# ElenaRyumina/AVCER

Measured on AMD Instinct MI355X. Metric: clips/sec (224x224x16f + 2s@16kHz), full AV path: static CNN + LSTM + wav2vec2 audio model + fusion, higher is better.
Workload: dtype f16x3 (f16 MFMA on hi/lo-split f32 operands, f32 accumulate)

## Files before the change

avcer_amd/_lib.py:

```python
from __future__ import annotations

import ctypes as C
import os

from .build import LIB, source_hash

c_ctx = C.c_void_p
c_stream = C.c_void_p


class ConvDesc(C.Structure):
    _fields_ = [
        ("batch", C.c_int32), ("in_h", C.c_int32), ("in_w", C.c_int32),
        ("out_h", C.c_int32), ("out_w", C.c_int32),
        ("cin", C.c_int32), ("kh", C.c_int32), ("kw", C.c_int32),
        ("stride_h", C.c_int32), ("stride_w", C.c_int32), ("pad_h", C.c_int32), ("pad_w", C.c_int32),
        ("dil_h", C.c_int32), ("dil_w", C.c_int32),
        ("x_stride_b", C.c_int64), ("x_stride_h", C.c_int64), ("x_stride_w", C.c_int64),
        ("x_coff", C.c_int32), ("n", C.c_int32),
        ("y_ld", C.c_int64), ("y_coff", C.c_int32),
        ("r_ld", C.c_int64), ("r_coff", C.c_int32),
        ("act", C.c_int32), ("res_after_act", C.c_int32), ("groups", C.c_int32),
        ("x2_cin", C.c_int32), ("x2_coff", C.c_int32), ("x2_stride", C.c_int32),
        ("x2_stride_b", C.c_int64), ("x2_stride_h", C.c_int64), ("x2_stride_w", C.c_int64),
        ("tile_n", C.c_int32),
        ("r_sub", C.c_int32), ("r_h", C.c_int32), ("r_w", C.c_int32),
        ("tile_m", C.c_int32),
    ]


ABI_VERSION = 8
SPLIT_TRAILER = 256

SIGNATURES = {
    "avcer_abi_version": (C.c_int, []),
    "avcer_source_hash": (C.c_char_p, []),
    "avcer_ctx_create": (C.c_int, [C.c_int, C.POINTER(c_ctx)]),
    "avcer_ctx_destroy": (None, [c_ctx]),
    "avcer_last_error": (C.c_char_p, [c_ctx]),
    "avcer_x3_overflow_count": (C.c_int, [c_ctx, C.c_int, C.POINTER(C.c_int64), c_stream]),
    "avcer_load_static": (C.c_int, [c_ctx, C.c_void_p, C.c_size_t]),
    "avcer_load_dynamic": (C.c_int, [c_ctx, C.c_void_p, C.c_size_t]),
    "avcer_load_audio": (C.c_int, [c_ctx, C.c_void_p, C.c_size_t]),
    "avcer_static_forward": (C.c_int, [c_ctx, C.c_void_p, C.c_int, C.c_int, C.c_int, C.c_int, C.c_void_p, C.c_void_p,
                                       C.c_void_p, c_stream]),
    "avcer_set_static_batch": (C.c_int, [c_ctx, C.c_int]),
    "avcer_set_static_back_batch": (C.c_int, [c_ctx, C.c_int]),
    "avcer_set_static_lanes": (C.c_int, [c_ctx, C.c_int]),
    "avcer_set_static_lane_range": (C.c_int, [c_ctx, C.c_int, C.c_int]),
    "avcer_static_forward_nchw": (C.c_int, [c_ctx, C.c_void_p, C.c_int, C.c_int, C.c_void_p, C.c_void_p, C.c_void_p,
                                            c_stream]),
    "avcer_gather_windows": (C.c_int, [c_ctx, C.c_void_p, C.c_void_p, C.c_int, C.c_void_p, c_stream]),
    "avcer_dynamic_forward": (C.c_int, [c_ctx, C.c_void_p, C.c_int, C.c_void_p, c_stream]),
    "avcer_dynamic_forward_mode": (C.c_int, [c_ctx, C.c_void_p, C.c_int, C.c_int, C.c_void_p, c_stream]),
    "avcer_audio_forward": (C.c_int, [c_ctx, C.c_void_p, C.c_int, C.c_int, C.c_int, C.c_int, C.c_void_p, c_stream]),
    "avcer_audio_num_classes": (C.c_int, [c_ctx]),
    "avcer_audio_head_kind": (C.c_int, [c_ctx]),
    "avcer_audio_forward_features": (C.c_int, [c_ctx, C.c_void_p, C.c_int, C.c_int, C.c_int, C.c_int, C.c_void_p, C.c_void_p,
                                               c_stream]),
    "avcer_gru_layer": (C.c_int, [c_ctx, C.c_void_p, C.c_void_p, C.c_void_p, C.c_int, C.c_int, C.c_int, C.c_int, C.c_void_p,
                                  c_stream]),
    "avcer_audio_chunks": (C.c_int, [c_ctx, C.c_void_p, C.c_void_p, C.c_void_p, C.c_int, C.c_int, C.c_int, C.c_void_p,
                                     c_stream]),
    "avcer_resample": (C.c_int, [c_ctx, C.c_void_p, C.c_int, C.c_int64, C.c_int, C.c_void_p, C.c_void_p, C.c_int, C.c_int, C.c_int,
                                 C.c_int, C.c_void_p, C.c_int64, c_stream]),
    "avcer_weight_search_counts": (C.c_int, [c_ctx, C.c_void_p, C.c_void_p, C.c_int64, C.c_int, C.c_int, C.c_void_p, C.c_int,
                                             C.c_void_p, C.c_void_p, c_stream]),
    "avcer_audio_frame_mean": (C.c_int, [c_ctx, C.c_void_p, C.c_void_p, C.c_void_p, C.c_int, C.c_int, C.c_int,
                                         C.c_void_p, C.c_void_p, c_stream]),
    "avcer_load_face": (C.c_int, [c_ctx, C.c_void_p, C.c_size_t]),
    "avcer_face_num_priors": (C.c_int, [C.c_int, C.c_int]),
    "avcer_face_kind": (C.c_int, [c_ctx]),
    "avcer_s3fd_num_priors": (C.c_int, [C.c_int, C.c_int]),
    "avcer_s3fd_detect": (C.c_int, [c_ctx, C.c_void_p, C.c_void_p, C.c_void_p] + [C.c_int] * 4 + [C.c_float] * 4 + [C.c_int] * 2 +
                          [C.c_float, C.c_void_p, C.c_void_p, c_stream]),
    "avcer_face_forward": (C.c_int, [c_ctx, C.c_void_p, C.c_int, C.c_int, C.c_int, C.c_int, C.c_int, C.c_void_p,
                                     C.c_void_p, C.c_void_p, c_stream]),
    "avcer_face_decode": (C.c_int, [c_ctx, C.c_void_p, C.c_void_p, C.c_void_p, C.c_void_p, C.c_int, C.c_int, C.c_int,
                                    C.c_float, C.c_float, C.c_void_p, c_stream]),
    "avcer_face_decode_batch": (C.c_int, [c_ctx, C.c_void_p, C.c_void_p, C.c_void_p, C.c_void_p, C.c_int, C.c_int, C.c_int, C.c_int,
                                          C.c_float, C.c_float, C.c_void_p, c_stream]),
    "avcer_track_faces": (C.c_int, [c_ctx, C.c_void_p, C.c_int, C.c_void_p, C.c_int, C.c_int, C.c_int, C.c_double, C.c_double,
                                    C.c_void_p, C.POINTER(C.c_int64)]),
    "avcer_lsap": (C.c_int, [C.c_int, C.c_int, C.c_void_p, C.c_void_p, C.c_void_p]),
    "avcer_tracker_create": (C.c_void_p, [C.c_double, C.c_double]),
    "avcer_tracker_push": (C.c_int, [C.c_void_p, C.c_void_p, C.c_int, C.c_void_p, C.c_int, C.c_int64, C.c_int, C.c_int, C.c_void_p,
                                     C.POINTER(C.c_int64)]),
    "avcer_tracker_last_error": (C.c_char_p, [C.c_void_p]),
    "avcer_tracker_destroy": (None, [C.c_void_p]),
    "avcer_jpeg_probe": (C.c_int, [C.c_void_p, C.c_size_t, C.c_void_p]),
    "avcer_jpeg_entropy_batch": (C.c_int, [c_ctx, C.c_void_p, C.c_void_p, C.c_int, C.c_void_p, C.c_int64, C.c_void_p, C.c_int,
                                           C.POINTER(C.c_int64)]),
    "avcer_jpeg_tiles": (C.c_int, [c_ctx, C.c_void_p, C.c_int64, C.c_void_p, C.c_int, C.c_void_p, C.c_void_p, c_stream]),
    "avcer_jpeg_rgb": (C.c_int, [c_ctx, C.c_void_p, C.c_int64, C.c_void_p, C.c_int, C.c_void_p, C.c_void_p, C.c_int, C.c_int, c_stream]),
    "avcer_jpeg_frames": (C.c_int, [c_ctx, C.c_void_p, C.c_int64, C.c_void_p, C.c_int, C.c_void_p, C.c_void_p, C.c_int, C.c_int, C.c_int,
                                    c_stream]),
    "avcer_jpeg_entropy_batch_ex": (C.c_int, [c_ctx, C.c_void_p, C.c_void_p, C.c_int, C.c_void_p, C.c_int64, C.c_void_p, C.c_int, C.c_int,
                                              C.POINTER(C.c_int64)]),
    "avcer_jpeg_scan_batch_ex": (C.c_int, [c_ctx, C.c_void_p, C.c_void_p, C.c_int, C.c_void_p, C.c_int64, C.c_void_p, C.c_void_p, C.c_void_p,
                                           C.c_int, C.c_int, C.c_int, C.POINTER(C.c_int32), C.POINTER(C.c_int64), C.POINTER(C.c_int64)]),
    "avcer_jpeg_quant_tables": (C.c_int, [C.c_int, C.c_void_p]),
    "avcer_jpeg_plan": (C.c_int, [C.c_void_p, C.c_int, C.c_int, C.c_int, C.c_void_p, C.POINTER(C.c_int64)]),
    "avcer_jpeg_forward": (C.c_int, [c_ctx, C.c_void_p, C.c_int, C.c_int, C.c_int, C.c_void_p, C.c_void_p, C.c_int, C.c_int, C.c_void_p,
                                     C.c_int64, c_stream]),
    "avcer_jpeg_write_batch": (C.c_int, [c_ctx, C.c_void_p, C.c_void_p, C.c_int, C.c_void_p, C.c_int64, C.c_void_p, C.c_int,
                                         C.POINTER(C.c_int64)]),
    "avcer_jpeg_roundtrip_tiles": (C.c_int, [c_ctx, C.c_void_p, C.c_int, C.c_int, C.c_int, C.c_void_p, C.c_void_p, C.c_int, C.c_int,
                                             C.c_void_p, C.c_int64, C.c_void_p, C.c_void_p, c_stream]),
    "avcer_jpeg_roundtrip_rgb": (C.c_int, [c_ctx, C.c_void_p, C.c_int, C.c_int, C.c_int, C.c_void_p, C.c_void_p, C.c_int, C.c_int,
                                           C.c_void_p, C.c_int64, C.c_void_p, C.c_void_p, C.c_int, C.c_int, c_stream]),
    "avcer_jpeg_pack": (C.c_int, [c_ctx, C.c_void_p, C.c_int64, C.c_void_p, C.c_int, C.c_void_p, C.c_int64, C.c_void_p, C.c_void_p,
                                  C.c_void_p, c_stream]),
    "avcer_jpeg_scan_batch": (C.c_int, [c_ctx, C.c_void_p, C.c_void_p, C.c_int, C.c_void_p, C.c_int64, C.c_void_p, C.c_void_p, C.c_void_p,
                                        C.c_int, C.c_int, C.POINTER(C.c_int32), C.POINTER(C.c_int64), C.POINTER(C.c_int64)]),
    "avcer_jpeg_unpack": (C.c_int, [c_ctx, C.c_void_p, C.c_int64, C.c_void_p, C.c_void_p, C.c_int, C.c_void_p, C.c_int, C.c_void_p,
                                    C.c_int64, C.c_void_p, C.c_int, c_stream]),
    "avcer_jpeg_unpack_host": (C.c_int, [c_ctx, C.c_void_p, C.c_int64, C.c_void_p, C.c_void_p, C.c_int, C.c_void_p, C.c_int, C.c_void_p,
                                         C.c_int64, C.c_void_p, C.c_int]),
    "avcer_crop_tiles": (C.c_int, [c_ctx, C.c_void_p, C.c_int, C.c_int, C.c_int, C.c_void_p, C.c_int, C.c_int,
                                   C.c_void_p, c_stream]),
    "avcer_static_forward_cam": (C.c_int, [c_ctx, C.c_void_p, C.c_int, C.c_int, C.c_int, C.c_int, C.c_void_p, C.c_void_p,
                                           C.c_void_p, C.c_void_p, c_stream]),
    "avcer_crop_resize_linear": (C.c_int, [c_ctx, C.c_void_p, C.c_int, C.c_int, C.c_int, C.c_void_p, C.c_int, C.c_int, C.c_int,
                                           C.c_int, C.c_void_p, c_stream]),
    "avcer_cam_render": (C.c_int, [c_ctx, C.c_void_p, C.c_void_p, C.c_void_p, C.c_void_p, C.c_int, C.c_void_p, C.c_double,
                                   C.c_void_p, c_stream]),
    "avcer_annotate_frames": (C.c_int, [c_ctx, C.c_void_p, C.c_int, C.c_int, C.c_int, C.c_void_p, C.c_int, C.c_void_p, C.c_int64,
                                        C.c_void_p, C.c_int, C.c_void_p, C.c_int, C.c_int64, c_stream]),
    "avcer_fuse":(C.c_int, [c_ctx, C.c_void_p, C.c_void_p, C.c_void_p, C.c_int, C.c_int, C.c_int, C.c_void_p,
                             C.c_void_p, C.c_int, C.c_int, C.c_void_p, C.c_void_p, c_stream]),
    "avcer_fuse_videos": (C.c_int, [c_ctx] + [C.c_void_p] * 8 + [C.c_int, C.c_int64, C.c_int64, C.c_int, C.c_void_p, C.c_void_p,
                                    C.c_int, C.c_int] + [C.c_void_p] * 4 + [c_stream]),
    "avcer_conv_gemm": (C.c_int, [c_ctx, C.POINTER(ConvDesc), C.c_int, C.c_void_p, C.c_void_p, C.c_void_p, C.c_void_p,
                                  C.c_void_p, C.c_void_p, c_stream]),
    "avcer_split_weights": (C.c_int, [c_ctx, C.c_void_p, C.c_void_p, C.c_size_t, c_stream]),
    "avcer_split_weight_rows": (C.c_int, [c_ctx, C.c_void_p, C.c_void_p, C.c_int, C.c_int, c_stream]),
    "avcer_weight_frags": (C.c_int, [c_ctx, C.c_void_p, C.c_void_p, C.c_int, C.c_int, c_stream]),
    "avcer_conv_gemm_dual": (C.c_int, [c_ctx, C.POINTER(ConvDesc), C.c_int, C.c_void_p, C.c_void_p, C.c_void_p, C.c_void_p,
                                       C.c_void_p, C.c_void_p, C.c_void_p, c_stream]),
    "avcer_face_nms": (C.c_int, [c_ctx, C.c_void_p, C.c_int, C.c_int, C.c_float, C.c_float, C.c_int, C.c_int, C.c_float,
                                 C.c_void_p, C.c_void_p, c_stream]),
    "avcer_dwsep": (C.c_int, [c_ctx] + [C.c_int] * 7 + [C.c_void_p] * 8 + [C.c_void_p]),
    "avcer_s3fd_stem": (C.c_int, [c_ctx, C.c_void_p] + [C.c_int] * 4 + [C.c_void_p] * 3 + [C.c_int, c_stream]),
    "avcer_maxpool2": (C.c_int, [c_ctx, C.c_void_p, C.c_void_p] + [C.c_int] * 6 + [c_stream]),
    "avcer_s3fd_head": (C.c_int, [c_ctx, C.c_void_p, C.c_int] + [C.c_void_p] * 3 + [C.c_int] * 7 + [C.c_void_p, C.c_void_p, c_stream]),
    "avcer_bneck_chain": (C.c_int, [c_ctx, C.c_int, C.c_int, C.c_int, C.c_int, C.c_void_p, C.c_void_p, C.c_int, C.c_int] + [C.c_void_p] * 9 +
                          [c_stream]),
    "avcer_bneck_tail": (C.c_int, [c_ctx, C.c_int, C.c_int64] + [C.c_void_p] * 8 + [c_stream]),
    "avcer_stem_pool": (C.c_int, [c_ctx, C.c_void_p, C.c_size_t, C.c_void_p, C.c_void_p, C.c_void_p, C.c_void_p, C.c_int, c_stream]),
    "avcer_stem_pool_u8": (C.c_int, [c_ctx, C.c_void_p, C.c_int, C.c_int, C.c_int, C.c_void_p, C.c_void_p, C.c_void_p, C.c_void_p,
                                     c_stream]),
    "avcer_attention_long": (C.c_int, [c_ctx, C.c_void_p, C.c_void_p, C.c_int, C.c_int, C.c_int, C.c_int, C.c_float, C.c_int, C.c_int,
                                       c_stream]),
    "avcer_set_audio_max_tokens": (C.c_int, [c_ctx, C.c_int]),
    "avcer_audio_max_tokens": (C.c_int, [c_ctx]),
    "avcer_attention": (C.c_int, [c_ctx, C.c_void_p, C.c_void_p, C.c_int, C.c_int, C.c_int, C.c_int, C.c_float, C.c_int, C.c_int,
                                  c_stream]),
    "avcer_measure_ceilings": (C.c_int, [c_ctx, C.POINTER(C.c_double), C.POINTER(C.c_double), c_stream]),
    "avcer_gemm_stats": (C.c_int, [c_ctx, C.POINTER(C.c_int64), C.POINTER(C.c_double), C.c_int]),
    "avcer_profile_enable": (C.c_int, [c_ctx, C.c_int]),
    "avcer_profile_read": (C.c_int, [c_ctx, C.POINTER(C.c_double), C.POINTER(C.c_int64)]),
    "avcer_profile_read_families": (C.c_int, [c_ctx, C.c_int, C.POINTER(C.c_double), C.POINTER(C.c_int64), C.POINTER(C.c_double),
                                              C.POINTER(C.c_double)]),
    "avcer_profile_read_launches": (C.c_int, [c_ctx, C.c_int64, C.c_void_p, C.c_void_p, C.c_void_p, C.c_void_p, C.c_void_p,
                                              C.POINTER(C.c_int64)]),
    "avcer_debug_tap": (C.c_int, [c_ctx, C.c_char_p, C.c_void_p, C.c_size_t]),
    "avcer_debug_tap_copied": (C.c_int64, [c_ctx]),
}

_lib = None
_PRODUCT_LIB = LIB


def load() -> C.CDLL:
    global _lib
    if _lib is None:
        if not os.path.exists(LIB):
            raise RuntimeError(
                f"{LIB} is missing: run `python -m avcer_amd.build` (hipcc, gfx950). "
                "avcer_amd has no CPU or PyTorch fallback for the hot path.")
        import torch

        lib = C.CDLL(LIB, mode=C.RTLD_GLOBAL)
        for name, (res, args) in SIGNATURES.items():
            fn = getattr(lib, name)
            fn.restype = res
            fn.argtypes = args
        if lib.avcer_abi_version() != ABI_VERSION:
            raise RuntimeError(f"{LIB}: ABI version {lib.avcer_abi_version()}, this binding is written for {ABI_VERSION} "
                               "(include/avcer_hip.h AVCER_ABI_VERSION): rebuild with `python -m avcer_amd.build`")
        check_source_hash(lib, LIB)
        _lib = lib
    return _lib


def check_source_hash(lib, path: str, tree_hash: str | None = None) -> str:
    have = lib.avcer_source_hash().decode()
    want = tree_hash if tree_hash is not None else source_hash()
    if "+lab" in have or os.path.abspath(path) != os.path.abspath(_PRODUCT_LIB):
        return have
    if have != want:
        raise RuntimeError(f"{path} was built from sources with hash {have}, the tree's csrc/ + include/ hash is {want}: "
                           "stale binary -- rebuild with `python -m avcer_amd.build`")
    return have


class AvcerError(RuntimeError):
    def __init__(self, code: int, msg: str):
        super().__init__(f"libavcer_hip error {code}: {msg}")
        self.code = code
```

avcer_amd/csrc/api.hip:

```cpp
#include "common.h"
#include "split_dev.h"
#include "_source_hash.h"

#include <algorithm>
#include <cmath>
#include <new>

int set_err(avcer_ctx* ctx, int code, const char* fmt, ...) {
    if (ctx) {
        va_list ap;
        va_start(ap, fmt);
        vsnprintf(ctx->err, sizeof(ctx->err), fmt, ap);
        va_end(ap);
    }
    return code;
}

int ws_reserve(avcer_ctx* ctx, int slot, size_t bytes, void** out) {
    DevBuf& b = ctx->ws[slot];
    if (b.cap < bytes) {
        if (b.p) {
            HIP_TRY(ctx, hipDeviceSynchronize());
            HIP_TRY(ctx, hipFree(b.p));
            b.p = nullptr;
// ... 261 lines not shown
    return d;
}

constexpr long kTailPairRows = 16384;
constexpr int kStages[4][3] = {{64, 3, 1}, {128, 4, 2}, {256, 6, 2}, {512, 3, 2}};

int begin_forward(avcer_ctx* ctx, const char* who, Model& m, int mode, bool bf16_form, hipStream_t st) {
    if (mode < AVCER_MODE_FP32 || mode > AVCER_MODE_F16X3) return set_err(ctx, AVCER_EINVAL, "%s: mode %d", who, mode);
    HIP_TRY(ctx, hipSetDevice(ctx->device));
    if (mode == AVCER_MODE_BF16 && bf16_form) TRY(ensure_all_bf16(ctx, m, st));
    if (mode == AVCER_MODE_F16X3) TRY(ensure_all_x3(ctx, m, st));
    return AVCER_OK;
}

struct FaceGeom {
    int OH, OW, PH, PW, MH, MW;
    int fh[5], fw[5];
    int priors;
    int max_frames;
};
FaceGeom face_geom(int H, int W) {
    FaceGeom g{};
    g.OH = (H - 1) / 2 + 1; g.OW = (W - 1) / 2 + 1;
    g.PH = 2 * (g.OH - 1) + 8; g.PW = 2 * (g.OW - 1) + 8;
    g.MH = (g.OH - 1) / 2 + 1; g.MW = (g.OW - 1) / 2 + 1;
    g.fh[1] = g.MH; g.fw[1] = g.MW;
    for (int li = 2; li <= 4; ++li) { g.fh[li] = (g.fh[li - 1] - 1) / 2 + 1; g.fw[li] = (g.fw[li - 1] - 1) / 2 + 1; }
    g.priors = 2 * (g.fh[2] * g.fw[2] + g.fh[3] * g.fw[3] + g.fh[4] * g.fw[4]);
    const size_t per_frame = std::max({(size_t)g.PH * g.PW * 4, (size_t)g.OH * g.OW * 64, (size_t)g.MH * g.MW * 256}) * 4;
    g.max_frames = (int)std::max<size_t>(1, (size_t)0xF0000000u / per_frame);
    return g;
}

}

extern "C" int avcer_abi_version(void) { return AVCER_ABI_VERSION; }
extern "C" const char* avcer_source_hash(void) { return AVCER_SOURCE_HASH; }

extern "C" int avcer_ctx_create(int device, avcer_ctx** out) {
    if (!out) return AVCER_EINVAL;
    *out = nullptr;
    int count = 0;
    if (hipGetDeviceCount(&count) != hipSuccess || device < 0 || device >= count) return AVCER_EHIP;
    if (hipSetDevice(device) != hipSuccess) return AVCER_EHIP;
    avcer_ctx* c = new (std::nothrow) avcer_ctx();
    if (!c) return AVCER_ENOMEM;
    c->device = device;
    hipDeviceProp_t prop;
    if (hipGetDeviceProperties(&prop, device) == hipSuccess && prop.multiProcessorCount > 0)
        c->block_slots = 2 * prop.multiProcessorCount;
    if (hipMalloc((void**)&c->ovf, 256) != hipSuccess || hipMemset(c->ovf, 0, 256) != hipSuccess) {
        (void)hipGetLastError();
        if (c->ovf) (void)hipFree(c->ovf);
        delete c;
        return AVCER_ENOMEM;
    }
    *out = c;
    return AVCER_OK;
}

extern "C" void avcer_ctx_destroy(avcer_ctx* ctx) {
    if (!ctx) return;
    (void)hipSetDevice(ctx->device);
    (void)hipDeviceSynchronize();
    free_model(ctx->stat);
    free_model(ctx->dyn);
    free_model(ctx->aud);
    free_model(ctx->face);
    for (auto& b : ctx->ws)
        if (b.p) (void)hipFree(b.p);
    for (hipEvent_t e : ctx->prof_ev) (void)hipEventDestroy(e);
    if (ctx->ovf) (void)hipFree(ctx->ovf);
    if (ctx->lane_stream) {
        (void)hipStreamDestroy(ctx->lane_stream);
        (void)hipEventDestroy(ctx->lane_ev[0]);
        (void)hipEventDestroy(ctx->lane_ev[1]);
    }
    delete ctx;
}

extern "C" const char* avcer_last_error(const avcer_ctx* ctx) { return ctx ? ctx->err : "null context"; }

extern "C" int avcer_x3_overflow_count(avcer_ctx* ctx, int reset, int64_t* count, avcer_stream_t stream) {
    if (!ctx) return AVCER_EINVAL;
    hipStream_t st = (hipStream_t)stream;
    HIP_TRY(ctx, hipSetDevice(ctx->device));
    if (!count) {
        if (!reset) return set_err(ctx, AVCER_EINVAL, "x3_overflow_count: null count without reset");
        HIP_TRY(ctx, hipMemsetAsync(ctx->ovf, 0, sizeof(unsigned), st));
        return AVCER_OK;
    }
    unsigned host = 0;
    HIP_TRY(ctx, hipMemcpyAsync(&host, ctx->ovf, sizeof(host), hipMemcpyDeviceToHost, st));
    if (reset) HIP_TRY(ctx, hipMemsetAsync(ctx->ovf, 0, sizeof(host), st));
    HIP_TRY(ctx, hipStreamSynchronize(st));
    *count = (int64_t)host;
    return AVCER_OK;
}

extern "C" int avcer_load_static(avcer_ctx* ctx, const void* blob, size_t nbytes) {
    if (!ctx) return AVCER_EINVAL;
    HIP_TRY(ctx, hipSetDevice(ctx->device));
    return load_blob(ctx, ctx->stat, blob, nbytes);
}
extern "C" int avcer_load_dynamic(avcer_ctx* ctx, const void* blob, size_t nbytes) {
    if (!ctx) return AVCER_EINVAL;
    HIP_TRY(ctx, hipSetDevice(ctx->device));
    return load_blob(ctx, ctx->dyn, blob, nbytes);
}
extern "C" int avcer_load_audio(avcer_ctx* ctx, const void* blob, size_t nbytes) {
    if (!ctx) return AVCER_EINVAL;
    HIP_TRY(ctx, hipSetDevice(ctx->device));
    ctx->aud_max_tokens = 256;
    TRY(load_blob(ctx, ctx->aud, blob, nbytes));
    auto it = ctx->aud.t.find("fd.w");
    if (it == ctx->aud.t.end()) return set_err(ctx, AVCER_EFORMAT, "audio blob lacks fd.w");
    ctx->aud_classes = (int)it->second.dims[0];
    const bool gru = ctx->aud.t.count("gru1.whh.w") != 0, tl = ctx->aud.t.count("tl1.qkv.w") != 0;
    ctx->aud_head = gru ? 1 : 3;
    if (gru == tl) {
        free_model(ctx->aud);
        ctx->aud_head = 0;
        ctx->aud_classes = 0;
        return set_err(ctx, AVCER_EINVAL, "audio blob holds %s: one of gru1.whh.w (ExprModelV1) and tl1.qkv.w (ExprModelV2 / V3) is expected",
                       gru ? "both a GRU and a transformer head" : "neither a GRU nor a transformer head");
    }
    return AVCER_OK;
}
extern "C" int avcer_audio_num_classes(const avcer_ctx* ctx) { return ctx ? ctx->aud_classes : 0; }
extern "C" int avcer_audio_head_kind(const avcer_ctx* ctx) { return ctx && ctx->aud.loaded ? ctx->aud_head : 0; }
extern "C" int avcer_audio_max_tokens(const avcer_ctx* ctx) { return ctx ? ctx->aud_max_tokens : 0; }
extern "C" int avcer_set_audio_max_tokens(avcer_ctx* ctx, int tokens) {
    if (!ctx) return AVCER_EINVAL;
    if (!ctx->aud.loaded) return set_err(ctx, AVCER_ESTATE, "set_audio_max_tokens: audio weights not loaded");
    if (tokens < 256 || tokens > AVCER_AUDIO_MAX_TOKENS)
        return set_err(ctx, AVCER_EINVAL, "set_audio_max_tokens: %d outside [256,%d]", tokens, AVCER_AUDIO_MAX_TOKENS);
    auto pe = ctx->aud.t.find("pe");
    if (ctx->aud_head == 3 && (pe == ctx->aud.t.end() || pe->second.dims[0] < tokens))
        return set_err(ctx, AVCER_EINVAL, "set_audio_max_tokens: %d tokens, but the loaded model's pe has %lld rows (pack_audio(sd, pe_rows=...))",
                       tokens, pe == ctx->aud.t.end() ? 0LL : (long long)pe->second.dims[0]);
    ctx->aud_max_tokens = tokens;
    return AVCER_OK;
}

struct Trunk {
    void* X;
    void* pp[2];
    void* T1;
    void* T2;
    int h, w, cin;
    bool stride_last;
    bool w2_frags;
    const char* tap;
};

static void run_bneck_stage(Net& net, Trunk& t, int li, int b_begin, int b_end, int nb, void* last_out, const std::string& end_tap) {
    avcer_ctx* ctx = net.ctx;
    const std::string tap = t.tap;
    const int act = net.act.kind;
    const size_t es = net.act.es;
    const int planes = kStages[li][0], blocks = kStages[li][1];
    const int fused_from = li == 0 ? 0 : 1;
    for (int b = b_begin; b < b_end; ++b) {
        const int s = t.stride_last ? (b == blocks - 1 && li < 3 ? kStages[li + 1][2] : 1) : (b == 0 ? kStages[li][2] : 1);
        const int h = t.h, w = t.w, oh = (h - 1) / s + 1, ow = (w - 1) / s + 1;
        const long M = (long)nb * h * w;
        const std::string p = "l" + std::to_string(li + 1) + "." + std::to_string(b) + ".",
                          pn = "l" + std::to_string(li + 1) + "." + std::to_string(b + 1) + ".";
        void* dst = (b == b_end - 1 && last_out) ? last_out : (t.X == t.pp[0] ? t.pp[1] : t.pp[0]);
        const bool fused = net.x3 && li < 3 && b >= fused_from, chain = fused && li < 2, next = b + 1 < blocks;
        if (!fused || b == fused_from)
            net.gemm(conv2d_desc(nb, h, w, t.cin, 1, 1, 1, 0, planes, 1), p + "c1.w", net.F(p + "c1.s"), net.F(p + "c1.b"), t.X,
                     nullptr, t.T1, act, act);
        if (chain) {
            const bool first = b == 0;
            const Tensor *w2 = net.T(p + "c2.wf"), *w3 = net.T(first ? p + "c3d.w" : p + "c3.wf"),
                         *w1n = next ? net.T(pn + "c1.wf") : nullptr;
            if (net.err != AVCER_OK) return;
            if (!w2->x3 || !w3->x3 || (next && !w1n->x3)) {
                net.err = set_err(ctx, AVCER_ESTATE, "%s: split chain weights not prepared", p.c_str());
                return;
            }
            net.chk(launch_bneck(ctx, planes, nb, h, w, t.T1, t.X, first ? t.cin : 0, s, dst, next ? t.T2 : nullptr, w2->x3,
                                 net.F(p + "c2.b"), w3->x3, net.F(first ? p + "c3d.b" : p + "c3.b"), next ? w1n->x3 : nullptr,
                                 next ? net.F(pn + "c1.b") : nullptr, net.st, t.w2_frags ? w2->x3f : nullptr));
            if (ctx->tap_dst) {
                net.tap((tap + "chain_out:" + p).c_str(), dst, (size_t)nb * oh * ow * planes * 4 * es);
                if (next) net.tap((tap + "chain_t1n:" + p).c_str(), t.T2, (size_t)M * planes * es);
            }
            std::swap(t.T1, t.T2);
        } else {
            net.gemm(conv2d_desc(nb, h, w, planes, 3, 3, s, 1, planes, 1), p + "c2.w", net.F(p + "c2.s"), net.F(p + "c2.b"), t.T1,
                     nullptr, t.T2, act, act);
            avcer_conv_desc d3 = conv2d_desc(nb, oh, ow, planes, 1, 1, 1, 0, planes * 4, 1);
            if (fused && next && M <= kTailPairRows) {
                net.gemm(d3, p + "c3.wf", nullptr, net.F(p + "c3.b"), t.T2, t.X, dst, act, act);
                net.gemm(conv2d_desc(nb, h, w, planes * 4, 1, 1, 1, 0, planes, 1), pn + "c1.wf", nullptr, net.F(pn + "c1.b"), dst,
                         nullptr, t.T1, act, act);
            } else if (fused && next) {
                const Tensor *w3 = net.T(p + "c3.wf"), *w1n = net.T(pn + "c1.wf");
                if (net.err != AVCER_OK) return;
                if (!w3->x3 || !w1n->x3) {
                    net.err = set_err(ctx, AVCER_ESTATE, "%s: split tail weights not prepared", p.c_str());
                    return;
                }
                net.chk(launch_bneck_tail(ctx, planes, M, t.T2, t.X, dst, t.T1, w3->x3, net.F(p + "c3.b"), w1n->x3,
                                          net.F(pn + "c1.b"), net.st));
                if (ctx->tap_dst) {
                    net.tap((tap + "tail_out:" + p).c_str(), dst, (size_t)M * planes * 4 * es);
                    net.tap((tap + "tail_t1n:" + p).c_str(), t.T1, (size_t)M * planes * es);
                }
            } else if (b == 0) {
                d3.x2_cin = t.cin; d3.x2_stride = s;
                d3.x2_stride_b = (int64_t)h * w * t.cin; d3.x2_stride_h = (int64_t)w * t.cin; d3.x2_stride_w = t.cin;
                net.gemm(d3, p + "c3d.w", nullptr, net.F(p + "c3d.b"), t.T2, nullptr, dst, act, act, t.X);
            } else {
                d3.r_sub = s; d3.r_h = h; d3.r_w = w;
                net.gemm(d3, p + "c3.w", net.F(p + "c3.s"), net.F(p + "c3.b"), t.T2, t.X, dst, act, act);
            }
        }
        t.X = dst;
        t.h = oh;
        t.w = ow;
        t.cin = planes * 4;
        const size_t out_bytes = (size_t)nb * oh * ow * t.cin * es;
        if (li == 0 && b == 0) {
            net.tap((tap + "l1b0_c1").c_str(), chain ? t.T2 : t.T1, (size_t)nb * oh * ow * planes * es);
            if (!chain) net.tap((tap + "l1b0_c2").c_str(), t.T2, (size_t)nb * oh * ow * planes * es);
            net.tap((tap + "l1b0").c_str(), t.X, out_bytes);
        }
        if (ctx->tap_dst) net.tap((tap + "blk" + std::to_string(li + 1) + "_" + std::to_string(b)).c_str(), t.X, out_bytes);
    }
    if (b_end == blocks) net.tap(end_tap.c_str(), t.X, (size_t)nb * t.h * t.w * t.cin * es);
}

template <class Lane>
static int run_two_lanes(avcer_ctx* ctx, hipStream_t st, const Lane& lane) {
    auto hip = [ctx](hipError_t e, const char* what) {
        return e == hipSuccess ? AVCER_OK : set_err(ctx, AVCER_EHIP, "two lanes: %s failed: %s", what, hipGetErrorString(e));
    };
    if (!ctx->lane_stream) {
        hipStream_t s = nullptr;
        hipEvent_t ev[2] = {nullptr, nullptr};
        int r = hip(hipStreamCreateWithFlags(&s, hipStreamNonBlocking), "hipStreamCreateWithFlags");
        for (hipEvent_t& e : ev)
            if (r == AVCER_OK) r = hip(hipEventCreateWithFlags(&e, hipEventDisableTiming), "hipEventCreateWithFlags");
        if (r != AVCER_OK) {
            for (hipEvent_t e : ev)
                if (e) (void)hipEventDestroy(e);
            if (s) (void)hipStreamDestroy(s);
            return r;
        }
        ctx->lane_stream = s;
        ctx->lane_ev[0] = ev[0];
        ctx->lane_ev[1] = ev[1];
    }
    hipStream_t s = ctx->lane_stream;
    TRY(hip(hipEventRecord(ctx->lane_ev[0], st), "fork hipEventRecord"));
    int r = hip(hipStreamWaitEvent(s, ctx->lane_ev[0], 0), "fork hipStreamWaitEvent");
    if (r == AVCER_OK) r = lane(1, s);
    if (r == AVCER_OK) r = lane(0, st);
    const hipError_t e = hipEventRecord(ctx->lane_ev[1], s);
    const int rj = hip(e == hipSuccess ? hipStreamWaitEvent(st, ctx->lane_ev[1], 0) : e, "join");
    if (rj != AVCER_OK) (void)hipStreamSynchronize(s);
    return r != AVCER_OK ? r : rj;
}

static int static_forward_lane(avcer_ctx* ctx, int slot, const uint8_t* frames, const float* nchw, int n, int in_h, int in_w, int mode,
                               float* logits, float* probs, float* feats, float* cam, hipStream_t st) {
    Net net{ctx, ctx->stat, mode_storage(mode), st};
    const int act = net.act.kind, bf = act == KIND_BF16;
    const size_t es = net.act.es;
    const int NB = std::min(n, ctx->static_batch);
    const int NS = std::min(n, ctx->static_back > 0 ? ctx->static_back : 2 * NB);
    const size_t back_elems = (size_t)NS * 28 * 28 * 512;
    if (back_elems * es >= 0xF0000000ull) return set_err(ctx, AVCER_EINVAL, "static_forward: %d frames per back pass", NS);
    const int kCamChunk = 256;
    void *P, *buf[4], *bbuf[4], *pooled_sp;
    float *pooled, *feat_ws, *cam_g = nullptr;
    TRY(ws_carve(ctx, slot, "static", [&](Arena& ar) {
        P = ar.get((size_t)NB * 230 * 230 * 4 * es);
        for (auto& b : buf) b = ar.get((size_t)NB * 112 * 112 * 64 * es);
        for (auto& b : bbuf) b = ar.get(back_elems * es);
        pooled = ar.get<float>((size_t)NS * 2048 * 4);
        pooled_sp = ar.get((size_t)NS * 2048 * 4);
        feat_ws = ar.get<float>((size_t)NS * 512 * 4);
        if (cam) cam_g = ar.get<float>((size_t)std::min(NS, kCamChunk) * 7 * 2048 * 4);
    }));
    auto run_stem = [&](int f0, int nb, void** B) {
        if (net.x3) {
            const Tensor* w = net.T("stem7.w");
            if (net.err != AVCER_OK) return;
            if (!w->x3) { net.err = set_err(ctx, AVCER_ESTATE, "stem7.w: split weights not prepared"); return; }
            if (frames) {
                net.chk(launch_stem_pool_u8(ctx, frames + (size_t)f0 * in_h * in_w * 3, in_h, in_w, w->x3, net.F("stem.s"),
                                            net.F("stem.b9"), B[1], nb, st));
                net.tap("stem", B[1], (size_t)nb * 55 * 55 * 64 * es);
                return;
            }
            net.chk(k_pack_nchw(ctx, nchw + (size_t)f0 * 3 * 224 * 224, nb, P, 3, st));
            net.chk(launch_stem_pool(ctx, P, (size_t)nb * 230 * 230 * 4 * 2, w->x3, net.F("stem.s"), net.F("stem.b"), B[1], nb, st));
            net.tap("stem", B[1], (size_t)nb * 55 * 55 * 64 * es);
            return;
        }
        if (frames) net.chk(k_preprocess(ctx, frames + (size_t)f0 * in_h * in_w * 3, nb, in_h, in_w, P, bf, st));
        else net.chk(k_pack_nchw(ctx, nchw + (size_t)f0 * 3 * 224 * 224, nb, P, bf, st));
        net.gemm(stem_desc(nb, 230, 230), "stem.w", net.F("stem.s"), net.F("stem.b"), P, nullptr, B[0], bf, act);
        net.tap("pre", P, (size_t)nb * 230 * 230 * 4 * es);
        net.tap("stem_conv", B[0], (size_t)nb * 112 * 112 * 64 * es);
        net.chk(k_maxpool(ctx, B[0], B[1], nb, 112, 112, 64, 3, 0, 55, 55, act, st));
        net.tap("stem", B[1], (size_t)nb * 55 * 55 * 64 * es);
    };
    for (int s0 = 0; s0 < n; s0 += NS) {
        const int nb = std::min(NS, n - s0);
        for (int c0 = 0; c0 < nb; c0 += NB) {
            const int cn = std::min(NB, nb - c0);
            Trunk t{buf[1], {buf[0], buf[1]}, buf[2], buf[3], 55, 55, 64, true, true, ""};
            run_stem(s0 + c0, cn, buf);
            run_bneck_stage(net, t, 0, 0, kStages[0][1], cn, nullptr, "layer1");
            run_bneck_stage(net, t, 1, 0, 1, cn, (char*)bbuf[0] + (size_t)c0 * 28 * 28 * 512 * es, "layer2");
        }
        Trunk t{bbuf[0], {bbuf[1], bbuf[0]}, bbuf[2], bbuf[3], 28, 28, 512, true, true, ""};
        for (int li = 1; li < 4; ++li)
            run_bneck_stage(net, t, li, li == 1 ? 1 : 0, kStages[li][1], nb, nullptr, "layer" + std::to_string(li + 1));
        net.chk(k_avgpool_hw(ctx, t.X, pooled, net.x3 ? pooled_sp : nullptr, nb, t.h * t.w, 2048, act, st));
        net.tap("avgpool", pooled, (size_t)nb * 2048 * 4);
        float* fo = feats ? feats + (size_t)s0 * 512 : feat_ws;
        {
            avcer_conv_desc fd = linear_desc(nb, 2048, 512, 0);
            fd.tile_n = 64;
            if (net.x3) net.gemm(fd, "fc1.w", nullptr, net.F("fc1.b"), pooled_sp, nullptr, fo, KIND_SP32, KIND_F32);
            else net.gemm(fd, "fc1.w", nullptr, net.F("fc1.b"), pooled, nullptr, fo, KIND_F32, KIND_F32);
        }
        if (logits || probs)
            net.chk(k_small_linear(ctx, fo, net.F("fc2.w"), net.F("fc2.b"), logits ? logits + (size_t)s0 * 7 : nullptr,
                                   probs ? probs + (size_t)s0 * 7 : nullptr, nb, 512, 7, 1, st));
        for (int m0 = 0; cam && m0 < nb && net.err == AVCER_OK; m0 += kCamChunk) {
            const int mn = std::min(kCamChunk, nb - m0);
            net.chk(k_cam_maps(ctx, (const char*)t.X + (size_t)m0 * 49 * 2048 * es, probs + (size_t)(s0 + m0) * 7, fo + (size_t)m0 * 512,
                               net.F("fc1.w"), net.F("fc2.w"), cam_g, cam + (size_t)(s0 + m0) * 343, mn, act, st));
        }
        if (net.err != AVCER_OK) return net.err;
    }
    return net.err;
}

static int static_forward_impl(avcer_ctx* ctx, const uint8_t* frames, const float* nchw, int n, int in_h, int in_w, int mode,
                               float* logits, float* probs, float* feats, float* cam, avcer_stream_t stream) {
    if (!ctx) return AVCER_EINVAL;
    if (!ctx->stat.loaded) return set_err(ctx, AVCER_ESTATE, "static weights not loaded");
    if ((!frames && !nchw) || n <= 0 || in_h <= 0 || in_w <= 0) return set_err(ctx, AVCER_EINVAL, "static_forward: bad arguments");
    hipStream_t st = (hipStream_t)stream;
    TRY(begin_forward(ctx, "static_forward", ctx->stat, mode, true, st));
    const bool two = ctx->static_lanes >= 2 && n >= ctx->lane_min && n <= ctx->lane_max && !ctx->prof && !ctx->tap_dst;
    if (!two) return static_forward_lane(ctx, WS_STATIC, frames, nchw, n, in_h, in_w, mode, logits, probs, feats, cam, st);
    const int n0 = (n + 1) / 2;
    const size_t fstep = frames ? (size_t)in_h * in_w * 3 : 0;
    return run_two_lanes(ctx, st, [&](int lane, hipStream_t s) {
        const size_t f0 = lane ? n0 : 0;
        return static_forward_lane(ctx, lane ? WS_STATIC_LANE1 : WS_STATIC, frames ? frames + f0 * fstep : nullptr,
                                   nchw ? nchw + f0 * 3 * 224 * 224 : nullptr, lane ? n - n0 : n0, in_h, in_w, mode,
                                   logits ? logits + f0 * 7 : nullptr, probs ? probs + f0 * 7 : nullptr, feats ? feats + f0 * 512 : nullptr,
                                   cam ? cam + f0 * 343 : nullptr, s);
    });
}

extern "C" int avcer_static_forward(avcer_ctx* ctx, const uint8_t* frames, int n, int in_h, int in_w, int mode,
                                    float* logits, float* probs, float* feats, avcer_stream_t stream) {
    if (!frames) return ctx ? set_err(ctx, AVCER_EINVAL, "static_forward: null frames") : AVCER_EINVAL;
    return static_forward_impl(ctx, frames, nullptr, n, in_h, in_w, mode, logits, probs, feats, nullptr, stream);
}

extern "C" int avcer_static_forward_cam(avcer_ctx* ctx, const uint8_t* frames, int n, int in_h, int in_w, int mode,
                                        float* logits, float* probs, float* feats, float* cam, avcer_stream_t stream) {
    if (!frames || !probs || !cam)
        return ctx ? set_err(ctx, AVCER_EINVAL, "static_forward_cam: null frames, probs or cam") : AVCER_EINVAL;
    return static_forward_impl(ctx, frames, nullptr, n, in_h, in_w, mode, logits, probs, feats, cam, stream);
}

extern "C" int avcer_static_forward_nchw(avcer_ctx* ctx, const float* x, int n, int mode, float* logits, float* probs,
                                         float* feats, avcer_stream_t stream) {
    if (!x) return ctx ? set_err(ctx, AVCER_EINVAL, "static_forward_nchw: null input") : AVCER_EINVAL;
    return static_forward_impl(ctx, nullptr, x, n, 224, 224, mode, logits, probs, feats, nullptr, stream);
}

static int face_forward_lane(avcer_ctx* ctx, int slot, int nb_cap, const uint8_t* frames, int n, int H, int W, int rgb, int mode,
                             float* loc, float* conf, float* landms, hipStream_t st) {
    Net net{ctx, ctx->face, mode_storage(mode), st};
    const int act = net.act.kind, bf = act == KIND_BF16;
    const size_t es = net.act.es;
    const FaceGeom g = face_geom(H, W);
    const int OH = g.OH, OW = g.OW, PH = g.PH, PW = g.PW, MH = g.MH, MW = g.MW, P = g.priors, *fh = g.fh, *fw = g.fw;
    const int NB = std::min({n, nb_cap, g.max_frames});
    const size_t big = (size_t)NB * std::max((size_t)OH * OW * 64, (size_t)MH * MW * 256);
    const size_t lvl = (size_t)NB * fh[2] * fw[2];
    void *Pimg, *buf[4], *feat[5] = {nullptr, nullptr, nullptr, nullptr, nullptr};
    void *pyr[3], *mrg, *S, *t51, *t72;
    float* hd;
    TRY(ws_carve(ctx, slot, "face", [&](Arena& ar) {
        Pimg = ar.get((size_t)NB * PH * PW * 4 * es);
        for (auto& b : buf) b = ar.get(big * es);
        for (int li = 2; li <= 4; ++li) feat[li] = ar.get((size_t)NB * fh[li] * fw[li] * kStages[li - 1][0] * 4 * es);
        for (auto& b : pyr) b = ar.get(lvl * 256 * es);
        mrg = ar.get(lvl * 256 * es);
        S = ar.get(lvl * 256 * es);
        t51 = ar.get(lvl * 64 * es);
        t72 = ar.get(lvl * 64 * es);
        hd = ar.get<float>(lvl * 64 * 4);
    }));

    for (int s0 = 0; s0 < n; s0 += NB) {
        const int nb = std::min(NB, n - s0);
        if (net.x3) {
            const Tensor* w7 = net.T("stem7.w");
            if (net.err != AVCER_OK) return net.err;
            if (!w7->x3) return set_err(ctx, AVCER_ESTATE, "face stem7.w: split weights not prepared");
            net.chk(launch_stem_pool_face(ctx, frames + (size_t)s0 * H * W * 3, H, W, rgb, w7->x3, net.F("stem.s"), net.F("stem.b"), buf[1],
                                          nb, st));
        } else {
            net.chk(k_face_pre(ctx, frames + (size_t)s0 * H * W * 3, nb, H, W, PH, PW, rgb, Pimg, bf, st));
            net.gemm(stem_desc(nb, PH, PW), "stem.w", net.F("stem.s"), net.F("stem.b"), Pimg, nullptr, buf[0], bf, act);
            net.tap("face_stem_conv", buf[0], (size_t)nb * OH * OW * 64 * es);
            net.chk(k_maxpool(ctx, buf[0], buf[1], nb, OH, OW, 64, 3, 1, MH, MW, act, st));
        }
        net.tap("face_pool", buf[1], (size_t)nb * MH * MW * 64 * es);
        Trunk t{buf[1], {buf[0], buf[1]}, buf[2], buf[3], MH, MW, 64, false, false, "face_"};
        for (int li = 0; li < 4; ++li)
            run_bneck_stage(net, t, li, 0, kStages[li][1], nb, li ? feat[li + 1] : nullptr,
                            li ? "face_body" + std::to_string(li) : "face_layer1");
        if (net.err != AVCER_OK) return net.err;
        for (int i = 0; i < 3; ++i) {
            const int li = i + 2, c = kStages[li - 1][0] * 4;
            const std::string p = "fpn.o" + std::to_string(i + 1) + ".";
            net.gemm(conv2d_desc(nb, fh[li], fw[li], c, 1, 1, 1, 0, 256, 1), p + "w", net.F(p + "s"), net.F(p + "b"), feat[li], nullptr,
                     pyr[i], act, act);
        }
        auto conv3 = [&](const std::string& p, const void* x, int hh, int ww, int c, void* y, int nout, int y_ld, int y_coff,
                         int relu, int okind) {
            avcer_conv_desc d = conv2d_desc(nb, hh, ww, c, 3, 3, 1, 1, nout, relu);
            d.y_ld = y_ld; d.y_coff = y_coff;
            net.gemm(d, p + "w", net.F(p + "s"), net.F(p + "b"), x, nullptr, y, act, okind);
        };
        void* lvl_in[3] = {nullptr, nullptr, pyr[2]};
        net.tap("face_lat1", pyr[0], (size_t)nb * fh[2] * fw[2] * 256 * es);
        net.tap("face_lat2", pyr[1], (size_t)nb * fh[3] * fw[3] * 256 * es);
        net.tap("face_lat3", pyr[2], (size_t)nb * fh[4] * fw[4] * 256 * es);
        net.chk(k_upsample_add(ctx, pyr[1], pyr[2], nb, fh[3], fw[3], fh[4], fw[4], 256, act, st));
        void* m2 = t.T1;
        net.tap("face_sum2", pyr[1], (size_t)nb * fh[3] * fw[3] * 256 * es);
        conv3("fpn.m2.", pyr[1], fh[3], fw[3], 256, m2, 256, 256, 0, 1, act);
        net.tap("face_fpn2", m2, (size_t)nb * fh[3] * fw[3] * 256 * es);
        net.chk(k_upsample_add(ctx, pyr[0], m2, nb, fh[2], fw[2], fh[3], fw[3], 256, act, st));
        conv3("fpn.m1.", pyr[0], fh[2], fw[2], 256, mrg, 256, 256, 0, 1, act);
        lvl_in[0] = mrg; lvl_in[1] = m2;
        net.tap("face_fpn1", mrg, (size_t)nb * fh[2] * fw[2] * 256 * es);
        int row0 = 0;
        for (int i = 0; i < 3; ++i) {
            const int hh = fh[i + 2], ww = fw[i + 2];
            const std::string p = "ssh" + std::to_string(i + 1) + ".";
            conv3(p + "c3.", lvl_in[i], hh, ww, 256, S, 128, 256, 0, 1, act);
            conv3(p + "c51.", lvl_in[i], hh, ww, 256, t51, 64, 64, 0, 1, act);
            conv3(p + "c52.", t51, hh, ww, 64, S, 64, 256, 128, 1, act);
            conv3(p + "c72.", t51, hh, ww, 64, t72, 64, 64, 0, 1, act);
            conv3(p + "c73.", t72, hh, ww, 64, S, 64, 256, 192, 1, act);
            if (i == 0) net.tap("face_ssh1", S, (size_t)nb * hh * ww * 256 * es);
            const std::string hp = "head" + std::to_string(i) + ".";
            net.gemm(linear_desc((long)nb * hh * ww, 256, 64, 0), hp + "w", nullptr, net.F(hp + "b"), S, nullptr, hd, act, KIND_F32);
            net.chk(k_face_head(ctx, hd, 64, nb, hh * ww, row0, P, loc + (size_t)s0 * P * 4, conf + (size_t)s0 * P * 2,
                                landms + (size_t)s0 * P * 10, st));
            row0 += hh * ww * 2;
        }
// ... 679 lines not shown
    if (frames < 1 || frames > 1024) return set_err(ctx, AVCER_EINVAL, "static batch %d outside [1,1024]", frames);
    ctx->static_batch = frames;
    return AVCER_OK;
}

extern "C" int avcer_set_static_lanes(avcer_ctx* ctx, int lanes) {
    if (!ctx) return AVCER_EINVAL;
    if (lanes < 1 || lanes > 2) return set_err(ctx, AVCER_EINVAL, "static lanes %d outside [1,2]", lanes);
    ctx->static_lanes = lanes;
    return AVCER_OK;
}

extern "C" int avcer_set_static_lane_range(avcer_ctx* ctx, int min_frames, int max_frames) {
    if (!ctx) return AVCER_EINVAL;
    if (min_frames < 2 || max_frames > 4096 || min_frames > max_frames)
        return set_err(ctx, AVCER_EINVAL, "static lane range [%d, %d] outside 2 <= min <= max <= 4096", min_frames, max_frames);
    ctx->lane_min = min_frames;
    ctx->lane_max = max_frames;
    return AVCER_OK;
}

extern "C" int avcer_set_static_back_batch(avcer_ctx* ctx, int frames) {
    if (!ctx) return AVCER_EINVAL;
    if (frames < 0 || frames > 2048) return set_err(ctx, AVCER_EINVAL, "static back batch %d outside [0,2048]", frames);
    ctx->static_back = frames;
    return AVCER_OK;
}

extern "C" int avcer_profile_enable(avcer_ctx* ctx, int on) {
    if (!ctx) return AVCER_EINVAL;
    ctx->prof = on != 0;
    ctx->prof_used = 0;
    for (int f = 0; f < 8; ++f) { ctx->fam_launches[f] = 0; ctx->fam_flops[f] = 0.0; ctx->fam_bytes[f] = 0.0; }
    return AVCER_OK;
}

extern "C" int avcer_profile_read_families(avcer_ctx* ctx, int n_fam, double* ms, int64_t* launches, double* flops, double* bytes) {
    if (!ctx || n_fam < 1 || n_fam > 8 || !ms || !launches || !flops || !bytes) return ctx ? set_err(ctx, AVCER_EINVAL, "profile_read_families: bad arguments") : AVCER_EINVAL;
    HIP_TRY(ctx, hipSetDevice(ctx->device));
    for (int f = 0; f < n_fam; ++f) { ms[f] = 0.0; launches[f] = 0; flops[f] = 0.0; bytes[f] = 0.0; }
    for (size_t i = 0; i + 1 < ctx->prof_used; i += 2) {
        HIP_TRY(ctx, hipEventSynchronize(ctx->prof_ev[i + 1]));
        float t = 0.f;
        HIP_TRY(ctx, hipEventElapsedTime(&t, ctx->prof_ev[i], ctx->prof_ev[i + 1]));
        const int f = ctx->prof_fam[i / 2];
        if (f < n_fam) ms[f] += t;
    }
    for (int f = 0; f < n_fam && f < 8; ++f) {
        launches[f] = ctx->fam_launches[f]; flops[f] = ctx->fam_flops[f]; bytes[f] = ctx->fam_bytes[f];
        ctx->fam_launches[f] = 0; ctx->fam_flops[f] = 0.0; ctx->fam_bytes[f] = 0.0;
    }
    ctx->prof_used = 0;
    return AVCER_OK;
}

extern "C" int avcer_profile_read_launches(avcer_ctx* ctx, int64_t max_n, int32_t* fam, double* ms, double* flops, double* bytes,
                                           int64_t* mnk, int64_t* n) {
    if (!ctx || max_n < 0 || !n || (max_n && (!fam || !ms || !flops || !bytes || !mnk)))
        return ctx ? set_err(ctx, AVCER_EINVAL, "profile_read_launches: bad arguments") : AVCER_EINVAL;
    HIP_TRY(ctx, hipSetDevice(ctx->device));
    const int64_t have = (int64_t)(ctx->prof_used / 2);
    for (int64_t i = 0; i < have && i < max_n; ++i) {
        HIP_TRY(ctx, hipEventSynchronize(ctx->prof_ev[2 * i + 1]));
        float t = 0.f;
        HIP_TRY(ctx, hipEventElapsedTime(&t, ctx->prof_ev[2 * i], ctx->prof_ev[2 * i + 1]));
        const auto& l = ctx->prof_log[i];
        fam[i] = ctx->prof_fam[i]; ms[i] = t; flops[i] = l.flops; bytes[i] = l.bytes;
        mnk[3 * i] = l.m; mnk[3 * i + 1] = l.n; mnk[3 * i + 2] = l.k;
    }
    *n = have;
    for (int f = 0; f < 8; ++f) { ctx->fam_launches[f] = 0; ctx->fam_flops[f] = 0.0; ctx->fam_bytes[f] = 0.0; }
    ctx->prof_used = 0;
    return AVCER_OK;
}

extern "C" int avcer_profile_read(avcer_ctx* ctx, double* total_ms, int64_t* launches) {
    if (!ctx) return AVCER_EINVAL;
    HIP_TRY(ctx, hipSetDevice(ctx->device));
    double ms = 0.0;
    for (size_t i = 0; i + 1 < ctx->prof_used; i += 2) {
        HIP_TRY(ctx, hipEventSynchronize(ctx->prof_ev[i + 1]));
        float t = 0.f;
        HIP_TRY(ctx, hipEventElapsedTime(&t, ctx->prof_ev[i], ctx->prof_ev[i + 1]));
        ms += t;
    }
    if (total_ms) *total_ms = ms;
    if (launches) *launches = (int64_t)(ctx->prof_used / 2);
    ctx->prof_used = 0;
    return AVCER_OK;
}

extern "C" int avcer_debug_tap(avcer_ctx* ctx, const char* name, void* dst_dev, size_t bytes) {
    if (!ctx || !name) return AVCER_EINVAL;
    ctx->tap_name = name;
    ctx->tap_dst = dst_dev;
    ctx->tap_bytes = bytes;
    ctx->tap_copied = -1;
    return AVCER_OK;
}

extern "C" int64_t avcer_debug_tap_copied(const avcer_ctx* ctx) { return ctx ? ctx->tap_copied : -1; }

extern "C" int avcer_conv_gemm_dual(avcer_ctx* ctx, const avcer_conv_desc* d, int dtype, const void* x, const void* x2,
                                    const void* w, const float* scale, const float* bias, const void* residual, void* y,
                                    avcer_stream_t stream) {
    if (!ctx || !d || !x2) return AVCER_EINVAL;
    HIP_TRY(ctx, hipSetDevice(ctx->device));
    return launch_conv_gemm(ctx, *d, dtype, x, w, scale, bias, residual, y, (hipStream_t)stream, x2);
}

extern "C" int avcer_bneck_chain(avcer_ctx* ctx, int planes, int nb, int h, int w, const void* t1, const void* x, int ds_cin,
                                 int out_step, void* out, void* t1n, const void* w2, const float* b2, const void* w3, const float* b3,
                                 const void* w1n, const float* b1n, const void* w2_frags, avcer_stream_t stream) {
    if (!ctx) return AVCER_EINVAL;
    if (nb <= 0 || h <= 0 || w <= 0) return set_err(ctx, AVCER_EINVAL, "bneck_chain: bad geometry");
    HIP_TRY(ctx, hipSetDevice(ctx->device));
    return launch_bneck(ctx, planes, nb, h, w, t1, x, ds_cin, out_step, out, t1n, w2, b2, w3, b3, w1n, b1n, (hipStream_t)stream, w2_frags);
}

extern "C" int avcer_bneck_tail(avcer_ctx* ctx, int planes, int64_t M, const void* t2, const void* x, void* out, void* t1n, const void* w3,
                                const float* b3, const void* w1n, const float* b1n, avcer_stream_t stream) {
    if (!ctx) return AVCER_EINVAL;
    HIP_TRY(ctx, hipSetDevice(ctx->device));
    return launch_bneck_tail(ctx, planes, (long)M, t2, x, out, t1n, w3, b3, w1n, b1n, (hipStream_t)stream);
}

extern "C" int avcer_dwsep(avcer_ctx* ctx, int cin, int cout, int stride, int mode, int nb, int h, int w, const float* x, const float* dw_w,
                           const float* dw_s, const float* dw_b, const void* pw_w, const float* pw_s, const float* pw_b, float* y,
                           avcer_stream_t stream) {
    if (!ctx) return AVCER_EINVAL;
    if (!x || !dw_w || !dw_s || !dw_b || !pw_w || !pw_s || !pw_b || !y) return set_err(ctx, AVCER_EINVAL, "dwsep: null argument");
    if (mode != AVCER_MODE_FP32 && mode != AVCER_MODE_F16X3)
        return set_err(ctx, AVCER_EINVAL, "dwsep: mode %d (AVCER_MODE_FP32 and AVCER_MODE_F16X3 only)", mode);
    HIP_TRY(ctx, hipSetDevice(ctx->device));
    return launch_dwsep(ctx, cin, cout, stride, mode == AVCER_MODE_F16X3, x, dw_w, dw_s, dw_b, pw_w, pw_s, pw_b, y, nb, h, w,
                        (hipStream_t)stream);
}

extern "C" int avcer_stem_pool(avcer_ctx* ctx, const void* planes_hi_lo, size_t plane_bytes, const void* w, const float* scale,
                               const float* bias, void* y, int n, avcer_stream_t stream) {
    if (!ctx) return AVCER_EINVAL;
    if (plane_bytes != (size_t)n * 230 * 230 * 4 * 2) return set_err(ctx, AVCER_EINVAL, "stem_pool: plane_bytes != n*230*230*4*2");
    HIP_TRY(ctx, hipSetDevice(ctx->device));
    return launch_stem_pool(ctx, planes_hi_lo, plane_bytes, w, scale, bias, y, n, (hipStream_t)stream);
}

extern "C" int avcer_stem_pool_u8(avcer_ctx* ctx, const uint8_t* frames, int n, int in_h, int in_w, const void* w, const float* scale,
                                  const float* shifts9, void* y, avcer_stream_t stream) {
    if (!ctx) return AVCER_EINVAL;
    HIP_TRY(ctx, hipSetDevice(ctx->device));
    return launch_stem_pool_u8(ctx, frames, in_h, in_w, w, scale, shifts9, y, n, (hipStream_t)stream);
}

extern "C" int avcer_split_weights(avcer_ctx* ctx, const float* w, void* out, size_t numel, avcer_stream_t stream) {
    if (!ctx) return AVCER_EINVAL;
    if (!w || !out || numel % 32) return set_err(ctx, AVCER_EINVAL, "split_weights: numel must be a multiple of 32");
    HIP_TRY(ctx, hipSetDevice(ctx->device));
    return k_split_weights(ctx, w, (bf16_t*)out, numel, (hipStream_t)stream);
}

extern "C" int avcer_split_weight_rows(avcer_ctx* ctx, const float* w, void* out, int n, int k, avcer_stream_t stream) {
    if (!ctx) return AVCER_EINVAL;
    if (!w || !out || n <= 0 || k <= 0) return set_err(ctx, AVCER_EINVAL, "split_weight_rows: bad arguments");
    HIP_TRY(ctx, hipSetDevice(ctx->device));
    return k_split_weight_rows(ctx, w, (bf16_t*)out, n, k, (hipStream_t)stream);
}

extern "C" int avcer_attention(avcer_ctx* ctx, const void* qkv, void* out, int n, int s, int heads, int head_dim, float scale,
                               int in_kind, int out_kind, avcer_stream_t stream) {
    if (!ctx) return AVCER_EINVAL;
    if (!qkv || !out || n <= 0 || heads <= 0) return set_err(ctx, AVCER_EINVAL, "attention: bad arguments");
    HIP_TRY(ctx, hipSetDevice(ctx->device));
    return k_attention(ctx, qkv, out, n, s, heads, head_dim, scale, in_kind, out_kind, (hipStream_t)stream);
}

extern "C" int avcer_attention_long(avcer_ctx* ctx, const void* qkv, void* out, int n, int s, int heads, int head_dim, float scale,
                                    int in_kind, int out_kind, avcer_stream_t stream) {
    if (!ctx) return AVCER_EINVAL;
    if (!qkv || !out || n <= 0 || heads <= 0) return set_err(ctx, AVCER_EINVAL, "attention_long: bad arguments");
    HIP_TRY(ctx, hipSetDevice(ctx->device));
    return k_attention_long(ctx, qkv, out, n, s, heads, head_dim, scale, in_kind, out_kind, (hipStream_t)stream);
}

extern "C" int avcer_weight_frags(avcer_ctx* ctx, const void* rows, void* out, int n, int k, avcer_stream_t stream) {
    if (!ctx) return AVCER_EINVAL;
    if (!rows || !out || n <= 0 || k <= 0) return set_err(ctx, AVCER_EINVAL, "weight_frags: bad arguments");
    HIP_TRY(ctx, hipSetDevice(ctx->device));
    return k_weight_frags(ctx, (const bf16_t*)rows, (bf16_t*)out, n, k, (hipStream_t)stream);
}

extern "C" int avcer_measure_ceilings(avcer_ctx* ctx, double* mfma_bf16_tflops, double* hbm_copy_tbs, avcer_stream_t stream) {
    if (!ctx) return AVCER_EINVAL;
    HIP_TRY(ctx, hipSetDevice(ctx->device));
    return measure_ceilings(ctx, mfma_bf16_tflops, hbm_copy_tbs, (hipStream_t)stream);
}

extern "C" int avcer_gemm_stats(avcer_ctx* ctx, int64_t* launches, double* flops, int reset) {
    if (!ctx) return AVCER_EINVAL;
    if (launches) *launches = ctx->gemm_launches;
    if (flops) *flops = ctx->gemm_flops;
    if (reset) {
        ctx->gemm_launches = 0;
        ctx->gemm_flops = 0.0;
    }
    return AVCER_OK;
}
```

avcer_amd/csrc/common.h:

```cpp
#pragma once

#include <hip/hip_runtime.h>

#include <cstdarg>
#include <cstdint>
#include <cstdio>
#include <cstring>
#include <map>
#include <string>
#include <type_traits>
#include <vector>

#include "../../include/avcer_hip.h"
#include "arena.h"

typedef uint16_t bf16_t;

struct DevBuf {
    void* p = nullptr;
    size_t cap = 0;
};

enum { WS_STATIC = 0, WS_DYNAMIC = 1, WS_AUDIO = 2, WS_FACE = 3, WS_NMS = 4, WS_CEILINGS = 5, WS_STATIC_LANE1 = 6, WS_FACE_LANE1 = 7,
       WS_GRU = 8, WS_JPEG = 9, WS_COUNT = 10 };

enum { KIND_F32 = 0, KIND_BF16 = 1, KIND_SP32 = 2 };
struct Storage { int kind; size_t es; };
inline Storage mode_storage(int mode) {
    return mode == AVCER_MODE_BF16 ? Storage{KIND_BF16, 2} : Storage{mode == AVCER_MODE_F16X3 ? KIND_SP32 : KIND_F32, 4};
}
struct sp32_t;
template <typename T> struct storage_tag { using type = T; };
template <typename T> constexpr int storage_kind = std::is_same<T, bf16_t>::value ? KIND_BF16 : std::is_same<T, sp32_t>::value ? KIND_SP32 : KIND_F32;
template <typename T0, typename... Ts, typename F> void with_storage(int kind, F&& f) {
    if (!((kind == storage_kind<Ts> ? (f(storage_tag<Ts>{}), true) : false) || ...)) f(storage_tag<T0>{});
}
template <typename F> void with_storage(int kind, F&& f) { with_storage<float, bf16_t, sp32_t>(kind, f); }

struct Tensor {
    float* f32 = nullptr;
    bf16_t* bf16 = nullptr;
    bf16_t* x3 = nullptr;
    bf16_t* x3f = nullptr;
    size_t numel = 0;
    int64_t dims[4] = {0, 0, 0, 0};
    int ndim = 0;
};

struct Model {
    bool loaded = false;
    std::map<std::string, Tensor> t;
    std::vector<void*> allocs;
};

struct avcer_ctx {
    int device = 0;
    char err[512] = {0};
    Model stat, dyn, aud, face;
    int face_kind = 0;
    int aud_classes = 0;
    int aud_head = 0;
    int aud_max_tokens = 256;
    int static_batch = 1024;
    int static_back = 0;
    int static_lanes = 2;
    int lane_min = 32, lane_max = 2048;
    hipStream_t lane_stream = nullptr;
    hipEvent_t lane_ev[2] = {nullptr, nullptr};
    int block_slots = 512;
    DevBuf ws[WS_COUNT];
    unsigned* ovf = nullptr;
    int64_t gemm_launches = 0;
    double gemm_flops = 0.0;
    bool prof = false;
    std::vector<hipEvent_t> prof_ev;
    std::vector<int> prof_fam;
    struct ProfLaunch { double flops, bytes; long m, n, k; };
    std::vector<ProfLaunch> prof_log;
    size_t prof_used = 0;
    int64_t fam_launches[8] = {0};
    double fam_flops[8] = {0};
    double fam_bytes[8] = {0};
    std::string tap_name;
    void* tap_dst = nullptr;
    size_t tap_bytes = 0;
    int64_t tap_copied = -1;
};

int set_err(avcer_ctx* ctx, int code, const char* fmt, ...);

#define HIP_TRY(ctx, expr)                                                                         \
    do {                                                                                           \
        hipError_t _e = (expr);                                                                    \
        if (_e != hipSuccess)                                                                      \
            return set_err((ctx), AVCER_EHIP, "%s failed: %s (%s:%d)", #expr, hipGetErrorString(_e), \
                           __FILE__, __LINE__);                                                    \
    } while (0)

#define TRY(expr)                  \
    do {                           \
        int _r = (expr);           \
        if (_r != AVCER_OK) return _r; \
    } while (0)

#define CHECK_LAUNCH(ctx, name)                                                                      \
    do {                                                                                             \
        hipError_t _e = hipGetLastError();                                                           \
        if (_e != hipSuccess) return set_err((ctx), AVCER_EHIP, name " launch: %s", hipGetErrorString(_e)); \
    } while (0)

inline int cdiv(long a, long b) { return (int)((a + b - 1) / b); }

int ws_reserve(avcer_ctx* ctx, int slot, size_t bytes, void** out);

template <class Alloc, class Carve>
int carve_measured(avcer_ctx* ctx, const char* what, const Alloc& alloc, const Carve& carve) {
    const size_t bytes = Arena().run(carve);
    void* p = nullptr;
    if (bytes) TRY(alloc(bytes, &p));
    return Arena(p, bytes).run(carve) == bytes ? AVCER_OK : set_err(ctx, AVCER_ENOMEM, "%s workspace arithmetic", what);
}

template <class Carve>
int ws_carve(avcer_ctx* ctx, int slot, const char* what, const Carve& carve) {
    return carve_measured(ctx, what, [&](size_t bytes, void** p) { return ws_reserve(ctx, slot, bytes, p); }, carve);
}

__device__ __forceinline__ int nearest_src(int o, int len) { return min((int)(((double)o + 0.5) * ((double)len / 224.0)), len - 1); }

inline double grid_rounds(long tiles, long slots) {
    const long whole = tiles / slots, rest = tiles % slots;
    if (whole == 0) return 2 * tiles <= slots ? 0.62 : 1.0;
    const double f = (double)rest / (double)slots;
    return (double)whole + (rest == 0 ? 0.0 : (2 * rest <= slots ? 0.25 + 0.7 * f : 1.0));
}

int launch_conv_gemm(avcer_ctx* ctx, const avcer_conv_desc& d, int dtype, const void* x, const void* w,
                     const float* scale, const float* bias, const void* residual, void* y, hipStream_t st,
                     const void* x2 = nullptr);

enum { FAM_GEMM = 0, FAM_GEMM_WD = 1, FAM_CHAIN = 2, FAM_TAIL = 3, FAM_STEM = 4, FAM_SKINNY = 5, FAM_GRU = 6, FAM_COUNT = 7 };
int prof_begin(avcer_ctx* ctx, hipStream_t st, hipEvent_t* ev0, hipEvent_t* ev1, int family, double flops, double bytes, long M = 0,
               long N = 0, long K = 0);

int launch_stem_pool(avcer_ctx* ctx, const void* planes, size_t plane_bytes, const void* w_x3, const float* scale,
                     const float* bias, void* y, int n, hipStream_t st);
int launch_stem_pool_u8(avcer_ctx* ctx, const uint8_t* frames, int in_h, int in_w, const void* w_x3, const float* scale,
                        const float* bias9, void* y, int n, hipStream_t st);
int launch_stem_pool_face(avcer_ctx* ctx, const uint8_t* frames, int h, int w, int rgb, const void* w_x3, const float* scale,
                          const float* bias, void* y, int n, hipStream_t st);
int launch_bneck(avcer_ctx* ctx, int planes, int nb, int h, int w, const void* t1, const void* x, int ds_cin, int out_step,
                 void* out, void* t1n, const void* w2, const float* b2, const void* w3, const float* b3, const void* w1n,
                 const float* b1n, hipStream_t st, const void* w2_frags = nullptr);

int launch_bneck_tail(avcer_ctx* ctx, int planes, long M, const void* t2, const void* x, void* out, void* t1n, const void* w3,
                      const float* b3, const void* w1n, const float* b1n, hipStream_t st);

int launch_gru_layer(avcer_ctx* ctx, const float* xp, const void* w, int x3, const float* bhh, int n, int S, float* h_seq, void* h_sp,
                     hipStream_t st);

int launch_mnet_stem(avcer_ctx* ctx, const uint8_t* frames, int n, int h, int w, int rgb, const float* wt, const float* s, const float* b,
                     float* y, hipStream_t st);
int launch_dwsep(avcer_ctx* ctx, int cin, int cout, int stride, int x3, const float* x, const float* dww, const float* dws,
                 const float* dwb, const void* pw, const float* pws, const float* pwb, float* y, int nb, int h, int w, hipStream_t st);
int launch_mnet_conv(avcer_ctx* ctx, int ks, const float* x, const float* wt, const float* s, const float* b, float* y, int n, int h, int w,
                     int cin, int cout, int y_ld, int y_coff, int act, hipStream_t st);

int launch_s3fd_stem(avcer_ctx* ctx, const uint8_t* frames, int n, int h, int w, int rgb, const float* wt, const float* b, void* y, int kind,
                     hipStream_t st);
int launch_s3fd_head(avcer_ctx* ctx, const void* x, int kind, float* inv, const float* wt, const float* b, int nb, int h, int w, int c,
                     int n_out, int row0, int P, float* loc, float* conf, hipStream_t st);
size_t s3fd_detect_ws_bytes(int T, int P, int nms_top_k);
int launch_s3fd_detect(avcer_ctx* ctx, const float* loc, const float* conf, const float* priors, int T, int P, int im_h, int im_w, float var0,
                       float var1, float conf_thresh, float nms_thresh, int nms_top_k, int top_k, float threshold, void* ws, float* out,
                       int32_t* out_n, hipStream_t st);

int measure_ceilings(avcer_ctx* ctx, double* mfma_bf16_tflops, double* hbm_copy_tbs, hipStream_t st);

int k_preprocess(avcer_ctx*, const uint8_t* frames, int n, int in_h, int in_w, void* out, int kind, hipStream_t);
int k_maxpool(avcer_ctx*, const void* x, void* y, int n, int h, int w, int c, int k, int pad, int oh, int ow, int kind, hipStream_t);
int k_avgpool_hw(avcer_ctx*, const void* x, float* y, void* y_sp32, int n, int hw, int c, int kind, hipStream_t);
int k_cam_maps(avcer_ctx*, const void* x, const float* probs, const float* h, const float* w1, const float* w2, float* g,
               float* cam, int n, int kind, hipStream_t);
int k_small_linear(avcer_ctx*, const float* x, const float* w, const float* b, float* logits, float* probs, int m,
                   int k, int n, int relu_in, hipStream_t);
int k_lstm_cell(avcer_ctx*, const float* xproj, int64_t xproj_ld, const float* hproj, float* c, float* h_out, void* h_sp,
                int64_t h_ld, int n, int hid, int first, hipStream_t);
int k_wav_normalize(avcer_ctx*, const float* x, float* y, int n, int t, hipStream_t);
int k_conv0_ln_gelu(avcer_ctx*, const float* x, const float* w, const float* b, const float* g, const float* beta,
                    void* y, int n, int t_in, int t_out, int kind, hipStream_t);
int k_layernorm(avcer_ctx*, const void* x, const void* res, const float* g, const float* b, void* yf, void* yb,
                int64_t rows, int c, float eps, int act, int in_kind, int yb_kind, hipStream_t);
int k_add_pe(avcer_ctx*, const float* x, const float* pe, float* yf, void* yb, int n, int s, int c, int yb_kind, hipStream_t);
int k_attention(avcer_ctx*, const void* qkv, void* out, int n, int s, int heads, int d, float scale, int in_kind,
                int out_kind, hipStream_t);
int k_attention_long(avcer_ctx*, const void* qkv, void* out, int n, int s, int heads, int d, float scale, int in_kind,
                int out_kind, hipStream_t);
int k_maxpool1d_relu(avcer_ctx*, const float* x, float* y, void* y_sp32, int n, int t_in, int t_out, int c, int k, hipStream_t);
int k_mean_time_relu(avcer_ctx*, const float* x, float* y, int n, int t, int c, hipStream_t);
int k_f32_to_bf16(avcer_ctx*, const float* x, bf16_t* y, size_t n, hipStream_t);
int k_frame_mean(avcer_ctx*, const float* win_logits, const int32_t* lo, const int32_t* hi, int n_win, int c,
                 int n_frames, float* out, int32_t* count, hipStream_t);
int k_fuse(avcer_ctx*, const float* stat, const float* dyn, const float* aud, int n, int n_aud, int aud_c,
           const double* w , int has_w1, int cwt, int cmask, double* comp_prob,
           int32_t* comp_argmax, hipStream_t);
int k_fuse_videos(avcer_ctx*, const float* stat, const float* dyn, const float* win, const int32_t* lo, const int32_t* hi,
                  const int32_t* frame_off, const int32_t* win_off, const int32_t* n_aud, int n_videos, int n, int n_win, int c,
                  const double* w, int has_w1, int cwt, int cmask, float* aud_mean, int32_t* count, double* comp_prob,
                  int32_t* comp_argmax, hipStream_t);
int k_pack_nchw(avcer_ctx*, const float* x, int n, void* out, int kind, hipStream_t);
int k_gather_windows(avcer_ctx*, const float* feats, const int32_t* idx, int nwin, float* out, hipStream_t);
int k_audio_chunks(avcer_ctx*, const float* wav, const int32_t* starts, const int32_t* ends, int n, int window, int mode,
                   float* out, hipStream_t);
int k_split_weights(avcer_ctx*, const float* w, bf16_t* out, size_t n, hipStream_t);
int k_split_weight_rows(avcer_ctx*, const float* w, bf16_t* out, int n, int k, hipStream_t);
int k_weight_frags(avcer_ctx*, const bf16_t* rows, bf16_t* out, int n, int k, hipStream_t);
int k_face_decode(avcer_ctx*, const float* loc, const float* conf, const float* landms, const float* priors, int T, int P, int im_h,
                  int im_w, float var0, float var1, float* dets, hipStream_t);
int k_face_nms(avcer_ctx*, const float* dets, int T, int P, float conf_thresh, float nms_thresh, int nms_top_k, int top_k,
               float threshold, int32_t* order, int32_t* count, float* out, int32_t* out_n, hipStream_t);
int k_face_pre(avcer_ctx*, const uint8_t* frames, int n, int h, int w, int ph, int pw, int rgb, void* out, int bf16, hipStream_t);
int k_upsample_add(avcer_ctx*, void* y, const void* coarse, int n, int h, int w, int ch, int cw, int c, int kind, hipStream_t);
int k_face_head(avcer_ctx*, const float* hd, int ld, int n, int hw, int row0, int P, float* loc, float* conf, float* landms,
                hipStream_t);
int k_crop_tiles(avcer_ctx*, const uint8_t* frames, int T, int H, int W, const int32_t* rects, int n, int swap_rb,
                 uint8_t* tiles, hipStream_t);
```

avcer_amd/csrc/fused.hip:

```cpp
#include "common.h"
#include "gemm_dev.h"

#include <algorithm>

namespace {

__device__ __forceinline__ void mfma3(f32x4_t& acc, const spx8_t wh, const spx8_t wl, const spx8_t ah, const spx8_t al) {
    acc = mfma_sp(wl, ah, acc);
    acc = mfma_sp(wh, al, acc);
    acc = mfma_sp(wh, ah, acc);
}

template <int A, int B>
__device__ __forceinline__ void pin(f32x4_t (&acc)[A][B]) {
#pragma unroll
    for (int a = 0; a < A; ++a)
#pragma unroll
        for (int b = 0; b < B; ++b) asm volatile("" : "+v"(acc[a][b]));
}
template <int A>
__device__ __forceinline__ void pin(f32x4_t (&acc)[A]) {
#pragma unroll
    for (int a = 0; a < A; ++a) asm volatile("" : "+v"(acc[a]));
}

__device__ __forceinline__ spx8_t ldfrag(const char* tile, int row, int chunk) {
    return *reinterpret_cast<const spx8_t*>(tile + swz(row, chunk));
}

__device__ __forceinline__ void lds_read8(const float* ptr, f32x4_t& a, f32x4_t& b) {
    const unsigned addr = (unsigned)(size_t)(__attribute__((address_space(3))) const float*)ptr;
    asm volatile("ds_read_b128 %0, %2\n\tds_read_b128 %1, %2 offset:16\n\ts_waitcnt lgkmcnt(0)" : "=&v"(a), "=&v"(b) : "v"(addr) : "memory");
}

__device__ __forceinline__ int xcd_remap(int bid, int nwg) {
    const int q = nwg >> 3, r = nwg & 7;
    const int xcd = bid & 7, idx = bid >> 3;
    return (xcd < r ? xcd * (q + 1) : r * (q + 1) + (xcd - r) * q) + idx;
}

struct StemParams {
    const char* P;
    const uint8_t* F;
    int in_h, in_w;
    const float* bias9;
    unsigned p_bytes;
    unsigned plane_bytes;
    const char* W;
    const float* scale;
    const float* bias;
    char* Y;
    int n;
    unsigned* ovf;
    int oh, ow, mh, mw, tiles_y, tiles_x, swap_rb;
    int mean[3];
};

constexpr int ST_TH = 8, ST_TW = 7;
constexpr int ST_RH = 2 * ST_TH + 1, ST_RW = 2 * ST_TW + 1;
constexpr int ST_TY = 7, ST_TX = 8;

__device__ __forceinline__ int stage64(int row, int chunk) { return row * 256 + ((chunk ^ (row & 7)) << 4); }

__global__ void __launch_bounds__(256, 2) stem_pool_kernel(const StemParams p) {
    constexpr int BN = 64, NK = 7;
    constexpr int PROWS = 2 * (ST_RH - 1) + NK, PCH = (2 * (ST_RW - 1) + 8) / 2;
    constexpr int PLANE = PROWS * PCH * 16;
    constexpr int NCH = 2 * PROWS * PCH;
    constexpr int WOFF = ((2 * PLANE + 1023) / 1024) * 1024;
    constexpr int WT = BN * ROWB;
    constexpr int LDS_BYTES = WOFF + NK * WT > 256 * 256 ? WOFF + NK * WT : 256 * 256;
    __shared__ __attribute__((aligned(16))) char smem[LDS_BYTES];
    const int tid = threadIdx.x, lane = tid & 63;
    const int wave = __builtin_amdgcn_readfirstlane(tid >> 6);
    const int blk = xcd_remap(blockIdx.x, gridDim.x);
    const int b = blk / (ST_TY * ST_TX), t = blk % (ST_TY * ST_TX);
    const int ty = t / ST_TX, tx = t % ST_TX;

    const float wmul = split_wmul(p.W, 64 * NK * ROWB);
    const auto prs = __builtin_amdgcn_make_buffer_rsrc(const_cast<char*>(p.P), (short)0, (int)p.p_bytes, 0x00020000);
    const auto wrs = __builtin_amdgcn_make_buffer_rsrc(const_cast<char*>(p.W), (short)0, 64 * NK * ROWB, 0x00020000);
    const unsigned origin = (unsigned)((((long)b * 230 + 4 * ST_TH * ty) * 230 + 4 * ST_TW * tx) * 8);
#pragma unroll
    for (int j = 0; j < (NCH + 255) / 256; ++j) {
        const int piece = wave + 4 * j;
        const int c = piece * 64 + lane;
        const int plane = c >= NCH / 2, ci = c - plane * (NCH / 2);
        const int prow = ci / PCH, pc = ci - prow * PCH;
        const unsigned off = c < NCH ? origin + (unsigned)(prow * (230 * 8) + pc * 16) + plane * p.plane_bytes : OOB;
        if (piece * 64 < NCH) dma16(prs, smem + piece * 1024, off);
    }
    {
        const int lrow8 = lane >> 3, slot = lane & 7;
#pragma unroll
        for (int j = 0; j < NK * 8 / 4; ++j) {
            const int piece = wave + 4 * j;
            const int ky = piece >> 3, row = (piece & 7) * 8 + lrow8;
            dma16(wrs, smem + WOFF + piece * 1024, (unsigned)(row * (NK * ROWB) + ky * ROWB + ((slot ^ swz_key(row)) << 4)));
        }
    }

    f32x4_t acc[4][4];
#pragma unroll
    for (int a = 0; a < 4; ++a)
#pragma unroll
        for (int c = 0; c < 4; ++c) acc[a][c] = f32x4_t{0};
    const int g = lane >> 4, l15 = lane & 15;
    int abase[4];
#pragma unroll
    for (int fm = 0; fm < 4; ++fm) {
        const int row = wave * 64 + fm * 16 + l15;
        const int ry = row / ST_RW, rx = row - ry * ST_RW;
        abase[fm] = row < ST_RH * ST_RW ? ((2 * ry) * PCH + rx + g) * 16 : 0;
    }
    __syncthreads();
#pragma unroll
    for (int ky = 0; ky < NK; ++ky) {
        const char* sb = smem + WOFF + ky * WT;
        spx8_t ah[4], al[4];
#pragma unroll
        for (int fm = 0; fm < 4; ++fm) {
            ah[fm] = *reinterpret_cast<const spx8_t*>(smem + abase[fm] + ky * (PCH * 16));
            al[fm] = *reinterpret_cast<const spx8_t*>(smem + PLANE + abase[fm] + ky * (PCH * 16));
        }
#pragma unroll
        for (int fn = 0; fn < 4; ++fn) {
            const spx8_t wh = ldfrag(sb, fn * 16 + l15, g), wl = ldfrag(sb, fn * 16 + l15, 4 + g);
#pragma unroll
            for (int fm = 0; fm < 4; ++fm) mfma3(acc[fn][fm], wh, wl, ah[fm], al[fm]);
        }
    }
    pin(acc);
    __syncthreads();
#pragma unroll
    for (int fn = 0; fn < 4; ++fn) {
        const int ch = 32 * (fn >> 1) + 8 * g + 4 * (fn & 1);
        float4 sc = *reinterpret_cast<const float4*>(p.scale + ch);
        const float4 bi = *reinterpret_cast<const float4*>(p.bias + ch);
        sc = make_float4(sc.x * wmul, sc.y * wmul, sc.z * wmul, sc.w * wmul);
#pragma unroll
        for (int fm = 0; fm < 4; ++fm) {
            const int row = wave * 64 + fm * 16 + l15;
            *reinterpret_cast<float4*>(smem + stage64(row, ch >> 2)) =
                make_float4(relu_nan(acc[fn][fm][0] * sc.x + bi.x), relu_nan(acc[fn][fm][1] * sc.y + bi.y),
                            relu_nan(acc[fn][fm][2] * sc.z + bi.z), relu_nan(acc[fn][fm][3] * sc.w + bi.w));
        }
    }
    __syncthreads();
    sp_flags_t ovm = 0;
#pragma unroll
    for (int pass = 0; pass < 2; ++pass) {
        const int item = pass * 256 + tid;
        const int pp = item >> 3, c8 = item & 7;
        const int ppy = pp / ST_TW, ppx = pp - ppy * ST_TW;
        const int py = ST_TH * ty + ppy, px = ST_TW * tx + ppx;
        if (pp >= ST_TH * ST_TW || py >= 55 || px >= 55) continue;
        float m[8];
        bool nan = false;
#pragma unroll
        for (int j = 0; j < 8; ++j) m[j] = 0.f;
        bool anynan[8] = {false, false, false, false, false, false, false, false};
#pragma unroll
        for (int dy = 0; dy < 3; ++dy)
#pragma unroll
            for (int dx = 0; dx < 3; ++dx) {
                const int row = (2 * ppy + dy) * ST_RW + 2 * ppx + dx;
                const float4 u = *reinterpret_cast<const float4*>(smem + stage64(row, 2 * c8));
                const float4 v = *reinterpret_cast<const float4*>(smem + stage64(row, 2 * c8 + 1));
                const float x[8] = {u.x, u.y, u.z, u.w, v.x, v.y, v.z, v.w};
#pragma unroll
                for (int j = 0; j < 8; ++j) { m[j] = fmaxf(m[j], x[j]); anynan[j] |= x[j] != x[j]; }
            }
        (void)nan;
#pragma unroll
        for (int j = 0; j < 8; ++j) if (anynan[j]) m[j] = NAN;
        spx8_t hi, lo;
        sp_split8(m, hi, lo, ovm);
        const long e = (((long)b * 55 + py) * 55 + px) * 64 + c8 * 8;
        char* yp = p.Y + sp32_byte(e);
        *reinterpret_cast<spx8_t*>(yp) = hi;
        *reinterpret_cast<spx8_t*>(yp + 64) = lo;
    }
    sp_commit(p.ovf, ovm);
}

template <bool FACE>
__global__ void __launch_bounds__(256, 3) stem_pool_u8_kernel(const StemParams p) {
    constexpr int NK = 7, WRING = 3;
    constexpr int PROWS = 2 * (ST_RH - 1) + NK, PCH = (2 * (ST_RW - 1) + 8) / 2;
    constexpr int NCH = PROWS * PCH;
    constexpr int WOFF = ((NCH * 16 + 1023) / 1024) * 1024;
    constexpr int WT = 64 * ROWB;
    constexpr int IMG = 256 * 128;
    constexpr int LDS_BYTES = WOFF + WRING * WT > IMG ? WOFF + WRING * WT : IMG;
    __shared__ __attribute__((aligned(16))) char smem[LDS_BYTES];
    const int tid = threadIdx.x, lane = tid & 63;
    const int wave = __builtin_amdgcn_readfirstlane(tid >> 6);
    const int blk = xcd_remap(blockIdx.x, gridDim.x);
    const int tiles_x = FACE ? p.tiles_x : ST_TX, tiles = FACE ? p.tiles_y * p.tiles_x : ST_TY * ST_TX;
    const int b = blk / tiles, t = blk % tiles;
    const int ty = t / tiles_x, tx = t % tiles_x;
    const int lrow8 = lane >> 3, slot = lane & 7;
    const float wmul = split_wmul(p.W, 64 * NK * ROWB);
    const auto wrs = __builtin_amdgcn_make_buffer_rsrc(const_cast<char*>(p.W), (short)0, 64 * NK * ROWB, 0x00020000);
    unsigned w_off[2];
#pragma unroll
    for (int j = 0; j < 2; ++j) {
        const int row = (wave * 2 + j) * 8 + lrow8;
        w_off[j] = (unsigned)(row * (NK * ROWB) + ((slot ^ swz_key(row)) << 4));
    }
#define AVCER_STEM_W(KY)                                                                                              \
    do {                                                                                                              \
        char* dst_ = smem + WOFF + ((KY) % WRING) * WT + wave * 2048;                                                 \
        dma16(wrs, dst_, w_off[0], (unsigned)((KY) * ROWB));                                                          \
        dma16(wrs, dst_ + 1024, w_off[1], (unsigned)((KY) * ROWB));                                                   \
    } while (0)
    AVCER_STEM_W(0);
    AVCER_STEM_W(1);
    {
        const uint8_t* fr = p.F + (long)b * p.in_h * p.in_w * 3;
        const bool resize = !FACE && (p.in_h != 224 || p.in_w != 224);
        const int ih = FACE ? p.in_h : 224, iw = FACE ? p.in_w : 224, org = FACE ? 5 : 2;
        constexpr int PASSES = (NCH + 255) / 256;
        uint8_t raw[PASSES][2][3];
        bool ok[PASSES][2];
#pragma unroll
        for (int j = 0; j < PASSES; ++j) {
            const int ci = min(j * 256 + tid, NCH - 1);
            const int prow = ci / PCH, pc = ci - prow * PCH;
            const int iy = 4 * ST_TH * ty + prow - org;
            int sy = min(max(iy, 0), ih - 1);
            if (resize) sy = min((int)(((double)sy + 0.5) * ((double)p.in_h / 224.0)), p.in_h - 1);
#pragma unroll
            for (int px = 0; px < 2; ++px) {
                const int ix = 4 * ST_TW * tx + 2 * pc + px - org;
                int sx = min(max(ix, 0), iw - 1);
                if (resize) sx = min((int)(((double)sx + 0.5) * ((double)p.in_w / 224.0)), p.in_w - 1);
                ok[j][px] = (unsigned)iy < (unsigned)ih && (unsigned)ix < (unsigned)iw;
                const uint8_t* q = fr + ((long)sy * p.in_w + sx) * 3;
                raw[j][px][0] = q[0]; raw[j][px][1] = q[1]; raw[j][px][2] = q[2];
            }
        }
#pragma unroll
        for (int j = 0; j < PASSES; ++j) {
            const int ci = j * 256 + tid;
            uint32_t wds[4];
#pragma unroll
            for (int px = 0; px < 2; ++px) {
                uint32_t lo2, hi2;
                if constexpr (FACE) {
                    const int c0 = (int)raw[j][px][p.swap_rb ? 2 : 0] - p.mean[0], c1 = (int)raw[j][px][1] - p.mean[1];
                    const int c2 = (int)raw[j][px][p.swap_rb ? 0 : 2] - p.mean[2];
                    lo2 = (uint32_t)f2sp((float)c0) | ((uint32_t)f2sp((float)c1) << 16);
                    hi2 = (uint32_t)f2sp((float)c2);
                } else {
                    lo2 = (uint32_t)f2sp((float)raw[j][px][2]) | ((uint32_t)f2sp((float)raw[j][px][1]) << 16);
                    hi2 = (uint32_t)f2sp((float)raw[j][px][0]);
                }
                wds[2 * px] = ok[j][px] ? lo2 : 0u;
                wds[2 * px + 1] = ok[j][px] ? hi2 : 0u;
            }
            if (ci < NCH) *reinterpret_cast<uint4*>(smem + ci * 16) = make_uint4(wds[0], wds[1], wds[2], wds[3]);
        }
    }
    f32x4_t acc[4][4];
#pragma unroll
    for (int a = 0; a < 4; ++a)
#pragma unroll
        for (int c = 0; c < 4; ++c) acc[a][c] = f32x4_t{0};
    const int g = lane >> 4, l15 = lane & 15;
    int abase[4];
#pragma unroll
    for (int fm = 0; fm < 4; ++fm) {
        const int row = wave * 64 + fm * 16 + l15;
        const int ry = row / ST_RW, rx = row - ry * ST_RW;
        abase[fm] = row < ST_RH * ST_RW ? ((2 * ry) * PCH + rx + g) * 16 : 0;
    }
    __syncthreads();
#pragma unroll
    for (int ky = 0; ky < NK; ++ky) {
        if (ky + 2 < NK) AVCER_STEM_W(ky + 2);
        asm volatile("" ::: "memory");
        const char* sb = smem + WOFF + (ky % WRING) * WT;
        spx8_t ah[4];
#pragma unroll
        for (int fm = 0; fm < 4; ++fm) ah[fm] = *reinterpret_cast<const spx8_t*>(smem + abase[fm] + ky * (PCH * 16));
#pragma unroll
        for (int fn = 0; fn < 4; ++fn) {
            const spx8_t wh = ldfrag(sb, fn * 16 + l15, g), wl = ldfrag(sb, fn * 16 + l15, 4 + g);
#pragma unroll
            for (int fm = 0; fm < 4; ++fm) {
                acc[fn][fm] = mfma_sp(wl, ah[fm], acc[fn][fm]);
                acc[fn][fm] = mfma_sp(wh, ah[fm], acc[fn][fm]);
            }
        }
        pin(acc);
        if (ky + 2 < NK) asm volatile("s_waitcnt vmcnt(2)" ::: "memory");
        else asm volatile("s_waitcnt vmcnt(0)" ::: "memory");
        asm volatile("s_waitcnt lgkmcnt(0)" ::: "memory");
        __builtin_amdgcn_s_barrier();
        asm volatile("" ::: "memory");
    }
#undef AVCER_STEM_W
    sp_flags_t ovm = 0;
#pragma unroll
    for (int half = 0; half < 2; ++half) {
#pragma unroll
        for (int fh = 0; fh < 2; ++fh) {
            const int fn = 2 * half + fh;
            const int ch = 32 * half + 8 * g + 4 * fh;
            float4 sc = *reinterpret_cast<const float4*>(p.scale + ch);
            sc = make_float4(sc.x * wmul, sc.y * wmul, sc.z * wmul, sc.w * wmul);
#pragma unroll
            for (int fm = 0; fm < 4; ++fm) {
                const int row = wave * 64 + fm * 16 + l15;
                const int ry = row / ST_RW, rx = row - ry * ST_RW;
                const int cy = 2 * ST_TH * ty + ry, cx = 2 * ST_TW * tx + rx;
                const int cls = 3 * (cy == 0 ? 0 : (cy >= 110 ? 2 : 1)) + (cx == 0 ? 0 : (cx >= 110 ? 2 : 1));
                const float4 bi = *reinterpret_cast<const float4*>(FACE ? p.bias + ch : p.bias9 + cls * 64 + ch);
                const int chunk = 2 * g + fh;
                *reinterpret_cast<float4*>(smem + row * 128 + ((chunk ^ (row & 7)) << 4)) =
                    make_float4(relu_nan(acc[fn][fm][0] * sc.x + bi.x), relu_nan(acc[fn][fm][1] * sc.y + bi.y),
                                relu_nan(acc[fn][fm][2] * sc.z + bi.z), relu_nan(acc[fn][fm][3] * sc.w + bi.w));
            }
        }
        __syncthreads();
        {
            const int pp = tid >> 2, c8 = tid & 3;
            const int ppy = pp / ST_TW, ppx = pp - ppy * ST_TW;
            const int py = ST_TH * ty + ppy, px = ST_TW * tx + ppx;
            if (pp < ST_TH * ST_TW && py < (FACE ? p.mh : 55) && px < (FACE ? p.mw : 55)) {
                float m[8];
#pragma unroll
                for (int j = 0; j < 8; ++j) m[j] = 0.f;
                bool anynan[8] = {false, false, false, false, false, false, false, false};
#pragma unroll
                for (int dy = 0; dy < 3; ++dy)
#pragma unroll
                    for (int dx = 0; dx < 3; ++dx) {
                        const int row = (2 * ppy + dy) * ST_RW + 2 * ppx + dx;
                        if constexpr (FACE) {
                            const int cy = 2 * py - 1 + dy, cx = 2 * px - 1 + dx;
                            if ((unsigned)cy >= (unsigned)p.oh || (unsigned)cx >= (unsigned)p.ow) continue;
                        }
                        const float4 u = *reinterpret_cast<const float4*>(smem + row * 128 + (((2 * c8) ^ (row & 7)) << 4));
                        const float4 v = *reinterpret_cast<const float4*>(smem + row * 128 + (((2 * c8 + 1) ^ (row & 7)) << 4));
                        const float x[8] = {u.x, u.y, u.z, u.w, v.x, v.y, v.z, v.w};
#pragma unroll
                        for (int j = 0; j < 8; ++j) { m[j] = fmaxf(m[j], x[j]); anynan[j] |= x[j] != x[j]; }
                    }
#pragma unroll
                for (int j = 0; j < 8; ++j) if (anynan[j]) m[j] = NAN;
                spx8_t hi, lo;
                sp_split8(m, hi, lo, ovm);
                const long e = (((long)b * (FACE ? p.mh : 55) + py) * (FACE ? p.mw : 55) + px) * 64 + 32 * half + c8 * 8;
                char* yp = p.Y + sp32_byte(e);
                *reinterpret_cast<spx8_t*>(yp) = hi;
                *reinterpret_cast<spx8_t*>(yp + 64) = lo;
            }
        }
        if (half == 0) __syncthreads();
    }
    sp_commit(p.ovf, ovm);
}

struct BneckParams {
    const char* T1;
    const char* X;
    char* OUT;
    char* T1N;
    const char* W2;
    const char* W2F;
    const char* W3;
    const char* W1N;
    const float *b2, *b3, *b1n;
    unsigned t1_bytes;
    int M, H, Wd;
    int OH, OW;
    unsigned* ovf;
    int nblocks;
};

template <int P, int BM, bool NEXT, int NQX, bool PATCH, int SUB = 1, bool T11 = false>
__global__ void __launch_bounds__(256, P == 64 ? 3 : 2) bneck_kernel(const BneckParams p) {
    static_assert(SUB == 1 || (SUB == 2 && !NEXT && NQX == 0 && !PATCH), "the strided form is the plain last block of a stage");
    static_assert(!T11 || (P == 64 && BM == 128 && !PATCH && SUB == 1), "the spatial-tile form serves planes 64 at full resolution");
    constexpr int NQ = P / 32;
    constexpr int NQT = NQ + NQX;
    constexpr int PSLOTS = PATCH ? (P == 64 ? 456 : 304) : 0;
    constexpr int T11_E = 11, T11_PW = T11_E + 2, T11_SLOTS = 176;
    constexpr int NT = BM / 64;
    constexpr int NG = 4 * P / 32;
    constexpr int TILE_A = (BM + P) * ROWB;
    constexpr int TILE_B = (32 * NQT + P) * ROWB;
    constexpr int PHASE_A = T11 ? NQ * T11_SLOTS * ROWB : (PATCH ? PSLOTS * ROWB + 2 * P * ROWB : 2 * TILE_A);
    constexpr int TILES = PHASE_A > 2 * TILE_B ? PHASE_A : 2 * TILE_B;
    constexpr int NBIAS = 6 * P;
    __shared__ __attribute__((aligned(16))) char smem[TILES + NBIAS * 4];
    float* sbias = reinterpret_cast<float*>(smem + TILES);
    for (int i = threadIdx.x; i < NBIAS; i += 256)
        sbias[i] = i < P ? p.b2[i] : (i < 2 * P ? (NEXT ? p.b1n[i - P] : 0.f) : p.b3[i - 2 * P]);
    const int wave = __builtin_amdgcn_readfirstlane((int)threadIdx.x >> 6);
    sp_flags_t ovm = 0;
    const int tid = threadIdx.x, lane = tid & 63;
    const int g = lane >> 4, l15 = lane & 15;
    const int lrow8 = lane >> 3, slot = lane & 7;
    const int blk = xcd_remap(blockIdx.x, gridDim.x);
    const int m_base = blk * BM;
    const int t11_b = T11 ? blk / 25 : 0, t11_y0 = T11 ? ((blk % 25) / 5) * T11_E : 0, t11_x0 = T11 ? (blk % 5) * T11_E : 0;
    auto row_pos = [&](int r, bool& ok) -> int {
        if constexpr (T11) {
            ok = r < T11_E * T11_E;
            const int rr = ok ? r : T11_E * T11_E - 1;
            const int ry = rr / T11_E, rx = rr - ry * T11_E;
            return (t11_b * 55 + t11_y0 + ry) * 55 + t11_x0 + rx;
        } else {
            const long m = (long)m_base + r;
            ok = m < p.M;
            return ok ? (int)m : 0;
        }
    };

    const float s2 = split_wmul(p.W2, P * 9 * P * 4), s3 = split_wmul(p.W3, 4 * P * (P + 32 * NQX) * 4);
    const float s1n = NEXT ? split_wmul(p.W1N, 4 * P * P * 4) : 1.f;
    (void)s1n;
    const auto t1rs = __builtin_amdgcn_make_buffer_rsrc(const_cast<char*>(p.T1), (short)0, (int)p.t1_bytes, 0x00020000);
    const auto w2rs = __builtin_amdgcn_make_buffer_rsrc(const_cast<char*>(p.W2), (short)0, P * 9 * P * 4, 0x00020000);
    const auto w3rs = __builtin_amdgcn_make_buffer_rsrc(const_cast<char*>(p.W3), (short)0, 4 * P * (P + 32 * NQX) * 4, 0x00020000);
    const auto w1rs = __builtin_amdgcn_make_buffer_rsrc(const_cast<char*>(NEXT ? p.W1N : p.W3), (short)0, 4 * P * P * 4, 0x00020000);

    constexpr int A_ISS = BM / 32;
    constexpr int W_ISS = P / 32;
    unsigned w_off[W_ISS];
#pragma unroll
    for (int j = 0; j < W_ISS; ++j) {
        const int row = wave * (W_ISS * 8) + j * 8 + lrow8;
        w_off[j] = (unsigned)((long)row * (9 * P * 4) + ((slot ^ swz_key(row)) << 4));
    }
    f32x4_t acc2[P / 16][NT];
#pragma unroll
    for (int i = 0; i < P / 16; ++i)
#pragma unroll
        for (int t = 0; t < NT; ++t) acc2[i][t] = f32x4_t{0};
    spx8_t t2h[NQ][NT], t2l[NQ][NT];
    if constexpr (T11) {
        constexpr int PIECES = T11_SLOTS / 8;
#pragma unroll
        for (int q = 0; q < NQ; ++q)
#pragma unroll
            for (int i = 0; i < (PIECES + 3) / 4; ++i) {
                const int ii = wave + 4 * i;
                const int sl = ii * 8 + lrow8;
                const int py = sl / T11_PW, px = sl - py * T11_PW;
                const int y = t11_y0 - 1 + py, x = t11_x0 - 1 + px;
                const bool ok = sl < T11_PW * T11_PW && (unsigned)y < 55u && (unsigned)x < 55u;
                const unsigned off = ok ? (unsigned)(((t11_b * 55 + y) * 55 + x) * (P * 4) + q * ROWB + ((slot ^ swz_key(py * T11_E + px)) << 4)) : OOB;
                if (ii < PIECES) dma16(t1rs, smem + q * (T11_SLOTS * ROWB) + ii * 1024, off);
            }
        constexpr int NKS = 9 * NQ, RING = 4, NPT = BM / 16;
        const unsigned lane16 = (unsigned)lane * 16u;
        const char* w2f = p.W2F + (size_t)wave * (NKS * 2048);
        u32x4_t wq[RING][2];
#define AVCER_T11_LOAD(KS)                                                                                              \
    do {                                                                                                                \
        const char* a_ = w2f + (size_t)(KS) * 2048;                                                                     \
        asm volatile("global_load_dwordx4 %0, %1, %2" : "=v"(wq[(KS) % RING][0]) : "v"(lane16), "s"(a_) : "memory");    \
        asm volatile("global_load_dwordx4 %0, %1, %2 offset:1024" : "=v"(wq[(KS) % RING][1]) : "v"(lane16), "s"(a_) : "memory"); \
    } while (0)
#define AVCER_T11_WAIT(N, KS) asm volatile("s_waitcnt vmcnt(" #N ")" : "+v"(wq[(KS) % RING][0]), "+v"(wq[(KS) % RING][1]) :: "memory")
        static_assert(P == 64, "four waves, four channel tiles");
        int sb8[NPT];
        int sq8[NPT];
#pragma unroll
        for (int t = 0; t < NPT; ++t) {
            const int r = min(t * 16 + l15, T11_E * T11_E - 1);
            const int ry = r / T11_E, rx = r - ry * T11_E;
            sb8[t] = (ry + 1) * T11_PW + rx + 1;
            sq8[t] = (ry + 1) * T11_E + rx + 1;
        }
        f32x4_t acc2c[NPT];
#pragma unroll
        for (int t = 0; t < NPT; ++t) acc2c[t] = f32x4_t{0};
        __syncthreads();
        AVCER_T11_LOAD(0);
        AVCER_T11_LOAD(1);
        AVCER_T11_LOAD(2);
#pragma unroll
        for (int ks = 0; ks < NKS; ++ks) {
            __builtin_amdgcn_sched_barrier(0);
            if (ks + 3 < NKS) { AVCER_T11_LOAD(ks + 3); }
            const int tap = ks / NQ, q = ks % NQ;
            const int toff = (tap / 3 - 1) * T11_PW + (tap % 3 - 1), toffq = (tap / 3 - 1) * T11_E + (tap % 3 - 1);
            const char* plane = smem + q * (T11_SLOTS * ROWB);
            if (ks + 3 < NKS) AVCER_T11_WAIT(6, ks);
            else if (ks + 2 < NKS) AVCER_T11_WAIT(4, ks);
            else if (ks + 1 < NKS) AVCER_T11_WAIT(2, ks);
            else AVCER_T11_WAIT(0, ks);
            __builtin_amdgcn_sched_barrier(0);
            const spx8_t wh = __builtin_bit_cast(spx8_t, wq[ks % RING][0]), wl = __builtin_bit_cast(spx8_t, wq[ks % RING][1]);
#pragma unroll
            for (int t = 0; t < NPT; ++t) {
                const char* row_ = plane + (sb8[t] + toff) * ROWB;
                const int key_ = swz_key(sq8[t] + toffq);
                const spx8_t ah = *reinterpret_cast<const spx8_t*>(row_ + ((g ^ key_) << 4));
                const spx8_t al = *reinterpret_cast<const spx8_t*>(row_ + (((4 + g) ^ key_) << 4));
                mfma3(acc2c[t], wh, wl, ah, al);
            }
        }
#undef AVCER_T11_LOAD
#undef AVCER_T11_WAIT
        pin(acc2c);
        __syncthreads();
        {
            const int qw = wave >> 1, half = wave & 1;
// ... 385 lines not shown
        if (j < G3_ISS) dma16(w3rs, smem + (G & 1) * W3B + g3_dst[j], live ? g3_off[j] : OOB, (unsigned)(G * 32 * P * 4));
        else dma16(w1rs, smem + 2 * W3B + (G & 1) * W1B + (wave * G1_ISS + (j - G3_ISS)) * 1024, live ? g1_off[j - G3_ISS] : OOB,
                   (unsigned)(G * ROWB));
    };
    issue_weights(0);

    const long m = (long)m_base + wave * 16 + l15;
    const bool m_ok = m < p.M;
    const long mc = m_ok ? m : 0;
    const long x_row = mc * (4L * P * 4) + 16 * g;
    const unsigned o_row = m_ok ? (unsigned)x_row : OOB;
    spx8_t t2h[NQ], t2l[NQ];
    {
        const char* tp = p.T1 + mc * (P * 4L) + 16 * g;
#pragma unroll
        for (int q = 0; q < NQ; ++q) {
            t2h[q] = *reinterpret_cast<const spx8_t*>(tp + q * 128);
            t2l[q] = *reinterpret_cast<const spx8_t*>(tp + q * 128 + 64);
        }
    }
    u32x4_t rh0, rl0, rh1, rl1;
    const char* xrow_p = p.X + x_row;
#define AVCER_LOAD_RES(G, H, L)                                                                              \
    do {                                                                                                     \
        const char* rp_ = xrow_p + (G) * 128;                                                                \
        asm volatile("global_load_dwordx4 %0, %1, off" : "=v"(H) : "v"(rp_) : "memory");                     \
        asm volatile("global_load_dwordx4 %0, %1, off offset:64" : "=v"(L) : "v"(rp_) : "memory");           \
    } while (0)
    AVCER_LOAD_RES(0, rh0, rl0);
    AVCER_LOAD_RES(1, rh1, rl1);
    f32x4_t acc1[P / 16];
#pragma unroll
    for (int i = 0; i < P / 16; ++i) acc1[i] = f32x4_t{0};
    sp_flags_t ovm = 0;
    asm volatile("s_waitcnt vmcnt(0)" : "+v"(rh0), "+v"(rl0), "+v"(rh1), "+v"(rl1)::"memory");
    __syncthreads();

#define AVCER_TAIL_GROUP(G, H, L, HN, LN)                                                                                      \
    do {                                                                                                                       \
        const char* w3t = smem + ((G) & 1) * W3B;                                                                              \
        const char* w1t = smem + 2 * W3B + ((G) & 1) * W1B;                                                                    \
        f32x4_t acc3[2] = {f32x4_t{0}, f32x4_t{0}};                                                                            \
        _Pragma("unroll") for (int q = 0; q < NQ; ++q) _Pragma("unroll") for (int tp = 0; tp < 2; ++tp) {                      \
            if (tp == 0) {      \
                            \
                __builtin_amdgcn_sched_barrier(0);                                                                             \
                issue_piece((G) + 1, q);                                                                                       \
                asm volatile("" ::: "memory");                                                                                 \
                __builtin_amdgcn_sched_barrier(0);                                                                             \
            }                                                                                                                  \
            const char* wt = w3t + q * (32 * ROWB);                                                                            \
            mfma3(acc3[tp], ldfrag(wt, tp * 16 + l15, g), ldfrag(wt, tp * 16 + l15, 4 + g), t2h[q], t2l[q]);                   \
        }                                                                                                                      \
        asm volatile("" ::: "memory");                   \
        f32x4_t b0, b1;                                                                                                        \
        lds_read8(sbias + P + 32 * (G) + 8 * g, b0, b1);                                                                       \
        float r[8];                                                                                                            \
        sp_join8(__builtin_bit_cast(uint4, H), __builtin_bit_cast(uint4, L), r);                                                \
        const float v[8] = {relu_nan(__builtin_fmaf(acc3[0][0], s3, b0[0]) + r[0]), relu_nan(__builtin_fmaf(acc3[0][1], s3, b0[1]) + r[1]), \
                            relu_nan(__builtin_fmaf(acc3[0][2], s3, b0[2]) + r[2]), relu_nan(__builtin_fmaf(acc3[0][3], s3, b0[3]) + r[3]), \
                            relu_nan(__builtin_fmaf(acc3[1][0], s3, b1[0]) + r[4]), relu_nan(__builtin_fmaf(acc3[1][1], s3, b1[1]) + r[5]), \
                            relu_nan(__builtin_fmaf(acc3[1][2], s3, b1[2]) + r[6]), relu_nan(__builtin_fmaf(acc3[1][3], s3, b1[3]) + r[7])}; \
        spx8_t oh, ol;                                                                                                       \
        sp_split8(v, oh, ol, ovm);                                                                                                    \
         \
         \
        __builtin_amdgcn_raw_buffer_store_b128(__builtin_bit_cast(u32x4_t, oh), outrs, o_row, (G) * 128, 0);                   \
        __builtin_amdgcn_raw_buffer_store_b128(__builtin_bit_cast(u32x4_t, ol), outrs, o_row, (G) * 128 + 64, 0);              \
        asm volatile("" ::: "memory");                                                                                         \
        AVCER_LOAD_RES((G) + 2 < NG ? (G) + 2 : NG - 1, H, L);           \
        _Pragma("unroll") for (int i = 0; i < P / 16; ++i)                                                                     \
            mfma3(acc1[i], ldfrag(w1t, i * 16 + l15, g), ldfrag(w1t, i * 16 + l15, 4 + g), oh, ol);                            \
        pin(acc1);                                                                                                             \
          \
                 \
                               \
        asm volatile("s_waitcnt vmcnt(4)" : "+v"(HN), "+v"(LN)::"memory");                                                     \
        asm volatile("s_waitcnt lgkmcnt(0)" ::: "memory");                                                                     \
        __builtin_amdgcn_s_barrier();                                                                                          \
        asm volatile("" ::: "memory");                                                                                         \
    } while (0)
    for (int G = 0; G < NG; G += 2) {
        AVCER_TAIL_GROUP(G, rh0, rl0, rh1, rl1);
        AVCER_TAIL_GROUP(G + 1, rh1, rl1, rh0, rl0);
    }
#undef AVCER_TAIL_GROUP
#undef AVCER_LOAD_RES
    asm volatile("s_waitcnt vmcnt(0)" : "+v"(rh0), "+v"(rl0), "+v"(rh1), "+v"(rl1)::"memory");
#pragma unroll
    for (int q = 0; q < NQ; ++q) {
        const float4 b0 = *reinterpret_cast<const float4*>(sbias + 32 * q + 8 * g), b1 = *reinterpret_cast<const float4*>(sbias + 32 * q + 8 * g + 4);
        const f32x4_t lo4 = acc1[2 * q], hi4 = acc1[2 * q + 1];
        const float v[8] = {relu_nan(__builtin_fmaf(lo4[0], s1n, b0.x)), relu_nan(__builtin_fmaf(lo4[1], s1n, b0.y)),
                            relu_nan(__builtin_fmaf(lo4[2], s1n, b0.z)), relu_nan(__builtin_fmaf(lo4[3], s1n, b0.w)),
                            relu_nan(__builtin_fmaf(hi4[0], s1n, b1.x)), relu_nan(__builtin_fmaf(hi4[1], s1n, b1.y)),
                            relu_nan(__builtin_fmaf(hi4[2], s1n, b1.z)), relu_nan(__builtin_fmaf(hi4[3], s1n, b1.w))};
        spx8_t hi, lo;
        sp_split8(v, hi, lo, ovm);
        if (m_ok) {
            char* yp = p.T1N + m * (P * 4L) + q * 128 + 16 * g;
            *reinterpret_cast<spx8_t*>(yp) = hi;
            *reinterpret_cast<spx8_t*>(yp + 64) = lo;
        }
    }
    sp_commit(p.ovf, ovm);
}

__global__ void __launch_bounds__(256, 2) mfma_rate_kernel(float* sink, int iters) {
    const int lane = threadIdx.x & 63;
    spx8_t a, b;
#pragma unroll
    for (int j = 0; j < 8; ++j) {
        a[j] = (spe_t)(0.25f + 0.001f * (float)((lane * 8 + j) % 97));
        b[j] = (spe_t)(-0.5f + 0.002f * (float)((lane * 5 + j * 3 + blockIdx.x) % 89));
    }
    f32x4_t acc[16];
#pragma unroll
    for (int i = 0; i < 16; ++i) acc[i] = f32x4_t{0};
    for (int it = 0; it < iters; ++it) {
#pragma unroll
        for (int i = 0; i < 16; ++i) acc[i] = mfma_sp(a, b, acc[i]);
    }
    float s = 0.f;
#pragma unroll
    for (int i = 0; i < 16; ++i) s += acc[i][0] + acc[i][3];
    if (s == 12345.678f) sink[0] = s;
}

__global__ void copy16_kernel(const uint4* __restrict__ src, uint4* __restrict__ dst, size_t n16) {
    const size_t i = (size_t)blockIdx.x * blockDim.x + threadIdx.x;
    if (i < n16) dst[i] = src[i];
}
}

int launch_stem_pool(avcer_ctx* ctx, const void* planes, size_t plane_bytes, const void* w_x3, const float* scale,
                     const float* bias, void* y, int n, hipStream_t st) {
    if (!planes || !w_x3 || !scale || !bias || !y || n <= 0) return set_err(ctx, AVCER_EINVAL, "stem_pool: bad arguments");
    if (2 * plane_bytes >= (size_t)OOB) return set_err(ctx, AVCER_EINVAL, "stem_pool: %d frames exceed the 4 GiB descriptor", n);
    StemParams p;
    memset(&p, 0, sizeof(p));
    p.P = (const char*)planes; p.plane_bytes = (unsigned)plane_bytes; p.p_bytes = (unsigned)(2 * plane_bytes);
    p.W = (const char*)w_x3; p.scale = scale; p.bias = bias; p.Y = (char*)y; p.n = n; p.ovf = ctx->ovf;
    hipEvent_t ev0 = nullptr, ev1 = nullptr;
    TRY(prof_begin(ctx, st, &ev0, &ev1, FAM_STEM, 2.0 * n * 112.0 * 112.0 * 64 * 147, (double)n * (2.0 * 230 * 230 * 4 * 2 + 55.0 * 55 * 64 * 4)));
    stem_pool_kernel<<<dim3(n * ST_TY * ST_TX), dim3(256), 0, st>>>(p);
    if (ev1) (void)hipEventRecord(ev1, st);
    CHECK_LAUNCH(ctx, "stem_pool");
    ctx->gemm_launches += 1;
    ctx->gemm_flops += 2.0 * n * 112.0 * 112.0 * 64 * 147;
    return AVCER_OK;
}

int launch_stem_pool_u8(avcer_ctx* ctx, const uint8_t* frames, int in_h, int in_w, const void* w_x3, const float* scale,
                        const float* bias9, void* y, int n, hipStream_t st) {
    if (!frames || !w_x3 || !scale || !bias9 || !y || n <= 0 || in_h <= 0 || in_w <= 0)
        return set_err(ctx, AVCER_EINVAL, "stem_pool_u8: bad arguments");
    StemParams p;
    memset(&p, 0, sizeof(p));
    p.F = frames; p.in_h = in_h; p.in_w = in_w; p.bias9 = bias9;
    p.W = (const char*)w_x3; p.scale = scale; p.Y = (char*)y; p.n = n; p.ovf = ctx->ovf;
    hipEvent_t ev0 = nullptr, ev1 = nullptr;
    TRY(prof_begin(ctx, st, &ev0, &ev1, FAM_STEM, 2.0 * n * 112.0 * 112.0 * 64 * 147, (double)n * ((double)in_h * in_w * 3 + 55.0 * 55 * 64 * 4)));
    stem_pool_u8_kernel<false><<<dim3(n * ST_TY * ST_TX), dim3(256), 0, st>>>(p);
    if (ev1) (void)hipEventRecord(ev1, st);
    CHECK_LAUNCH(ctx, "stem_pool_u8");
    ctx->gemm_launches += 1;
    ctx->gemm_flops += 2.0 * n * 112.0 * 112.0 * 64 * 147;
    return AVCER_OK;
}

int launch_stem_pool_face(avcer_ctx* ctx, const uint8_t* frames, int h, int w, int rgb, const void* w_x3, const float* scale,
                          const float* bias, void* y, int n, hipStream_t st) {
    if (!frames || !w_x3 || !scale || !bias || !y || n <= 0 || h <= 0 || w <= 0) return set_err(ctx, AVCER_EINVAL, "stem_pool_face: bad arguments");
    StemParams p;
    memset(&p, 0, sizeof(p));
    p.F = frames; p.in_h = h; p.in_w = w; p.bias = bias;
    p.W = (const char*)w_x3; p.scale = scale; p.Y = (char*)y; p.n = n; p.ovf = ctx->ovf;
    p.oh = (h - 1) / 2 + 1; p.ow = (w - 1) / 2 + 1;
    p.mh = (p.oh - 1) / 2 + 1; p.mw = (p.ow - 1) / 2 + 1;
    p.tiles_y = (p.mh + ST_TH - 1) / ST_TH; p.tiles_x = (p.mw + ST_TW - 1) / ST_TW;
    p.swap_rb = rgb ? 1 : 0;
    p.mean[0] = 104; p.mean[1] = 117; p.mean[2] = 123;
    const long grid = (long)n * p.tiles_y * p.tiles_x;
    if (grid >= (1L << 31)) return set_err(ctx, AVCER_EINVAL, "stem_pool_face: %d frames of %d x %d are too many tiles for one launch", n, h, w);
    hipEvent_t ev0 = nullptr, ev1 = nullptr;
    const double flops = 2.0 * n * (double)p.oh * p.ow * 64 * 147;
    TRY(prof_begin(ctx, st, &ev0, &ev1, FAM_STEM, flops, (double)n * ((double)h * w * 3 + (double)p.mh * p.mw * 64 * 4), (long)n * p.oh * p.ow, 64, 147));
    stem_pool_u8_kernel<true><<<dim3((unsigned)grid), dim3(256), 0, st>>>(p);
    if (ev1) (void)hipEventRecord(ev1, st);
    CHECK_LAUNCH(ctx, "stem_pool_face");
    ctx->gemm_launches += 1;
    ctx->gemm_flops += flops;
    return AVCER_OK;
}

int launch_bneck(avcer_ctx* ctx, int planes, int nb, int h, int w, const void* t1, const void* x, int ds_cin, int out_step,
                 void* out, void* t1n, const void* w2, const float* b2, const void* w3, const float* b3, const void* w1n,
                 const float* b1n, hipStream_t st, const void* w2_frags) {
    if (out_step != 1 && out_step != 2) return set_err(ctx, AVCER_EINVAL, "bneck: out_step %d (1 or 2)", out_step);
    if (out_step == 2 && (t1n || ds_cin)) return set_err(ctx, AVCER_EINVAL, "bneck: the strided form is the last block of a stage (no next conv1, no downsample)");
    const int oh = (h - 1) / out_step + 1, ow = (w - 1) / out_step + 1;
    const long M = (long)nb * oh * ow, M_in = (long)nb * h * w;
    if (!t1 || !x || !out || !w2 || !w3 || !b2 || !b3 || M <= 0)
        return set_err(ctx, AVCER_EINVAL, "bneck: bad arguments");
    if ((t1n != nullptr) != (w1n != nullptr) || (t1n && !b1n))
        return set_err(ctx, AVCER_EINVAL, "bneck: next-block conv1 needs weights, bias and an output");
    if (planes != 64 && planes != 128) return set_err(ctx, AVCER_EINVAL, "bneck: planes %d (64 or 128)", planes);
    if (ds_cin != 0 && !(ds_cin == 64 && planes == 64 && t1n))
        return set_err(ctx, AVCER_EINVAL, "bneck: the downsample form exists for planes 64 with a 64-channel input and a next conv1");
    const long x_bytes = M_in * (long)(ds_cin ? ds_cin : 4 * planes) * 4L, out_bytes = M * 4L * planes * 4L;
    if (M_in * planes * 4L >= (long)OOB || x_bytes >= (long)OOB || out_bytes >= (long)OOB)
        return set_err(ctx, AVCER_EINVAL, "bneck: %ld positions in, %ld out: a tensor of the pass reaches the 4 GiB offset range "
                                          "(at most %ld positions per call at planes %d)", M_in, M, ((long)OOB - 1) / (16L * planes), planes);
    BneckParams p;
    p.T1 = (const char*)t1; p.X = (const char*)x; p.OUT = (char*)out; p.T1N = (char*)t1n;
    p.W2 = (const char*)w2; p.W2F = (const char*)w2_frags; p.W3 = (const char*)w3; p.W1N = (const char*)w1n;
    p.b2 = b2; p.b3 = b3; p.b1n = b1n;
    p.t1_bytes = (unsigned)(M_in * planes * 4);
    p.M = (int)M; p.H = h; p.Wd = w; p.OH = oh; p.OW = ow; p.ovf = ctx->ovf;
    constexpr int BM = 128;
    const bool t11 = planes == 64 && h == 55 && w == 55 && out_step == 1 && t1n && w2_frags;
    p.nblocks = t11 ? nb * 25 : (int)((M + BM - 1) / BM);
    const int grid = p.nblocks;
    hipEvent_t ev0 = nullptr, ev1 = nullptr;
    {
        const double bytes = 4.0 * ((double)M_in * planes + (double)M * (ds_cin ? ds_cin : 4 * planes) + (double)M * 4 * planes +
                                    (t1n ? (double)M * planes : 0.0));
        TRY(prof_begin(ctx, st, &ev0, &ev1, FAM_CHAIN, 2.0 * (double)M * planes * (planes * (9.0 + 4.0 + (t1n ? 4.0 : 0.0)) + 4.0 * ds_cin), bytes, M,
                       4 * planes, planes));
    }
    const int rows_worst = (w - 1 + BM + w - 1) / w + 2 + 2;
    const bool patch = planes == 128 && (long)h * w >= BM && rows_worst * (w + 2) <= 304;
    if (out_step == 2) {
        if (planes == 64) bneck_kernel<64, BM, false, 0, false, 2><<<dim3(grid), dim3(256), 0, st>>>(p);
        else bneck_kernel<128, BM, false, 0, false, 2><<<dim3(grid), dim3(256), 0, st>>>(p);
    } else if (ds_cin) {
        if (t11) bneck_kernel<64, BM, true, 2, false, 1, true><<<dim3(grid), dim3(256), 0, st>>>(p);
        else bneck_kernel<64, BM, true, 2, false><<<dim3(grid), dim3(256), 0, st>>>(p);
    } else if (planes == 64) {
        if (t11) bneck_kernel<64, BM, true, 0, false, 1, true><<<dim3(grid), dim3(256), 0, st>>>(p);
        else if (t1n) bneck_kernel<64, BM, true, 0, false><<<dim3(grid), dim3(256), 0, st>>>(p);
        else bneck_kernel<64, BM, false, 0, false><<<dim3(grid), dim3(256), 0, st>>>(p);
    } else {
        if (t1n) {
            if (patch) bneck_kernel<128, BM, true, 0, true><<<dim3(grid), dim3(256), 0, st>>>(p);
            else bneck_kernel<128, BM, true, 0, false><<<dim3(grid), dim3(256), 0, st>>>(p);
        } else {
            if (patch) bneck_kernel<128, BM, false, 0, true><<<dim3(grid), dim3(256), 0, st>>>(p);
            else bneck_kernel<128, BM, false, 0, false><<<dim3(grid), dim3(256), 0, st>>>(p);
        }
    }
    if (ev1) (void)hipEventRecord(ev1, st);
    CHECK_LAUNCH(ctx, "bneck");
    ctx->gemm_launches += 1;
    ctx->gemm_flops += 2.0 * (double)M * planes * (planes * (9.0 + 4.0 + (t1n ? 4.0 : 0.0)) + 4.0 * ds_cin);
    return AVCER_OK;
}

int launch_bneck_tail(avcer_ctx* ctx, int planes, long M, const void* t2, const void* x, void* out, void* t1n, const void* w3,
                      const float* b3, const void* w1n, const float* b1n, hipStream_t st) {
    if (!t2 || !x || !out || !t1n || !w3 || !b3 || !w1n || !b1n || M <= 0) return set_err(ctx, AVCER_EINVAL, "bneck_tail: bad arguments");
    if (planes != 256) return set_err(ctx, AVCER_EINVAL, "bneck_tail: planes %d (256)", planes);
    if (M * 4096L >= (1L << 32) - 4096) return set_err(ctx, AVCER_EINVAL, "bneck_tail: M=%ld exceeds the 4 GiB descriptor range", M);
    BneckParams p;
    memset(&p, 0, sizeof(p));
    p.T1 = (const char*)t2; p.X = (const char*)x; p.OUT = (char*)out; p.T1N = (char*)t1n;
    p.W3 = (const char*)w3; p.W1N = (const char*)w1n; p.b3 = b3; p.b1n = b1n;
    p.M = (int)M; p.ovf = ctx->ovf;
    hipEvent_t ev0 = nullptr, ev1 = nullptr;
    TRY(prof_begin(ctx, st, &ev0, &ev1, FAM_TAIL, 2.0 * (double)M * planes * planes * 8.0, 4.0 * (double)M * planes * 10.0, M, 4 * planes, planes));
    p.t1_bytes = (unsigned)(M * 4096L);
    bneck_tail2_kernel<256><<<dim3((int)((M + 127) / 128)), dim3(512), 0, st>>>(p);
    if (ev1) (void)hipEventRecord(ev1, st);
    CHECK_LAUNCH(ctx, "bneck_tail");
    ctx->gemm_launches += 1;
    ctx->gemm_flops += 2.0 * (double)M * planes * planes * 8.0;
    return AVCER_OK;
}

int measure_ceilings(avcer_ctx* ctx, double* mfma_bf16_tflops, double* hbm_copy_tbs, hipStream_t st) {
    hipEvent_t e0, e1;
    HIP_TRY(ctx, hipEventCreate(&e0));
    HIP_TRY(ctx, hipEventCreate(&e1));
    void* buf = nullptr;
    const size_t bytes = (size_t)1 << 30;
    TRY(ws_reserve(ctx, WS_CEILINGS, 2 * bytes, &buf));
    float ms = 0.f;
    const int blocks = 256 * 2, iters = 20000;
    mfma_rate_kernel<<<blocks, 256, 0, st>>>((float*)buf, 2000);
    HIP_TRY(ctx, hipEventRecord(e0, st));
    mfma_rate_kernel<<<blocks, 256, 0, st>>>((float*)buf, iters);
    HIP_TRY(ctx, hipEventRecord(e1, st));
    HIP_TRY(ctx, hipEventSynchronize(e1));
    HIP_TRY(ctx, hipEventElapsedTime(&ms, e0, e1));
    if (mfma_bf16_tflops) *mfma_bf16_tflops = (double)blocks * 4 * iters * 16 * (2.0 * 16 * 16 * 32) / (ms * 1e-3) / 1e12;
    HIP_TRY(ctx, hipMemsetAsync(buf, 1, bytes, st));
    const int cgrid = (int)(bytes / 16 / 256);
    copy16_kernel<<<cgrid, 256, 0, st>>>((const uint4*)buf, (uint4*)((char*)buf + bytes), bytes / 16);
    HIP_TRY(ctx, hipEventRecord(e0, st));
    for (int i = 0; i < 4; ++i) copy16_kernel<<<cgrid, 256, 0, st>>>((const uint4*)buf, (uint4*)((char*)buf + bytes), bytes / 16);
    HIP_TRY(ctx, hipEventRecord(e1, st));
    HIP_TRY(ctx, hipEventSynchronize(e1));
    HIP_TRY(ctx, hipEventElapsedTime(&ms, e0, e1));
    if (hbm_copy_tbs) *hbm_copy_tbs = 4.0 * 2.0 * (double)bytes / (ms * 1e-3) / 1e12;
    (void)hipEventDestroy(e0);
    (void)hipEventDestroy(e1);
    hipError_t e = hipGetLastError();
    if (e != hipSuccess) return set_err(ctx, AVCER_EHIP, "measure_ceilings: %s", hipGetErrorString(e));
    return AVCER_OK;
}
```

avcer_amd/csrc/gemm.hip:

```cpp
#include "common.h"
#include "gemm_dev.h"

#include <type_traits>

namespace {

struct GemmParams {
    const char* X;
    const char* W;
    const float* scale;
    const float* bias;
    const char* R;
    char* Y;
    unsigned x_bytes, w_bytes;
    const char* X2;
    unsigned x2_bytes;
    int K1;
    long sB2, sH2, sW2;
    int coff2, st2;
    int M, N, K;
    int OH, OW, H, Wd, Cin, KW;
    int sh, sw, ph, pw, dh, dw;
    long sB, sH, sW;
    int coff;
    long ldY;
    int yoff;
    long ldR;
    int roff;
    int act, res_after;
    int ntn, ntm, nwg;
    int gm;
    int groups;
    int KH;
    int fast;
    int tile_n;
    int tile_m;
    int tap_inner;
    const char* WF;
    int tapH4, tapW4;
    int slots;
    int rsub, rH, rW;
    unsigned* ovf;
};

template <int OUT>
__device__ __forceinline__ void res_load(const GemmParams& p, long m, int n0, uint4& r0, uint4& r1) {
    if (p.rsub > 1) {
        const int ohw = p.OH * p.OW;
        const int b = (int)(m / ohw), rem = (int)m - b * ohw;
        const int oy = rem / p.OW, ox = rem - oy * p.OW;
        m = ((long)b * p.rH + (long)oy * p.rsub) * p.rW + (long)ox * p.rsub;
    }
    const long e = m * p.ldR + p.roff + n0;
    if constexpr (OUT == 0) {
        const char* rp = p.R + e * 4;
        r0 = *reinterpret_cast<const uint4*>(rp);
        r1 = *reinterpret_cast<const uint4*>(rp + 16);
    } else if constexpr (OUT == 1) {
        r0 = *reinterpret_cast<const uint4*>(p.R + e * 2);
        r1 = make_uint4(0u, 0u, 0u, 0u);
    } else {
        const char* rp = p.R + sp32_byte(e);
        r0 = *reinterpret_cast<const uint4*>(rp);
        r1 = *reinterpret_cast<const uint4*>(rp + 64);
    }
}

template <int OUT, int ACT>
__device__ __forceinline__ void finish8(const GemmParams& p, long m, int n0, const float4 a, const float4 b, const uint4 r0,
                                        const uint4 r1, sp_flags_t& ovm) {
#pragma clang fp contract(off)
    float v[8] = {a.x, a.y, a.z, a.w, b.x, b.y, b.z, b.w};
    float r[8];
    if constexpr (OUT == 0) {
        r[0] = __builtin_bit_cast(float, r0.x); r[1] = __builtin_bit_cast(float, r0.y);
        r[2] = __builtin_bit_cast(float, r0.z); r[3] = __builtin_bit_cast(float, r0.w);
        r[4] = __builtin_bit_cast(float, r1.x); r[5] = __builtin_bit_cast(float, r1.y);
        r[6] = __builtin_bit_cast(float, r1.z); r[7] = __builtin_bit_cast(float, r1.w);
    } else if constexpr (OUT == 1) {
        const uint32_t w[4] = {r0.x, r0.y, r0.z, r0.w};
#pragma unroll
        for (int j = 0; j < 4; ++j) { r[2 * j] = bf2f((bf16_t)(w[j] & 0xffff)); r[2 * j + 1] = bf2f((bf16_t)(w[j] >> 16)); }
    } else {
        sp_join8(r0, r1, r);
    }
#pragma unroll
    for (int j = 0; j < 8; ++j) {
        float x = p.res_after ? v[j] : v[j] + r[j];
        if constexpr (ACT == 1) x = relu_nan(x);
        if constexpr (ACT == 2) x = gelu_erf(x);
        if constexpr (ACT == 3) x = gelu_fast(x);
        v[j] = p.res_after ? x + r[j] : x;
    }
    const long e = m * p.ldY + p.yoff + n0;
    if constexpr (OUT == 0) {
        char* yp = p.Y + e * 4;
        *reinterpret_cast<float4*>(yp) = make_float4(v[0], v[1], v[2], v[3]);
        *reinterpret_cast<float4*>(yp + 16) = make_float4(v[4], v[5], v[6], v[7]);
    } else if constexpr (OUT == 1) {
        uint4 t;
        t.x = (uint32_t)f2bf(v[0]) | ((uint32_t)f2bf(v[1]) << 16);
        t.y = (uint32_t)f2bf(v[2]) | ((uint32_t)f2bf(v[3]) << 16);
        t.z = (uint32_t)f2bf(v[4]) | ((uint32_t)f2bf(v[5]) << 16);
        t.w = (uint32_t)f2bf(v[6]) | ((uint32_t)f2bf(v[7]) << 16);
        *reinterpret_cast<uint4*>(p.Y + e * 2) = t;
    } else {
        float amax = 0.f;
        uint4 h, l;
        sp_split8(v, amax, h, l);
        sp_flag(ovm, amax);
        char* yp = p.Y + sp32_byte(e);
        *reinterpret_cast<uint4*>(yp) = h;
        *reinterpret_cast<uint4*>(yp + 64) = l;
    }
}

template <int BN>
__device__ __forceinline__ int stage_off(int row, int chunk) { return row * (BN * 4) + ((chunk ^ (row & 7)) << 4); }

template <int MODE, int BN, typename AccT, int NFN, int NFM>
__device__ __forceinline__ void stage_acc(const GemmParams& p, char* smem, AccT (&acc)[NFN][NFM], int n_base, int row0, int wn,
                                          int lane) {
    constexpr int WN = BN / 2;
    if constexpr (MODE == 0) {
#pragma unroll
        for (int fn = 0; fn < NFN; ++fn)
#pragma unroll
            for (int g = 0; g < 4; ++g) {
                const int nl = wn * WN + fn * 32 + 8 * g + 4 * (lane >> 5);
                float4 sc = make_float4(1.f, 1.f, 1.f, 1.f), bi = make_float4(0.f, 0.f, 0.f, 0.f);
                if (p.scale) sc = *reinterpret_cast<const float4*>(p.scale + n_base + nl);
                if (p.bias) bi = *reinterpret_cast<const float4*>(p.bias + n_base + nl);
#pragma unroll
                for (int fm = 0; fm < NFM; ++fm) {
                    const int ml = row0 + fm * 32 + (lane & 31);
                    *reinterpret_cast<float4*>(smem + stage_off<BN>(ml, nl >> 2)) =
                        make_float4(acc[fn][fm][4 * g + 0] * sc.x + bi.x, acc[fn][fm][4 * g + 1] * sc.y + bi.y,
                                    acc[fn][fm][4 * g + 2] * sc.z + bi.z, acc[fn][fm][4 * g + 3] * sc.w + bi.w);
                }
            }
    } else {
#pragma unroll
        for (int fn = 0; fn < NFN; ++fn) {
            const int nl = wn * WN + fn * 16 + 4 * (lane >> 4);
            float4 sc = make_float4(1.f, 1.f, 1.f, 1.f), bi = make_float4(0.f, 0.f, 0.f, 0.f);
            if (p.scale) sc = *reinterpret_cast<const float4*>(p.scale + n_base + nl);
            if (p.bias) bi = *reinterpret_cast<const float4*>(p.bias + n_base + nl);
#pragma unroll
            for (int fm = 0; fm < NFM; ++fm) {
                const int ml = row0 + fm * 16 + (lane & 15);
                *reinterpret_cast<float4*>(smem + stage_off<BN>(ml, nl >> 2)) =
                    make_float4(acc[fn][fm][0] * sc.x + bi.x, acc[fn][fm][1] * sc.y + bi.y, acc[fn][fm][2] * sc.z + bi.z,
                                acc[fn][fm][3] * sc.w + bi.w);
            }
        }
    }
}

template <int BMT, int BN> struct DrainMap {
    static constexpr int EP_ROWS = BMT;
    static constexpr int TPR = BN / 8;
    static constexpr int RPP = 256 / TPR;
    static constexpr int NP = EP_ROWS / RPP;
};

template <int OUT, int BMT, int BN>
__device__ __forceinline__ void res_prefetch(const GemmParams& p, int m_base, int n_base, int tid,
                                             uint4 (&rr)[DrainMap<BMT, BN>::NP][2]) {
    using D = DrainMap<BMT, BN>;
    const int c8 = tid % D::TPR, r0 = tid / D::TPR;
#pragma unroll
    for (int pass = 0; pass < D::NP; ++pass) {
        const long m = (long)m_base + pass * D::RPP + r0;
        rr[pass][0] = make_uint4(0u, 0u, 0u, 0u);
        rr[pass][1] = make_uint4(0u, 0u, 0u, 0u);
        if (p.R && m < p.M) res_load<OUT>(p, m, n_base + c8 * 8, rr[pass][0], rr[pass][1]);
    }
}

template <int OUT, int BMT, int BN, int ACT>
__device__ __forceinline__ void drain_stage(const GemmParams& p, const char* smem, int m_base, int n_base, int tid,
                                            const uint4 (&rr)[DrainMap<BMT, BN>::NP][2]) {
    using D = DrainMap<BMT, BN>;
    const int c8 = tid % D::TPR, r0 = tid / D::TPR;
#pragma unroll
    for (int pass = 0; pass < D::NP; ++pass) {
        const int row = pass * D::RPP + r0;
        const long m = (long)m_base + row;
        if (m < p.M) {
            const float4 a = *reinterpret_cast<const float4*>(smem + stage_off<BN>(row, 2 * c8));
            const float4 b = *reinterpret_cast<const float4*>(smem + stage_off<BN>(row, 2 * c8 + 1));
            sp_flags_t unused = 0;
            finish8<OUT, ACT>(p, m, n_base + c8 * 8, a, b, rr[pass][0], rr[pass][1], unused);
        }
    }
}

template <int OUT, int NFN, int NFM>
__device__ __forceinline__ void res_prefetch_direct(const GemmParams& p, int m0, int c0, int lane, uint4 (&rr)[NFN / 2][NFM][2]) {
#pragma unroll
    for (int j = 0; j < NFN / 2; ++j)
#pragma unroll
        for (int fm = 0; fm < NFM; ++fm) {
            rr[j][fm][0] = make_uint4(0u, 0u, 0u, 0u);
            rr[j][fm][1] = make_uint4(0u, 0u, 0u, 0u);
            const long m = (long)m0 + fm * 16 + (lane & 15);
            if (p.R && m < p.M) res_load<OUT>(p, m, c0 + 32 * j + 8 * (lane >> 4), rr[j][fm][0], rr[j][fm][1]);
        }
}

__device__ __forceinline__ float4 scale_bias4(const f32x4_t a, const float4 s, const float4 b) {
    return make_float4(__builtin_fmaf(a[0], s.x, b.x), __builtin_fmaf(a[1], s.y, b.y), __builtin_fmaf(a[2], s.z, b.z),
                       __builtin_fmaf(a[3], s.w, b.w));
}

template <int OUT, int ACT, int NFN, int NFM>
__device__ __forceinline__ void epilogue_direct(const GemmParams& p, f32x4_t (&acc)[NFN][NFM], int m0, int c0, int lane,
                                                const uint4 (&rr)[NFN / 2][NFM][2], const float wmul, sp_flags_t& ovm) {
#pragma unroll
    for (int j = 0; j < NFN / 2; ++j) {
        const int ch = c0 + 32 * j + 8 * (lane >> 4);
        float4 s0 = make_float4(1.f, 1.f, 1.f, 1.f), s1 = s0, b0 = make_float4(0.f, 0.f, 0.f, 0.f), b1 = b0;
        if (p.scale) { s0 = *reinterpret_cast<const float4*>(p.scale + ch); s1 = *reinterpret_cast<const float4*>(p.scale + ch + 4); }
        if (p.bias) { b0 = *reinterpret_cast<const float4*>(p.bias + ch); b1 = *reinterpret_cast<const float4*>(p.bias + ch + 4); }
        s0 = make_float4(s0.x * wmul, s0.y * wmul, s0.z * wmul, s0.w * wmul);
        s1 = make_float4(s1.x * wmul, s1.y * wmul, s1.z * wmul, s1.w * wmul);
#pragma unroll
        for (int fm = 0; fm < NFM; ++fm) {
            const long m = (long)m0 + fm * 16 + (lane & 15);
            if (m >= p.M) continue;
            const f32x4_t lo = acc[2 * j][fm], hi = acc[2 * j + 1][fm];
            finish8<OUT, ACT>(p, m, ch, scale_bias4(lo, s0, b0), scale_bias4(hi, s1, b1), rr[j][fm][0], rr[j][fm][1], ovm);
        }
    }
}

template <int MODE, int BMT, int BN, int TILE_BYTES, typename AccT, int NFN, int NFM>
__device__ __forceinline__ void mfma_step(const GemmParams& p, const char* smem, int cur, AccT (&acc)[NFN][NFM], int wm, int wn,
                                      int lane, sp_flags_t& ovm) {
    constexpr bool IS_F32 = MODE == 0;
    constexpr int WN = BN / 2;
    constexpr int WM = BMT / 2;
    const char* sa = smem + cur * TILE_BYTES;
    const char* sb = sa + BMT * ROWB;
    if constexpr (IS_F32) {
#pragma unroll
        for (int kq = 0; kq < 4; ++kq) {
            const int ch = kq * 2 + (lane >> 5);
            float4 af[NFM], wf[NFN];
#pragma unroll
            for (int fm = 0; fm < NFM; ++fm)
                af[fm] = *reinterpret_cast<const float4*>(sa + swz(wm * WM + fm * 32 + (lane & 31), ch));
#pragma unroll
            for (int fn = 0; fn < NFN; ++fn)
                wf[fn] = *reinterpret_cast<const float4*>(sb + swz(wn * WN + fn * 32 + (lane & 31), ch));
#pragma unroll
            for (int fn = 0; fn < NFN; ++fn)
#pragma unroll
                for (int fm = 0; fm < NFM; ++fm) {
                    acc[fn][fm] = __builtin_amdgcn_mfma_f32_32x32x2f32(wf[fn].x, af[fm].x, acc[fn][fm], 0, 0, 0);
                    acc[fn][fm] = __builtin_amdgcn_mfma_f32_32x32x2f32(wf[fn].y, af[fm].y, acc[fn][fm], 0, 0, 0);
                    acc[fn][fm] = __builtin_amdgcn_mfma_f32_32x32x2f32(wf[fn].z, af[fm].z, acc[fn][fm], 0, 0, 0);
                    acc[fn][fm] = __builtin_amdgcn_mfma_f32_32x32x2f32(wf[fn].w, af[fm].w, acc[fn][fm], 0, 0, 0);
                }
        }
    } else if constexpr (MODE == 2 || MODE == 3) {
        const int g = lane >> 4;
        spx8_t ahi[NFM], alo[NFM];
#pragma unroll
        for (int fm = 0; fm < NFM; ++fm) {
            const int row = wm * WM + fm * 16 + (lane & 15);
            if constexpr (MODE == 3) {
                ahi[fm] = *reinterpret_cast<const spx8_t*>(sa + swz(row, g));
                alo[fm] = *reinterpret_cast<const spx8_t*>(sa + swz(row, 4 + g));
                continue;
            }
            const float4 x = *reinterpret_cast<const float4*>(sa + swz(row, 2 * g));
            const float4 y = *reinterpret_cast<const float4*>(sa + swz(row, 2 * g + 1));
            const float v[8] = {x.x, x.y, x.z, x.w, y.x, y.y, y.z, y.w};
            sp_split8(v, ahi[fm], alo[fm], ovm);
        }
#pragma unroll
        for (int fn = 0; fn < NFN; ++fn) {
            const int row = wn * WN + fn * 16 + (lane & 15);
            const spx8_t whi = *reinterpret_cast<const spx8_t*>(sb + swz(row, g));
            const spx8_t wlo = *reinterpret_cast<const spx8_t*>(sb + swz(row, 4 + g));
#pragma unroll
            for (int fm = 0; fm < NFM; ++fm) {
                acc[fn][fm] = mfma_sp(wlo, ahi[fm], acc[fn][fm]);
                acc[fn][fm] = mfma_sp(whi, alo[fm], acc[fn][fm]);
                acc[fn][fm] = mfma_sp(whi, ahi[fm], acc[fn][fm]);
            }
        }
    } else {
#pragma unroll
        for (int ks = 0; ks < 2; ++ks) {
            const int ch = ks * 4 + (lane >> 4);
            bf16x8_t af[NFM], wf[NFN];
#pragma unroll
            for (int fm = 0; fm < NFM; ++fm)
                af[fm] = *reinterpret_cast<const bf16x8_t*>(sa + swz(wm * WM + fm * 16 + (lane & 15), ch));
#pragma unroll
            for (int fn = 0; fn < NFN; ++fn)
                wf[fn] = *reinterpret_cast<const bf16x8_t*>(sb + swz(wn * WN + fn * 16 + (lane & 15), ch));
#pragma unroll
            for (int fn = 0; fn < NFN; ++fn)
#pragma unroll
                for (int fm = 0; fm < NFM; ++fm)
                    acc[fn][fm] = __builtin_amdgcn_mfma_f32_16x16x32_bf16(wf[fn], af[fm], acc[fn][fm], 0, 0, 0);
        }
    }
}

template <int MODE, int OUT, int BN>
__global__ void __launch_bounds__(256, 2) conv_gemm_kernel(const GemmParams p) {
    constexpr int BMT = 128;
    constexpr bool IS_F32 = MODE == 0;
    constexpr int ES = MODE == 1 ? 2 : 4;
    constexpr int VEC = 16 / ES;
    constexpr int BK = ROWB / ES;
    constexpr int TILE_BYTES = (BMT + BN) * ROWB;
    constexpr int WN = BN / 2;
    constexpr int WM = BMT / 2;
    __shared__ __attribute__((aligned(16))) char smem[2 * TILE_BYTES];

    const int tid = threadIdx.x;
    const int lane = tid & 63;
    const int wave = __builtin_amdgcn_readfirstlane(tid >> 6);
    const int wm = (wave >> 1) & 1, wn = wave & 1;
    const int dw = wave;

    int bid = blockIdx.x;
    {
        const int q = p.nwg >> 3, r = p.nwg & 7;
        const int xcd = bid & 7, idx = bid >> 3;
        bid = (xcd < r ? xcd * (q + 1) : r * (q + 1) + (xcd - r) * q) + idx;
    }
    int tile_n, tile_m;
    if (p.gm > 1) {
        const int per_group = p.gm * p.ntn;
        const int group = bid / per_group, within = bid - group * per_group;
        const int first_m = group * p.gm;
        const int gsize = min(p.gm, p.ntm - first_m);
        tile_m = first_m + within % gsize;
        tile_n = within / gsize;
    } else {
        tile_n = bid % p.ntn;
        tile_m = bid / p.ntn;
    }
    const int m_base = tile_m * BMT;
    const int grp = blockIdx.y;
    const int n_base = grp * p.N + tile_n * BN;
    const int x_coff = p.coff + grp * p.Cin;

    const auto xrs = __builtin_amdgcn_make_buffer_rsrc(const_cast<char*>(p.X), (short)0, (int)p.x_bytes, 0x00020000);
    const auto wrs = __builtin_amdgcn_make_buffer_rsrc(const_cast<char*>(p.W), (short)0, (int)p.w_bytes, 0x00020000);
    const auto x2rs = __builtin_amdgcn_make_buffer_rsrc(const_cast<char*>(p.X2 ? p.X2 : p.X), (short)0,
                                                        (int)(p.X2 ? p.x2_bytes : p.x_bytes), 0x00020000);

    constexpr int A_ISS = BMT / 8 / 4;
    constexpr int B_ISS = BN / 8 / 4;
    const int lrow8 = lane >> 3;
    const int slot = lane & 7;
#define AVCER_DMA_SETUP()                                                                                           \
    unsigned a_off[A_ISS];                                                                                          \
    unsigned a_off2[A_ISS];                                                                                         \
// ... 765 lines not shown
```

avcer_amd/csrc/gemm_dev.h:

```cpp
#pragma once

#include "act_io.h"

typedef __attribute__((ext_vector_type(8))) __bf16 bf16x8_t;
typedef __attribute__((ext_vector_type(4))) float f32x4_t;
typedef __attribute__((ext_vector_type(16))) float f32x16_t;

namespace {

constexpr int ROWB = 128;

typedef __attribute__((ext_vector_type(4))) unsigned int u32x4_t;
typedef __attribute__((ext_vector_type(2))) unsigned int u32x2_t;
constexpr unsigned OOB = 0xFFFFFF00u;

template <typename Rsrc>
__device__ __forceinline__ void dma16(Rsrc rs, char* lds_wave_base, unsigned voff, unsigned soff = 0u) {
#if defined(__HIP_DEVICE_COMPILE__)
    __builtin_amdgcn_raw_ptr_buffer_load_lds(rs, (__attribute__((address_space(3))) void*)lds_wave_base, 16, voff, soff, 0, 0);
#endif
}

__device__ __forceinline__ int swz_key(int row) { return (int)((0x32765410u >> (((row >> 1) & 7) * 4)) & 7u); }
__device__ __forceinline__ int swz(int row, int chunk) { return row * ROWB + ((chunk ^ swz_key(row)) << 4); }

__device__ __forceinline__ float gelu_erf(float x) {
#pragma clang fp contract(off)
    return 0.5f * x * (1.0f + erff(x * 0.70710678118654752440f));
}

__device__ __forceinline__ float gelu_fast(float x) {
#pragma clang fp contract(off)
    const float z = x * 0.70710678118654752440f, a = __builtin_fabsf(z);
    const float t = __builtin_amdgcn_rcpf(__builtin_fmaf(0.3275911f, a, 1.0f));
    float p = __builtin_fmaf(1.061405429f, t, -1.453152027f);
    p = __builtin_fmaf(p, t, 1.421413741f);
    p = __builtin_fmaf(p, t, -0.284496736f);
    p = __builtin_fmaf(p, t, 0.254829592f);
    p *= t;
    const float e = __builtin_amdgcn_exp2f(-1.4426950408889634f * a * a);
    const float erfz = __builtin_copysignf(__builtin_fmaf(-p, e, 1.0f), z);
    return 0.5f * x * (1.0f + erfz);
}

}
```

avcer_amd/engine.py:

```python
from __future__ import annotations

import ctypes as C
import weakref

import numpy as np
import torch

from . import _lib, packing
from ._lib import SPLIT_TRAILER, AvcerError, ConvDesc
from .jpeg import DESC as _JPEG_DESC

MODE_FP32 = 0
MODE_BF16 = 1
MODE_F16X3 = 2
MODE_DEFAULT = MODE_F16X3
PAD_MODES = {"mean": 0, "constant": 1, "repeat": 2}
_JPEG_DESC_BYTES = _JPEG_DESC.itemsize


def _ptr(t):
    return None if t is None else C.c_void_p(t.data_ptr())


def _pack_detections(dets_per_frame):
# ... 658 lines not shown

    def conv_gemm(self, desc: ConvDesc, dtype: int, x, w, scale, bias, residual, y):
        self._check(self.lib.avcer_conv_gemm(self.ctx, C.byref(desc), dtype, _ptr(x), _ptr(w), _ptr(scale), _ptr(bias),
                                             _ptr(residual), _ptr(y), self._stream()))

    def profile_enable(self, on: bool = True):
        self._check(self.lib.avcer_profile_enable(self.ctx, int(on)))

    def profile_read(self):
        ms, n = C.c_double(0.0), C.c_int64(0)
        self._check(self.lib.avcer_profile_read(self.ctx, C.byref(ms), C.byref(n)))
        return ms.value, n.value

    FAMILIES = ("conv_gemm_kernel", "conv_gemm_wd_kernel", "bneck_kernel", "bneck_tail2_kernel", "stem_pool_kernel",
                "conv_gemm_skinny_kernel", "gru_layer_kernel")

    def profile_read_families(self):
        n = len(self.FAMILIES)
        ms, fl, by = (C.c_double * n)(), (C.c_double * n)(), (C.c_double * n)()
        la = (C.c_int64 * n)()
        self._check(self.lib.avcer_profile_read_families(self.ctx, n, ms, la, fl, by))
        return {name: (ms[i], int(la[i]), fl[i], by[i]) for i, name in enumerate(self.FAMILIES)}

    def profile_read_launches(self, max_n: int = 8192):
        fam = np.zeros(max_n, np.int32)
        ms, fl, by = np.zeros(max_n), np.zeros(max_n), np.zeros(max_n)
        mnk = np.zeros((max_n, 3), np.int64)
        n = C.c_int64(0)
        vp = lambda a: a.ctypes.data_as(C.c_void_p)
        self._check(self.lib.avcer_profile_read_launches(self.ctx, max_n, vp(fam), vp(ms), vp(fl), vp(by), vp(mnk), C.byref(n)))
        k = min(int(n.value), max_n)
        return [dict(family=self.FAMILIES[fam[i]], ms=float(ms[i]), flops=float(fl[i]), bytes=float(by[i]), m=int(mnk[i, 0]),
                     n=int(mnk[i, 1]), k=int(mnk[i, 2])) for i in range(k)]

    def debug_tap(self, name: str, numel: int, dtype=torch.float32):
        dst = torch.zeros(numel, dtype=dtype, device=self.device)
        self._tap_keepalive = dst
        self._check(self.lib.avcer_debug_tap(self.ctx, name.encode(), _ptr(dst), dst.numel() * dst.element_size()))
        return dst

    def debug_tap_copied(self) -> int:
        return int(self.lib.avcer_debug_tap_copied(self.ctx))

    def split_weights(self, w):
        w = self._dev(w, torch.float32)
        out = torch.empty(w.numel() * 2, dtype=torch.int16, device=self.device)
        self._check(self.lib.avcer_split_weights(self.ctx, _ptr(w), _ptr(out), w.numel(), self._stream()))
        return out

    def split_weight_rows(self, w):
        w = self._dev(w, torch.float32)
        if w.dim() != 2:
            raise ValueError("split_weight_rows: w [N,K]")
        out = torch.empty(w.numel() * 2 + SPLIT_TRAILER // 2, dtype=torch.int16, device=self.device)
        self._check(self.lib.avcer_split_weight_rows(self.ctx, _ptr(w), _ptr(out), int(w.shape[0]), int(w.shape[1]), self._stream()))
        return out

    def weight_frags(self, w):
        w = self._dev(w, torch.float32)
        rows = self.split_weight_rows(w)
        out = torch.empty_like(rows)
        self._check(self.lib.avcer_weight_frags(self.ctx, _ptr(rows), _ptr(out), int(w.shape[0]), int(w.shape[1]), self._stream()))
        return out

    def conv_gemm_dual(self, desc: ConvDesc, dtype: int, x, x2, w, scale, bias, residual, y):
        self._check(self.lib.avcer_conv_gemm_dual(self.ctx, C.byref(desc), dtype, _ptr(x), _ptr(x2), _ptr(w), _ptr(scale),
                                                  _ptr(bias), _ptr(residual), _ptr(y), self._stream()))

    def bneck_chain(self, planes: int, nb: int, h: int, w: int, t1, x, out, t1n, w2, b2, w3, b3, w1n=None, b1n=None, ds_cin: int = 0,
                    out_step: int = 1, w2_frags=None):
        self._check(self.lib.avcer_bneck_chain(self.ctx, planes, nb, h, w, _ptr(t1), _ptr(x), int(ds_cin), int(out_step), _ptr(out),
                                               _ptr(t1n), _ptr(w2), _ptr(b2), _ptr(w3), _ptr(b3), _ptr(w1n), _ptr(b1n),
                                               _ptr(w2_frags), self._stream()))

    def bneck_tail(self, planes: int, m: int, t2, x, out, t1n, w3, b3, w1n, b1n):
        self._check(self.lib.avcer_bneck_tail(self.ctx, int(planes), int(m), _ptr(t2), _ptr(x), _ptr(out), _ptr(t1n), _ptr(w3),
                                              _ptr(b3), _ptr(w1n), _ptr(b1n), self._stream()))

    def dwsep(self, x, dw_w, dw_s, dw_b, pw_w, pw_s, pw_b, stride: int, mode: int = MODE_FP32):
        x = self._dev(x, torch.float32)
        nb, h, w, cin = (int(v) for v in x.shape)
        pw = self._dev(pw_w, torch.float32)
        cout = int(pw.shape[0])
        pad = torch.zeros((cout + 63) // 64 * 64, (cin + 31) // 32 * 32, dtype=torch.float32, device=self.device)
        pad[:cout, :cin] = pw
        wdev = self.split_weight_rows(pad) if mode == MODE_F16X3 else pad
        args = [self._dev(t, torch.float32) for t in (dw_w, dw_s, dw_b, pw_s, pw_b)]
        y = self._new(nb, (h - 1) // stride + 1, (w - 1) // stride + 1, cout)
        self._check(self.lib.avcer_dwsep(self.ctx, cin, cout, int(stride), int(mode), nb, h, w, _ptr(x), _ptr(args[0]), _ptr(args[1]),
                                         _ptr(args[2]), _ptr(wdev), _ptr(args[3]), _ptr(args[4]), _ptr(y), self._stream()))
        return y

    def s3fd_stem(self, frames_u8, wt, bias, rgb: bool = False, sp32: bool = False):
        x = self._dev(frames_u8, torch.uint8)
        n, h, w = (int(v) for v in x.shape[:3])
        wt, bias = self._dev(wt, torch.float32), self._dev(bias, torch.float32)
        y = self._new(n, h, w, 128, dtype=torch.int16) if sp32 else self._new(n, h, w, 64)
        self._check(self.lib.avcer_s3fd_stem(self.ctx, _ptr(x), n, h, w, 1 if rgb else 0, _ptr(wt), _ptr(bias), _ptr(y), 2 if sp32 else 0,
                                             self._stream()))
        return y

    def maxpool2(self, x, ceil_mode: bool = False, sp32: bool = False):
        x = self._dev(x, torch.int16 if sp32 else torch.float32)
        n, h, w = (int(v) for v in x.shape[:3])
        c = int(x.shape[3]) // (2 if sp32 else 1)
        oh, ow = ((h + 1) // 2, (w + 1) // 2) if ceil_mode else (h // 2, w // 2)
        if oh < 1 or ow < 1:
            raise ValueError(f"maxpool2: a {h} x {w} map has no 2 x 2 window")
        y = torch.empty(n, oh, ow, int(x.shape[3]), dtype=x.dtype, device=self.device)
        self._check(self.lib.avcer_maxpool2(self.ctx, _ptr(x), _ptr(y), n, h, w, c, int(ceil_mode), 2 if sp32 else 0, self._stream()))
        return y

    def s3fd_head(self, x, wt, bias, l2norm: bool, sp32: bool = False):
        x = self._dev(x, torch.int16 if sp32 else torch.float32)
        nb, h, w = (int(v) for v in x.shape[:3])
        c = int(x.shape[3]) // (2 if sp32 else 1)
        wt, bias = self._dev(wt, torch.float32), self._dev(bias, torch.float32)
        loc, conf = self._new(nb, h * w, 4), self._new(nb, h * w, 2)
        inv = self._new(nb * h * w) if l2norm else None
        self._check(self.lib.avcer_s3fd_head(self.ctx, _ptr(x), 2 if sp32 else 0, _ptr(inv), _ptr(wt), _ptr(bias), nb, h, w, c,
                                             int(wt.shape[2]), 0, h * w, _ptr(loc), _ptr(conf), self._stream()))
        return loc, conf

    def attention(self, qkv, out, n: int, s: int, heads: int, head_dim: int, scale: float, in_kind: int, out_kind: int):
        self._check(self.lib.avcer_attention(self.ctx, _ptr(qkv), _ptr(out), n, s, heads, head_dim, float(scale), in_kind,
                                             out_kind, self._stream()))

    def attention_long(self, qkv, out, n: int, s: int, heads: int, head_dim: int, scale: float, in_kind: int, out_kind: int):
        self._check(self.lib.avcer_attention_long(self.ctx, _ptr(qkv), _ptr(out), n, s, heads, head_dim, float(scale), in_kind,
                                                  out_kind, self._stream()))

    def measure_ceilings(self):
        a, b = C.c_double(0.0), C.c_double(0.0)
        self._check(self.lib.avcer_measure_ceilings(self.ctx, C.byref(a), C.byref(b), self._stream()))
        return a.value, b.value

    def stem_pool(self, planes_hi_lo, w_split, scale, bias, n: int):
        planes = self._dev(planes_hi_lo, torch.int16)
        if tuple(planes.shape) != (2, n, 230, 230, 4):
            raise ValueError("stem_pool: planes [2, n, 230, 230, 4] int16 (fp16 bits)")
        y = torch.empty(n, 55, 55, 128, dtype=torch.int16, device=self.device)
        self._check(self.lib.avcer_stem_pool(self.ctx, _ptr(planes), n * 230 * 230 * 4 * 2, _ptr(w_split), _ptr(scale), _ptr(bias),
                                             _ptr(y), n, self._stream()))
        return y

    def stem_pool_u8(self, frames_u8, w_split, scale, shifts9):
        fr = self._dev(frames_u8, torch.uint8)
        n, h, w = int(fr.shape[0]), int(fr.shape[1]), int(fr.shape[2])
        y = torch.empty(n, 55, 55, 128, dtype=torch.int16, device=self.device)
        self._check(self.lib.avcer_stem_pool_u8(self.ctx, _ptr(fr), n, h, w, _ptr(w_split), _ptr(scale), _ptr(shifts9), _ptr(y),
                                                self._stream()))
        return y

    def gemm_stats(self, reset: bool = True):
        n, f = C.c_int64(0), C.c_double(0.0)
        self._check(self.lib.avcer_gemm_stats(self.ctx, C.byref(n), C.byref(f), int(reset)))
        return n.value, f.value
```

include/avcer_hip.h:

```cpp
#ifndef AVCER_HIP_H
#define AVCER_HIP_H

#include <stddef.h>
#include <stdint.h>

#ifdef __cplusplus
extern "C" {
#endif

typedef struct avcer_ctx avcer_ctx;
typedef void* avcer_stream_t;

enum {
    AVCER_OK = 0,
    AVCER_EINVAL = -1,
    AVCER_ENOMEM = -2,
    AVCER_EHIP = -3,
    AVCER_ESTATE = -4,
    AVCER_EFORMAT = -5
};

enum {
    AVCER_MODE_FP32 = 0,
    AVCER_MODE_BF16 = 1,
// ... 89 lines not shown

int avcer_static_forward_cam(avcer_ctx* ctx, const uint8_t* frames, int n, int in_h, int in_w, int mode, float* logits, float* probs,
                             float* feats, float* cam, avcer_stream_t stream);
int avcer_crop_resize_linear(avcer_ctx* ctx, const uint8_t* frames, int n_frames, int h, int w, const int32_t* rects, int n,
                             int swap_rb, int out_h, int out_w, uint8_t* out, avcer_stream_t stream);
int avcer_cam_render(avcer_ctx* ctx, const float* cam, const int32_t* rows, const int32_t* cls, const uint8_t* base_rgb, int n,
                     const uint8_t* lut_bgr, double image_weight, uint8_t* out_bgr, avcer_stream_t stream);

enum { AVCER_DRAW_OUTLINE = 0, AVCER_DRAW_FILL = 1, AVCER_DRAW_MASK = 2 };
typedef struct avcer_draw_item {
    int32_t frame;
    int32_t kind;
    int32_t x0, y0;
    int32_t x1, y1;
    int32_t arg;
    int32_t mask;
    int32_t colour[3];
    int32_t pad;
} avcer_draw_item;
int avcer_annotate_frames(avcer_ctx* ctx, uint8_t* frames, int n, int h, int w, const avcer_draw_item* items, int m, const uint8_t* masks,
                          int64_t masks_bytes, const int32_t* table, int n_masks, const int32_t* work, int n_work, int64_t n_tiles,
                          avcer_stream_t stream);

int avcer_track_faces(avcer_ctx* ctx, const float* dets_host, int ld, const int32_t* counts_host, int n_frames, int frame_w,
                      int frame_h, double iou_threshold, double minimum_face_size, int64_t* records_host, int64_t* n_records);
int avcer_lsap(int nr, int nc, const double* cost_host, int32_t* rows_host, int32_t* cols_host);

typedef struct avcer_tracker avcer_tracker;
avcer_tracker* avcer_tracker_create(double iou_threshold, double minimum_face_size);
int avcer_tracker_push(avcer_tracker* tracker, const float* dets_host, int ld, const int32_t* counts_host, int n_frames,
                       int64_t first_frame, int frame_w, int frame_h, int64_t* records_host, int64_t* n_records);
const char* avcer_tracker_last_error(const avcer_tracker* tracker);
void avcer_tracker_destroy(avcer_tracker* tracker);

enum { AVCER_JPEG_OK = 0, AVCER_JPEG_NOT_HANDLED = 1 };
typedef struct avcer_jpeg_desc {
    int32_t status, reason;
    int32_t width, height, ncomp;
    int32_t hs, vs;
    int32_t bw[3], bh[3];
    int32_t tq[3];
    int64_t coef_block, n_blocks;
    uint16_t qt[3][64];
} avcer_jpeg_desc;
int avcer_jpeg_probe(const uint8_t* bytes_host, size_t len, avcer_jpeg_desc* info_host);
int avcer_jpeg_entropy_batch(avcer_ctx* ctx, const uint8_t* const* files_host, const int64_t* lens_host, int n, int16_t* coeffs_host,
                             int64_t cap_blocks, avcer_jpeg_desc* desc_host, int threads, int64_t* blocks_needed);
int avcer_jpeg_tiles(avcer_ctx* ctx, const int16_t* coeffs, int64_t n_blocks, const avcer_jpeg_desc* desc, int n, int32_t* flags,
                     uint8_t* tiles, avcer_stream_t stream);
int avcer_jpeg_rgb(avcer_ctx* ctx, const int16_t* coeffs, int64_t n_blocks, const avcer_jpeg_desc* desc, int n, int32_t* flags,
                   uint8_t* canvas, int hmax, int wmax, avcer_stream_t stream);

#define AVCER_JPEG_STD_TABLES 1
int avcer_jpeg_entropy_batch_ex(avcer_ctx* ctx, const uint8_t* const* files_host, const int64_t* lens_host, int n, int16_t* coeffs_host,
                                int64_t cap_blocks, avcer_jpeg_desc* desc_host, int threads, int hflags, int64_t* blocks_needed);
int avcer_jpeg_frames(avcer_ctx* ctx, const int16_t* coeffs, int64_t n_blocks, const avcer_jpeg_desc* desc, int n, int32_t* flags,
                      uint8_t* frames, int H, int W, int bgr, avcer_stream_t stream);

int avcer_jpeg_quant_tables(int quality, uint16_t qt[2][64]);
int avcer_jpeg_plan(const int32_t* sizes_host, int n, int subsampling, int quality, avcer_jpeg_desc* desc_host, int64_t* blocks_needed);
int avcer_jpeg_forward(avcer_ctx* ctx, const uint8_t* src, int N, int H, int W, const int32_t* rects, const avcer_jpeg_desc* desc, int n,
                       int bgr, int16_t* coeffs, int64_t n_blocks, avcer_stream_t stream);
int avcer_jpeg_write_batch(avcer_ctx* ctx, const int16_t* coeffs_host, avcer_jpeg_desc* desc_host, int n, uint8_t* out_host,
                           int64_t cap_bytes, int64_t* offsets_host, int threads, int64_t* bytes_needed);

int avcer_jpeg_pack(avcer_ctx* ctx, const int16_t* coeffs, int64_t n_blocks, const avcer_jpeg_desc* desc, int n, uint8_t* out,
                    int64_t cap_bytes, int64_t* offsets, int32_t* status, int64_t* bytes_needed, avcer_stream_t stream);

int avcer_jpeg_roundtrip_tiles(avcer_ctx* ctx, const uint8_t* src, int N, int H, int W, const int32_t* rects, const avcer_jpeg_desc* desc,
                               int n, int bgr, int16_t* coeffs_or_null, int64_t n_blocks, int32_t* flags, uint8_t* tiles,
                               avcer_stream_t stream);
int avcer_jpeg_roundtrip_rgb(avcer_ctx* ctx, const uint8_t* src, int N, int H, int W, const int32_t* rects, const avcer_jpeg_desc* desc,
                             int n, int bgr, int16_t* coeffs_or_null, int64_t n_blocks, int32_t* flags, uint8_t* canvas, int hmax,
                             int wmax, avcer_stream_t stream);

typedef struct avcer_jpeg_tab {
    uint8_t bits[17];
    uint8_t vals[256];
    uint8_t pad[15];
} avcer_jpeg_tab;
typedef struct avcer_jpeg_scan {
    int64_t offset, nbytes;
    int32_t restart;
    int32_t dc[3], ac[3];
    int32_t pad;
} avcer_jpeg_scan;
int avcer_jpeg_scan_batch(avcer_ctx* ctx, const uint8_t* const* files_host, const int64_t* lens_host, int n, uint8_t* bytes_host,
                          int64_t cap_bytes, avcer_jpeg_desc* desc_host, avcer_jpeg_scan* scan_host, avcer_jpeg_tab* tabs_host, int cap_tabs,
                          int threads, int32_t* n_tabs, int64_t* bytes_needed, int64_t* blocks_needed);
int avcer_jpeg_scan_batch_ex(avcer_ctx* ctx, const uint8_t* const* files_host, const int64_t* lens_host, int n, uint8_t* bytes_host,
                             int64_t cap_bytes, avcer_jpeg_desc* desc_host, avcer_jpeg_scan* scan_host, avcer_jpeg_tab* tabs_host,
                             int cap_tabs, int threads, int hflags, int32_t* n_tabs, int64_t* bytes_needed, int64_t* blocks_needed);
int avcer_jpeg_unpack(avcer_ctx* ctx, const uint8_t* bytes, int64_t n_bytes, const avcer_jpeg_scan* scan, const avcer_jpeg_tab* tabs,
                      int n_tabs, avcer_jpeg_desc* desc, int n, int16_t* coeffs, int64_t n_blocks, int32_t* status, int sub_bits,
                      avcer_stream_t stream);
int avcer_jpeg_unpack_host(avcer_ctx* ctx, const uint8_t* bytes_host, int64_t n_bytes, const avcer_jpeg_scan* scan_host,
                           const avcer_jpeg_tab* tabs_host, int n_tabs, avcer_jpeg_desc* desc_host, int n, int16_t* coeffs_host,
                           int64_t n_blocks, int32_t* status_host, int sub_bits);

int avcer_fuse(avcer_ctx* ctx, const float* stat, const float* dyn_logits, const float* aud_mean, int n, int n_aud,
               int aud_c, const double* w1_host, const double* w2_host, int ce_weights_type, int ce_mask,
               double* comp_prob, int32_t* comp_argmax, avcer_stream_t stream);

int avcer_fuse_videos(avcer_ctx* ctx, const float* stat, const float* dyn_logits, const float* win_logits,
                      const int32_t* frame_lo, const int32_t* frame_hi, const int32_t* frame_off, const int32_t* win_off,
                      const int32_t* n_aud, int n_videos, int64_t n_frames, int64_t n_windows, int c, const double* w1_host,
                      const double* w2_host, int ce_weights_type, int ce_mask, float* aud_mean, int32_t* count,
                      double* comp_prob, int32_t* comp_argmax, avcer_stream_t stream);

typedef struct avcer_conv_desc {
    int32_t batch, in_h, in_w;
    int32_t out_h, out_w;
    int32_t cin;
    int32_t kh, kw;
    int32_t stride_h, stride_w, pad_h, pad_w, dil_h, dil_w;
    int64_t x_stride_b, x_stride_h, x_stride_w;
    int32_t x_coff;
    int32_t n;
    int64_t y_ld; int32_t y_coff;
    int64_t r_ld; int32_t r_coff;
    int32_t act;
    int32_t res_after_act;
    int32_t groups;
    int32_t x2_cin, x2_coff, x2_stride;
    int64_t x2_stride_b, x2_stride_h, x2_stride_w;
    int32_t tile_n;
    int32_t r_sub, r_h, r_w;
    int32_t tile_m;
} avcer_conv_desc;

int avcer_conv_gemm(avcer_ctx* ctx, const avcer_conv_desc* d, int dtype, const void* x, const void* w,
                    const float* scale, const float* bias, const void* residual, void* y, avcer_stream_t stream);

int avcer_conv_gemm_dual(avcer_ctx* ctx, const avcer_conv_desc* d, int dtype, const void* x, const void* x2, const void* w,
                         const float* scale, const float* bias, const void* residual, void* y, avcer_stream_t stream);

int avcer_bneck_chain(avcer_ctx* ctx, int planes, int nb, int h, int w, const void* t1, const void* x, int ds_cin, int out_step,
                      void* out, void* t1n, const void* w2, const float* b2, const void* w3, const float* b3, const void* w1n,
                      const float* b1n, const void* w2_frags, avcer_stream_t stream);
int avcer_bneck_tail(avcer_ctx* ctx, int planes, int64_t M, const void* t2, const void* x, void* out, void* t1n, const void* w3,
                     const float* b3, const void* w1n, const float* b1n, avcer_stream_t stream);
int avcer_dwsep(avcer_ctx* ctx, int cin, int cout, int stride, int mode, int nb, int h, int w, const float* x, const float* dw_w,
                const float* dw_s, const float* dw_b, const void* pw_w, const float* pw_s, const float* pw_b, float* y,
                avcer_stream_t stream);
int avcer_s3fd_stem(avcer_ctx* ctx, const uint8_t* frames, int n, int h, int w, int rgb, const float* wt, const float* bias, void* y,
                    int kind, avcer_stream_t stream);
int avcer_maxpool2(avcer_ctx* ctx, const void* x, void* y, int n, int h, int w, int c, int ceil_mode, int kind, avcer_stream_t stream);
int avcer_s3fd_head(avcer_ctx* ctx, const void* x, int kind, float* inv_norm, const float* wt, const float* bias, int nb, int h, int w,
                    int c, int n_out, int row0, int n_priors, float* loc, float* conf, avcer_stream_t stream);
int avcer_stem_pool(avcer_ctx* ctx, const void* planes_hi_lo, size_t plane_bytes, const void* w, const float* scale,
                    const float* bias, void* y, int n, avcer_stream_t stream);
int avcer_stem_pool_u8(avcer_ctx* ctx, const uint8_t* frames, int n, int in_h, int in_w, const void* w, const float* scale,
                       const float* shifts9, void* y, avcer_stream_t stream);

int avcer_split_weights(avcer_ctx* ctx, const float* w, void* out, size_t numel, avcer_stream_t stream);

#define AVCER_SPLIT_TRAILER 256

int avcer_split_weight_rows(avcer_ctx* ctx, const float* w, void* out, int n, int k, avcer_stream_t stream);

int avcer_weight_frags(avcer_ctx* ctx, const void* rows, void* out, int n, int k, avcer_stream_t stream);

int avcer_gru_layer(avcer_ctx* ctx, const float* xp, const float* w_hh, const float* b_hh, int n, int s, int h, int mode,
                    float* h_seq, avcer_stream_t stream);

int avcer_attention(avcer_ctx* ctx, const void* qkv, void* out, int n, int s, int heads, int head_dim, float scale,
                    int in_kind, int out_kind, avcer_stream_t stream);
#define AVCER_ATT_LONG_KT 128
#define AVCER_ATT_LONG_QB 128
int avcer_attention_long(avcer_ctx* ctx, const void* qkv, void* out, int n, int s, int heads, int head_dim, float scale,
                         int in_kind, int out_kind, avcer_stream_t stream);

int avcer_measure_ceilings(avcer_ctx* ctx, double* mfma16_tflops, double* hbm_copy_tbs, avcer_stream_t stream);

int avcer_gemm_stats(avcer_ctx* ctx, int64_t* launches, double* flops, int reset);

int avcer_profile_enable(avcer_ctx* ctx, int on);
int avcer_profile_read(avcer_ctx* ctx, double* total_ms, int64_t* launches);
enum {
    AVCER_FAM_GEMM = 0,
    AVCER_FAM_GEMM_WD = 1,
    AVCER_FAM_CHAIN = 2,
    AVCER_FAM_TAIL = 3,
    AVCER_FAM_STEM = 4,
    AVCER_FAM_SKINNY = 5,
    AVCER_FAM_GRU = 6,
    AVCER_FAM_COUNT = 7
};
int avcer_profile_read_families(avcer_ctx* ctx, int n_fam, double* ms, int64_t* launches, double* flops, double* bytes);
int avcer_profile_read_launches(avcer_ctx* ctx, int64_t max_n, int32_t* fam, double* ms, double* flops, double* bytes, int64_t* mnk,
                                int64_t* n);

int avcer_debug_tap(avcer_ctx* ctx, const char* name, void* dst_dev, size_t bytes);
int64_t avcer_debug_tap_copied(const avcer_ctx* ctx);

#ifdef __cplusplus
}
#endif
#endif
```

Baseline: 2191.

## Fuse layer1.0 conv1 1x1 GEMM into the u8 stem+maxpool kernel

The u8 stem+pool kernel now optionally runs layer1.0's 1x1 conv (64->64) on each pooled tile while it is still in LDS. It writes T1 directly with MFMA on split hi/lo fragments, and the bottleneck stage skips the separate conv1 GEMM launch when the stem already produced it. This removes one kernel launch and one re-read of the stem output from global memory. In exchange the stem kernel needs more LDS, extra registers for the weight fragments and accumulators, and a barrier after every half, which may lower occupancy. GemmParams and finish8 move to a shared header so the stem kernel can reuse them.

```diff
diff --git a/avcer_amd/_lib.py b/avcer_amd/_lib.py
--- a/avcer_amd/_lib.py
+++ b/avcer_amd/_lib.py
@@ -150,6 +150,7 @@
     "avcer_stem_pool": (C.c_int, [c_ctx, C.c_void_p, C.c_size_t, C.c_void_p, C.c_void_p, C.c_void_p, C.c_void_p, C.c_int, c_stream]),
     "avcer_stem_pool_u8": (C.c_int, [c_ctx, C.c_void_p, C.c_int, C.c_int, C.c_int, C.c_void_p, C.c_void_p, C.c_void_p, C.c_void_p,
                                      c_stream]),
+    "avcer_stem_pool_u8_conv1": (C.c_int, [c_ctx, C.c_void_p, C.c_int, C.c_int, C.c_int] + [C.c_void_p] * 8 + [c_stream]),
     "avcer_attention_long": (C.c_int, [c_ctx, C.c_void_p, C.c_void_p, C.c_int, C.c_int, C.c_int, C.c_int, C.c_float, C.c_int, C.c_int,
                                        c_stream]),
     "avcer_set_audio_max_tokens": (C.c_int, [c_ctx, C.c_int]),
diff --git a/avcer_amd/csrc/api.hip b/avcer_amd/csrc/api.hip
--- a/avcer_amd/csrc/api.hip
+++ b/avcer_amd/csrc/api.hip
@@ -437,6 +437,7 @@
     bool stride_last;
     bool w2_frags;
     const char* tap;
+    bool c1_done = false;
 };
 
 static void run_bneck_stage(Net& net, Trunk& t, int li, int b_begin, int b_end, int nb, void* last_out, const std::string& end_tap) {
@@ -454,7 +455,7 @@
                           pn = "l" + std::to_string(li + 1) + "." + std::to_string(b + 1) + ".";
         void* dst = (b == b_end - 1 && last_out) ? last_out : (t.X == t.pp[0] ? t.pp[1] : t.pp[0]);
         const bool fused = net.x3 && li < 3 && b >= fused_from, chain = fused && li < 2, next = b + 1 < blocks;
-        if (!fused || b == fused_from)
+        if ((!fused || b == fused_from) && !(t.c1_done && li == 0 && b == 0))
             net.gemm(conv2d_desc(nb, h, w, t.cin, 1, 1, 1, 0, planes, 1), p + "c1.w", net.F(p + "c1.s"), net.F(p + "c1.b"), t.X,
                      nullptr, t.T1, act, act);
         if (chain) {
@@ -572,21 +573,25 @@
         feat_ws = ar.get<float>((size_t)NS * 512 * 4);
         if (cam) cam_g = ar.get<float>((size_t)std::min(NS, kCamChunk) * 7 * 2048 * 4);
     }));
-    auto run_stem = [&](int f0, int nb, void** B) {
+    auto run_stem = [&](int f0, int nb, void** B) -> bool {
         if (net.x3) {
             const Tensor* w = net.T("stem7.w");
-            if (net.err != AVCER_OK) return;
-            if (!w->x3) { net.err = set_err(ctx, AVCER_ESTATE, "stem7.w: split weights not prepared"); return; }
+            if (net.err != AVCER_OK) return false;
+            if (!w->x3) { net.err = set_err(ctx, AVCER_ESTATE, "stem7.w: split weights not prepared"); return false; }
             if (frames) {
+                const Tensor* w1 = net.T("l1.0.c1.w");
+                if (net.err != AVCER_OK) return false;
+                if (!w1->x3f) { net.err = set_err(ctx, AVCER_ESTATE, "l1.0.c1.w: split weights not prepared"); return false; }
                 net.chk(launch_stem_pool_u8(ctx, frames + (size_t)f0 * in_h * in_w * 3, in_h, in_w, w->x3, net.F("stem.s"),
-                                            net.F("stem.b9"), B[1], nb, st));
+                                            net.F("stem.b9"), B[1], nb, st, w1->x3f, net.F("l1.0.c1.s"), net.F("l1.0.c1.b"), B[2]));
                 net.tap("stem", B[1], (size_t)nb * 55 * 55 * 64 * es);
-                return;
+                net.tap("out:l1.0.c1.w", B[2], (size_t)nb * 55 * 55 * 64 * es);
+                return net.err == AVCER_OK;
             }
             net.chk(k_pack_nchw(ctx, nchw + (size_t)f0 * 3 * 224 * 224, nb, P, 3, st));
             net.chk(launch_stem_pool(ctx, P, (size_t)nb * 230 * 230 * 4 * 2, w->x3, net.F("stem.s"), net.F("stem.b"), B[1], nb, st));
             net.tap("stem", B[1], (size_t)nb * 55 * 55 * 64 * es);
-            return;
+            return false;
         }
         if (frames) net.chk(k_preprocess(ctx, frames + (size_t)f0 * in_h * in_w * 3, nb, in_h, in_w, P, bf, st));
         else net.chk(k_pack_nchw(ctx, nchw + (size_t)f0 * 3 * 224 * 224, nb, P, bf, st));
@@ -595,13 +600,14 @@
         net.tap("stem_conv", B[0], (size_t)nb * 112 * 112 * 64 * es);
         net.chk(k_maxpool(ctx, B[0], B[1], nb, 112, 112, 64, 3, 0, 55, 55, act, st));
         net.tap("stem", B[1], (size_t)nb * 55 * 55 * 64 * es);
+        return false;
     };
     for (int s0 = 0; s0 < n; s0 += NS) {
         const int nb = std::min(NS, n - s0);
         for (int c0 = 0; c0 < nb; c0 += NB) {
             const int cn = std::min(NB, nb - c0);
             Trunk t{buf[1], {buf[0], buf[1]}, buf[2], buf[3], 55, 55, 64, true, true, ""};
-            run_stem(s0 + c0, cn, buf);
+            t.c1_done = run_stem(s0 + c0, cn, buf);
             run_bneck_stage(net, t, 0, 0, kStages[0][1], cn, nullptr, "layer1");
             run_bneck_stage(net, t, 1, 0, 1, cn, (char*)bbuf[0] + (size_t)c0 * 28 * 28 * 512 * es, "layer2");
         }
@@ -1587,6 +1593,15 @@
     return launch_stem_pool_u8(ctx, frames, in_h, in_w, w, scale, shifts9, y, n, (hipStream_t)stream);
 }
 
+extern "C" int avcer_stem_pool_u8_conv1(avcer_ctx* ctx, const uint8_t* frames, int n, int in_h, int in_w, const void* w, const float* scale,
+                                        const float* shifts9, void* y, const void* w1_frags, const float* scale1, const float* bias1,
+                                        void* t1, avcer_stream_t stream) {
+    if (!ctx) return AVCER_EINVAL;
+    if (!t1) return set_err(ctx, AVCER_EINVAL, "stem_pool_u8_conv1: null t1");
+    HIP_TRY(ctx, hipSetDevice(ctx->device));
+    return launch_stem_pool_u8(ctx, frames, in_h, in_w, w, scale, shifts9, y, n, (hipStream_t)stream, w1_frags, scale1, bias1, t1);
+}
+
 extern "C" int avcer_split_weights(avcer_ctx* ctx, const float* w, void* out, size_t numel, avcer_stream_t stream) {
     if (!ctx) return AVCER_EINVAL;
     if (!w || !out || numel % 32) return set_err(ctx, AVCER_EINVAL, "split_weights: numel must be a multiple of 32");
diff --git a/avcer_amd/csrc/common.h b/avcer_amd/csrc/common.h
--- a/avcer_amd/csrc/common.h
+++ b/avcer_amd/csrc/common.h
@@ -146,7 +146,8 @@
 int launch_stem_pool(avcer_ctx* ctx, const void* planes, size_t plane_bytes, const void* w_x3, const float* scale,
                      const float* bias, void* y, int n, hipStream_t st);
 int launch_stem_pool_u8(avcer_ctx* ctx, const uint8_t* frames, int in_h, int in_w, const void* w_x3, const float* scale,
-                        const float* bias9, void* y, int n, hipStream_t st);
+                        const float* bias9, void* y, int n, hipStream_t st, const void* w1_frags = nullptr,
+                        const float* scale1 = nullptr, const float* bias1 = nullptr, void* t1 = nullptr);
 int launch_stem_pool_face(avcer_ctx* ctx, const uint8_t* frames, int h, int w, int rgb, const void* w_x3, const float* scale,
                           const float* bias, void* y, int n, hipStream_t st);
 int launch_bneck(avcer_ctx* ctx, int planes, int nb, int h, int w, const void* t1, const void* x, int ds_cin, int out_step,
diff --git a/avcer_amd/csrc/fused.hip b/avcer_amd/csrc/fused.hip
--- a/avcer_amd/csrc/fused.hip
+++ b/avcer_amd/csrc/fused.hip
@@ -54,6 +54,10 @@
     unsigned* ovf;
     int oh, ow, mh, mw, tiles_y, tiles_x, swap_rb;
     int mean[3];
+    const char* W1F;
+    const float* s1;
+    const float* b1;
+    char* T1;
 };
 
 constexpr int ST_TH = 8, ST_TW = 7;
@@ -184,15 +188,18 @@
     sp_commit(p.ovf, ovm);
 }
 
-template <bool FACE>
+template <bool FACE, bool C1 = false>
 __global__ void __launch_bounds__(256, 3) stem_pool_u8_kernel(const StemParams p) {
+    static_assert(!(FACE && C1), "layer1.0.conv1 follows the recognition CNN's stem only");
     constexpr int NK = 7, WRING = 3;
     constexpr int PROWS = 2 * (ST_RH - 1) + NK, PCH = (2 * (ST_RW - 1) + 8) / 2;
     constexpr int NCH = PROWS * PCH;
     constexpr int WOFF = ((NCH * 16 + 1023) / 1024) * 1024;
     constexpr int WT = 64 * ROWB;
     constexpr int IMG = 256 * 128;
-    constexpr int LDS_BYTES = WOFF + WRING * WT > IMG ? WOFF + WRING * WT : IMG;
+    constexpr int C1B = IMG;
+    constexpr int LDS_BYTES = C1 ? C1B + 64 * ROWB : (WOFF + WRING * WT > IMG ? WOFF + WRING * WT : IMG);
+    static_assert(WOFF + WRING * WT <= LDS_BYTES, "patch + weight ring");
     __shared__ __attribute__((aligned(16))) char smem[LDS_BYTES];
     const int tid = threadIdx.x, lane = tid & 63;
     const int wave = __builtin_amdgcn_readfirstlane(tid >> 6);
@@ -302,6 +309,27 @@
         asm volatile("" ::: "memory");
     }
 #undef AVCER_STEM_W
+    const int c1j = wave & 1, c1p = wave >> 1;
+    spx8_t c1w[2][2][2];
+    f32x4_t c1acc[2][2];
+    float4 c1s[2], c1b[2];
+    if constexpr (C1) {
+#pragma unroll
+        for (int ks = 0; ks < 2; ++ks)
+#pragma unroll
+            for (int t = 0; t < 2; ++t) {
+                const char* f = p.W1F + (((2 * c1j + t) * 2 + ks) * 2) * 1024 + lane * 16;
+                c1w[ks][t][0] = *reinterpret_cast<const spx8_t*>(f);
+                c1w[ks][t][1] = *reinterpret_cast<const spx8_t*>(f + 1024);
+            }
+#pragma unroll
+        for (int t = 0; t < 2; ++t) {
+            c1s[t] = *reinterpret_cast<const float4*>(p.s1 + 32 * c1j + 8 * g + 4 * t);
+            c1b[t] = *reinterpret_cast<const float4*>(p.b1 + 32 * c1j + 8 * g + 4 * t);
+#pragma unroll
+            for (int fm = 0; fm < 2; ++fm) c1acc[t][fm] = f32x4_t{0};
+        }
+    }
     sp_flags_t ovm = 0;
 #pragma unroll
     for (int half = 0; half < 2; ++half) {
@@ -357,9 +385,42 @@
                 char* yp = p.Y + sp32_byte(e);
                 *reinterpret_cast<spx8_t*>(yp) = hi;
                 *reinterpret_cast<spx8_t*>(yp + 64) = lo;
-            }
-        }
-        if (half == 0) __syncthreads();
+                if constexpr (C1) {
+                    *reinterpret_cast<spx8_t*>(smem + C1B + swz(pp, c8)) = hi;
+                    *reinterpret_cast<spx8_t*>(smem + C1B + swz(pp, 4 + c8)) = lo;
+                }
+            }
+        }
+        if (half == 0 || C1) __syncthreads();
+        if constexpr (C1) {
+            spx8_t bh[2], bl[2];
+#pragma unroll
+            for (int fm = 0; fm < 2; ++fm) {
+                bh[fm] = ldfrag(smem + C1B, (2 * c1p + fm) * 16 + l15, g);
+                bl[fm] = ldfrag(smem + C1B, (2 * c1p + fm) * 16 + l15, 4 + g);
+            }
+#pragma unroll
+            for (int t = 0; t < 2; ++t)
+#pragma unroll
+                for (int fm = 0; fm < 2; ++fm) mfma3(c1acc[t][fm], c1w[half][t][0], c1w[half][t][1], bh[fm], bl[fm]);
+        }
+    }
+    if constexpr (C1) {
+        GemmParams gp = {};
+        gp.Y = p.T1; gp.ldY = 64;
+        const float w1mul = split_wmul(p.W1F, 64 * 64 * 4);
+        const float4 s0 = make_float4(c1s[0].x * w1mul, c1s[0].y * w1mul, c1s[0].z * w1mul, c1s[0].w * w1mul);
+        const float4 s1 = make_float4(c1s[1].x * w1mul, c1s[1].y * w1mul, c1s[1].z * w1mul, c1s[1].w * w1mul);
+        const uint4 none = make_uint4(0u, 0u, 0u, 0u);
+#pragma unroll
+        for (int fm = 0; fm < 2; ++fm) {
+            const int pp = (2 * c1p + fm) * 16 + l15;
+            const int ppy = pp / ST_TW, ppx = pp - ppy * ST_TW;
+            const int py = ST_TH * ty + ppy, px = ST_TW * tx + ppx;
+            if (pp < ST_TH * ST_TW && py < 55 && px < 55)
+                finish8<2, 1>(gp, ((long)b * 55 + py) * 55 + px, 32 * c1j + 8 * g, scale_bias4(c1acc[0][fm], s0, c1b[0]),
+                              scale_bias4(c1acc[1][fm], s1, c1b[1]), none, none, ovm);
+        }
     }
     sp_commit(p.ovf, ovm);
 }
@@ -1051,20 +1112,26 @@
 }
 
 int launch_stem_pool_u8(avcer_ctx* ctx, const uint8_t* frames, int in_h, int in_w, const void* w_x3, const float* scale,
-                        const float* bias9, void* y, int n, hipStream_t st) {
+                        const float* bias9, void* y, int n, hipStream_t st, const void* w1_frags, const float* scale1,
+                        const float* bias1, void* t1) {
     if (!frames || !w_x3 || !scale || !bias9 || !y || n <= 0 || in_h <= 0 || in_w <= 0)
         return set_err(ctx, AVCER_EINVAL, "stem_pool_u8: bad arguments");
+    if (t1 && (!w1_frags || !scale1 || !bias1)) return set_err(ctx, AVCER_EINVAL, "stem_pool_u8: a conv1 output needs its weights, scale and bias");
     StemParams p;
     memset(&p, 0, sizeof(p));
     p.F = frames; p.in_h = in_h; p.in_w = in_w; p.bias9 = bias9;
     p.W = (const char*)w_x3; p.scale = scale; p.Y = (char*)y; p.n = n; p.ovf = ctx->ovf;
+    p.W1F = (const char*)w1_frags; p.s1 = scale1; p.b1 = bias1; p.T1 = (char*)t1;
+    const double flops = 2.0 * n * 112.0 * 112.0 * 64 * 147 + (t1 ? 2.0 * n * 55.0 * 55 * 64 * 64 : 0.0);
+    const double bytes = (double)n * ((double)in_h * in_w * 3 + 55.0 * 55 * 64 * 4) + (t1 ? (double)n * 55.0 * 55 * 64 * 4 + 64.0 * 64 * 4 : 0.0);
     hipEvent_t ev0 = nullptr, ev1 = nullptr;
-    TRY(prof_begin(ctx, st, &ev0, &ev1, FAM_STEM, 2.0 * n * 112.0 * 112.0 * 64 * 147, (double)n * ((double)in_h * in_w * 3 + 55.0 * 55 * 64 * 4)));
-    stem_pool_u8_kernel<false><<<dim3(n * ST_TY * ST_TX), dim3(256), 0, st>>>(p);
+    TRY(prof_begin(ctx, st, &ev0, &ev1, FAM_STEM, flops, bytes));
+    if (t1) stem_pool_u8_kernel<false, true><<<dim3(n * ST_TY * ST_TX), dim3(256), 0, st>>>(p);
+    else stem_pool_u8_kernel<false><<<dim3(n * ST_TY * ST_TX), dim3(256), 0, st>>>(p);
     if (ev1) (void)hipEventRecord(ev1, st);
     CHECK_LAUNCH(ctx, "stem_pool_u8");
     ctx->gemm_launches += 1;
-    ctx->gemm_flops += 2.0 * n * 112.0 * 112.0 * 64 * 147;
+    ctx->gemm_flops += flops;
     return AVCER_OK;
 }
 
diff --git a/avcer_amd/csrc/gemm.hip b/avcer_amd/csrc/gemm.hip
--- a/avcer_amd/csrc/gemm.hip
+++ b/avcer_amd/csrc/gemm.hip
@@ -4,44 +4,6 @@
 #include <type_traits>
 
 namespace {
-
-struct GemmParams {
-    const char* X;
-    const char* W;
-    const float* scale;
-    const float* bias;
-    const char* R;
-    char* Y;
-    unsigned x_bytes, w_bytes;
-    const char* X2;
-    unsigned x2_bytes;
-    int K1;
-    long sB2, sH2, sW2;
-    int coff2, st2;
-    int M, N, K;
-    int OH, OW, H, Wd, Cin, KW;
-    int sh, sw, ph, pw, dh, dw;
-    long sB, sH, sW;
-    int coff;
-    long ldY;
-    int yoff;
-    long ldR;
-    int roff;
-    int act, res_after;
-    int ntn, ntm, nwg;
-    int gm;
-    int groups;
-    int KH;
-    int fast;
-    int tile_n;
-    int tile_m;
-    int tap_inner;
-    const char* WF;
-    int tapH4, tapW4;
-    int slots;
-    int rsub, rH, rW;
-    unsigned* ovf;
-};
 
 template <int OUT>
 __device__ __forceinline__ void res_load(const GemmParams& p, long m, int n0, uint4& r0, uint4& r1) {
@@ -66,55 +28,6 @@
     }
 }
 
-template <int OUT, int ACT>
-__device__ __forceinline__ void finish8(const GemmParams& p, long m, int n0, const float4 a, const float4 b, const uint4 r0,
-                                        const uint4 r1, sp_flags_t& ovm) {
-#pragma clang fp contract(off)
-    float v[8] = {a.x, a.y, a.z, a.w, b.x, b.y, b.z, b.w};
-    float r[8];
-    if constexpr (OUT == 0) {
-        r[0] = __builtin_bit_cast(float, r0.x); r[1] = __builtin_bit_cast(float, r0.y);
-        r[2] = __builtin_bit_cast(float, r0.z); r[3] = __builtin_bit_cast(float, r0.w);
-        r[4] = __builtin_bit_cast(float, r1.x); r[5] = __builtin_bit_cast(float, r1.y);
-        r[6] = __builtin_bit_cast(float, r1.z); r[7] = __builtin_bit_cast(float, r1.w);
-    } else if constexpr (OUT == 1) {
-        const uint32_t w[4] = {r0.x, r0.y, r0.z, r0.w};
-#pragma unroll
-        for (int j = 0; j < 4; ++j) { r[2 * j] = bf2f((bf16_t)(w[j] & 0xffff)); r[2 * j + 1] = bf2f((bf16_t)(w[j] >> 16)); }
-    } else {
-        sp_join8(r0, r1, r);
-    }
-#pragma unroll
-    for (int j = 0; j < 8; ++j) {
-        float x = p.res_after ? v[j] : v[j] + r[j];
-        if constexpr (ACT == 1) x = relu_nan(x);
-        if constexpr (ACT == 2) x = gelu_erf(x);
-        if constexpr (ACT == 3) x = gelu_fast(x);
-        v[j] = p.res_after ? x + r[j] : x;
-    }
-    const long e = m * p.ldY + p.yoff + n0;
-    if constexpr (OUT == 0) {
-        char* yp = p.Y + e * 4;
-        *reinterpret_cast<float4*>(yp) = make_float4(v[0], v[1], v[2], v[3]);
-        *reinterpret_cast<float4*>(yp + 16) = make_float4(v[4], v[5], v[6], v[7]);
-    } else if constexpr (OUT == 1) {
-        uint4 t;
-        t.x = (uint32_t)f2bf(v[0]) | ((uint32_t)f2bf(v[1]) << 16);
-        t.y = (uint32_t)f2bf(v[2]) | ((uint32_t)f2bf(v[3]) << 16);
-        t.z = (uint32_t)f2bf(v[4]) | ((uint32_t)f2bf(v[5]) << 16);
-        t.w = (uint32_t)f2bf(v[6]) | ((uint32_t)f2bf(v[7]) << 16);
-        *reinterpret_cast<uint4*>(p.Y + e * 2) = t;
-    } else {
-        float amax = 0.f;
-        uint4 h, l;
-        sp_split8(v, amax, h, l);
-        sp_flag(ovm, amax);
-        char* yp = p.Y + sp32_byte(e);
-        *reinterpret_cast<uint4*>(yp) = h;
-        *reinterpret_cast<uint4*>(yp + 64) = l;
-    }
-}
-
 template <int BN>
 __device__ __forceinline__ int stage_off(int row, int chunk) { return row * (BN * 4) + ((chunk ^ (row & 7)) << 4); }
 
@@ -207,11 +120,6 @@
             const long m = (long)m0 + fm * 16 + (lane & 15);
             if (p.R && m < p.M) res_load<OUT>(p, m, c0 + 32 * j + 8 * (lane >> 4), rr[j][fm][0], rr[j][fm][1]);
         }
-}
-
-__device__ __forceinline__ float4 scale_bias4(const f32x4_t a, const float4 s, const float4 b) {
-    return make_float4(__builtin_fmaf(a[0], s.x, b.x), __builtin_fmaf(a[1], s.y, b.y), __builtin_fmaf(a[2], s.z, b.z),
-                       __builtin_fmaf(a[3], s.w, b.w));
 }
 
 template <int OUT, int ACT, int NFN, int NFM>
diff --git a/avcer_amd/csrc/gemm_dev.h b/avcer_amd/csrc/gemm_dev.h
--- a/avcer_amd/csrc/gemm_dev.h
+++ b/avcer_amd/csrc/gemm_dev.h
@@ -43,4 +43,96 @@
     return 0.5f * x * (1.0f + erfz);
 }
 
+struct GemmParams {
+    const char* X;
+    const char* W;
+    const float* scale;
+    const float* bias;
+    const char* R;
+    char* Y;
+    unsigned x_bytes, w_bytes;
+    const char* X2;
+    unsigned x2_bytes;
+    int K1;
+    long sB2, sH2, sW2;
+    int coff2, st2;
+    int M, N, K;
+    int OH, OW, H, Wd, Cin, KW;
+    int sh, sw, ph, pw, dh, dw;
+    long sB, sH, sW;
+    int coff;
+    long ldY;
+    int yoff;
+    long ldR;
+    int roff;
+    int act, res_after;
+    int ntn, ntm, nwg;
+    int gm;
+    int groups;
+    int KH;
+    int fast;
+    int tile_n;
+    int tile_m;
+    int tap_inner;
+    const char* WF;
+    int tapH4, tapW4;
+    int slots;
+    int rsub, rH, rW;
+    unsigned* ovf;
+};
+
+__device__ __forceinline__ float4 scale_bias4(const f32x4_t a, const float4 s, const float4 b) {
+    return make_float4(__builtin_fmaf(a[0], s.x, b.x), __builtin_fmaf(a[1], s.y, b.y), __builtin_fmaf(a[2], s.z, b.z),
+                       __builtin_fmaf(a[3], s.w, b.w));
 }
+
+template <int OUT, int ACT>
+__device__ __forceinline__ void finish8(const GemmParams& p, long m, int n0, const float4 a, const float4 b, const uint4 r0,
+                                        const uint4 r1, sp_flags_t& ovm) {
+#pragma clang fp contract(off)
+    float v[8] = {a.x, a.y, a.z, a.w, b.x, b.y, b.z, b.w};
+    float r[8];
+    if constexpr (OUT == 0) {
+        r[0] = __builtin_bit_cast(float, r0.x); r[1] = __builtin_bit_cast(float, r0.y);
+        r[2] = __builtin_bit_cast(float, r0.z); r[3] = __builtin_bit_cast(float, r0.w);
+        r[4] = __builtin_bit_cast(float, r1.x); r[5] = __builtin_bit_cast(float, r1.y);
+        r[6] = __builtin_bit_cast(float, r1.z); r[7] = __builtin_bit_cast(float, r1.w);
+    } else if constexpr (OUT == 1) {
+        const uint32_t w[4] = {r0.x, r0.y, r0.z, r0.w};
+#pragma unroll
+        for (int j = 0; j < 4; ++j) { r[2 * j] = bf2f((bf16_t)(w[j] & 0xffff)); r[2 * j + 1] = bf2f((bf16_t)(w[j] >> 16)); }
+    } else {
+        sp_join8(r0, r1, r);
+    }
+#pragma unroll
+    for (int j = 0; j < 8; ++j) {
+        float x = p.res_after ? v[j] : v[j] + r[j];
+        if constexpr (ACT == 1) x = relu_nan(x);
+        if constexpr (ACT == 2) x = gelu_erf(x);
+        if constexpr (ACT == 3) x = gelu_fast(x);
+        v[j] = p.res_after ? x + r[j] : x;
+    }
+    const long e = m * p.ldY + p.yoff + n0;
+    if constexpr (OUT == 0) {
+        char* yp = p.Y + e * 4;
+        *reinterpret_cast<float4*>(yp) = make_float4(v[0], v[1], v[2], v[3]);
+        *reinterpret_cast<float4*>(yp + 16) = make_float4(v[4], v[5], v[6], v[7]);
+    } else if constexpr (OUT == 1) {
+        uint4 t;
+        t.x = (uint32_t)f2bf(v[0]) | ((uint32_t)f2bf(v[1]) << 16);
+        t.y = (uint32_t)f2bf(v[2]) | ((uint32_t)f2bf(v[3]) << 16);
+        t.z = (uint32_t)f2bf(v[4]) | ((uint32_t)f2bf(v[5]) << 16);
+        t.w = (uint32_t)f2bf(v[6]) | ((uint32_t)f2bf(v[7]) << 16);
+        *reinterpret_cast<uint4*>(p.Y + e * 2) = t;
+    } else {
+        float amax = 0.f;
+        uint4 h, l;
+        sp_split8(v, amax, h, l);
+        sp_flag(ovm, amax);
+        char* yp = p.Y + sp32_byte(e);
+        *reinterpret_cast<uint4*>(yp) = h;
+        *reinterpret_cast<uint4*>(yp + 64) = l;
+    }
+}
+
+}
diff --git a/avcer_amd/engine.py b/avcer_amd/engine.py
--- a/avcer_amd/engine.py
+++ b/avcer_amd/engine.py
@@ -834,6 +834,15 @@
                                                 self._stream()))
         return y
 
+    def stem_pool_u8_conv1(self, frames_u8, w_split, scale, shifts9, w1_frags, scale1, bias1):
+        fr = self._dev(frames_u8, torch.uint8)
+        n, h, w = int(fr.shape[0]), int(fr.shape[1]), int(fr.shape[2])
+        y = torch.empty(n, 55, 55, 128, dtype=torch.int16, device=self.device)
+        t1 = torch.empty_like(y)
+        self._check(self.lib.avcer_stem_pool_u8_conv1(self.ctx, _ptr(fr), n, h, w, _ptr(w_split), _ptr(scale), _ptr(shifts9), _ptr(y),
+                                                      _ptr(w1_frags), _ptr(scale1), _ptr(bias1), _ptr(t1), self._stream()))
+        return y, t1
+
     def gemm_stats(self, reset: bool = True):
         n, f = C.c_int64(0), C.c_double(0.0)
         self._check(self.lib.avcer_gemm_stats(self.ctx, C.byref(n), C.byref(f), int(reset)))
diff --git a/include/avcer_hip.h b/include/avcer_hip.h
--- a/include/avcer_hip.h
+++ b/include/avcer_hip.h
@@ -265,6 +265,9 @@
                     const float* bias, void* y, int n, avcer_stream_t stream);
 int avcer_stem_pool_u8(avcer_ctx* ctx, const uint8_t* frames, int n, int in_h, int in_w, const void* w, const float* scale,
                        const float* shifts9, void* y, avcer_stream_t stream);
+int avcer_stem_pool_u8_conv1(avcer_ctx* ctx, const uint8_t* frames, int n, int in_h, int in_w, const void* w, const float* scale,
+                             const float* shifts9, void* y, const void* w1_frags, const float* scale1, const float* bias1, void* t1,
+                             avcer_stream_t stream);
 
 int avcer_split_weights(avcer_ctx* ctx, const float* w, void* out, size_t numel, avcer_stream_t stream);
 
```

New measurement: 2196 (median of 6 runs). No clear change (+0.2%).
